# Bluear7878/Remote-Sensing-Vision-Language-Diffusion-Model

Measured on NVIDIA B200. Metric: stage2_denoise_steps_per_s_1024sq_cfg2, higher is better.
Workload: dtype bf16

## Files before the change

include/b200sr.h:

```cpp
#ifndef B200SR_H_
#define B200SR_H_

#include <stddef.h>
#include <stdint.h>

#ifdef __cplusplus
extern "C" {
#endif

int b200sr_abi_version(void);
int b200sr_num_sms(void);

typedef struct b200sr_epilogue {
  const float* bias;
  const float* rowvec;
  int32_t rows_per_group;
  int64_t ld_rowvec;
  const void* residual;
  int64_t ldr;
  void* out;
  int64_t ldc;
  int32_t out_fp32;
  int32_t geglu;
  float alpha;
  int32_t act;
  int32_t softmax_valid;
  int32_t w_dynamic;
  int32_t w_rows_per_group;
  int64_t w_group_stride;
  const float* a_gn_stats;
  const float* a_gn_weight;
  const float* a_gn_bias;
  int32_t a_gn_groups;
  int32_t a_gn_silu;
  const float* ln_stats;
  int32_t ln_parts;
  const float* ln_colsum;
  const float* ln_shift;
  float ln_eps;
  float* ln_stats_out;
  int32_t row_softmax;
  int32_t row_softmax_valid;
} b200sr_epilogue;

int b200sr_gemm_bf16(const void* A, int64_t lda, const void* W, int32_t M, int32_t N, int32_t K,
                     const b200sr_epilogue* epi, int32_t force_bn, void* stream);

int b200sr_gemm_n_tile(int32_t M, int32_t N, int32_t K);

int b200sr_conv3x3_bf16(const void* x, const void* w, int32_t N, int32_t H, int32_t W, int32_t Cin, int32_t Cout,
                        int32_t stride, int32_t pad_lo, const b200sr_epilogue* epi, int32_t force_bn, void* stream);

int b200sr_conv3x3_small(const void* x, const void* w, const float* bias, const void* addend, void* y, int32_t N,
                         int32_t H, int32_t W, int32_t Cin, int32_t Cout, int32_t out_nchw_f32, void* stream);

size_t b200sr_group_norm_workspace_bytes(int32_t N, int32_t HW, int32_t C, int32_t groups);
int b200sr_group_norm_launches(int32_t N, int32_t HW, int32_t C, int32_t groups);
int b200sr_group_norm_nhwc(const void* x, void* y, const float* weight, const float* bias, int32_t N, int32_t HW,
                           int32_t C, int32_t groups, float eps, int32_t silu, const void* sft_gamma,
                           const void* sft_beta, const void* raw, float control_scale, void* workspace, void* stream);

int b200sr_group_norm_stats(const void* x, int32_t N, int32_t HW, int32_t C, int32_t groups, float eps, float* stats_out,
                            void* workspace, void* stream);

int b200sr_layer_norm(const void* x, void* y, const float* weight, const float* bias, int32_t M, int32_t C, float eps,
                      void* stream);

size_t b200sr_attention_d64_workspace_bytes(int32_t B, int32_t H, int32_t Nq, int32_t Nk);
int b200sr_attention_d64(const void* q, int64_t ldq, int32_t q_col, const void* k, int64_t ldk, int32_t k_col,
                         const void* v, int64_t ldv, int32_t v_col, void* out, int64_t ldo, int32_t B, int32_t H,
                         int32_t Nq, int32_t Nk, float scale, int32_t causal, void* workspace, void* stream);

int b200sr_row_softmax_fold(const float* parts, int32_t n_parts, int64_t rows, float* out, void* stream);

int b200sr_softmax_rows(const float* x, void* y, int32_t rows, int32_t cols, int32_t valid_cols, float scale,
                        void* stream);

int b200sr_nchw_f32_to_nhwc_bf16(const float* x, void* y, int32_t N, int32_t C, int32_t HW, float scale, void* stream);
int b200sr_nhwc_bf16_to_nchw_f32(const void* x, float* y, int32_t N, int32_t C, int32_t HW, void* stream);
int b200sr_nhwc_bf16_to_nchw_f32_strided(const void* x, float* y, int32_t N, int32_t C, int32_t Cs, int32_t HW, void* stream);

int b200sr_upsample2x_nhwc(const void* x, void* y, int32_t N, int32_t H, int32_t W, int32_t C, void* stream);

int b200sr_concat_add(const void* a, int32_t Ca, const void* b, int32_t Cb, const void* c, void* out, int64_t rows,
                      void* stream);

int b200sr_axpy_bf16(const void* a, const void* b, void* y, float alpha, int64_t n, void* stream);

int b200sr_pad_channels(const void* x, void* y, int32_t C, int32_t Cpad, int64_t rows, void* stream);

int b200sr_silu_bf16(const void* x, void* y, int64_t n, void* stream);

int b200sr_embed_tokens(const int64_t* ids, const float* tok, const float* pos, void* out, int32_t B, int32_t T, int32_t C,
                        int32_t vocab, void* stream);

int b200sr_sinusoid_embedding(const float* t, void* out, int32_t B, int32_t dim, float max_period, int32_t sin_first,
                              void* stream);

int b200sr_sampler_pre(const float* x, const float* noise, const float* scalars, float* x_hat, void* net_in, int32_t B,
                       int32_t C, int32_t HW, int32_t cfg_copies, void* stream);
int b200sr_sampler_post(const float* eps, const float* x_hat, const float* scalars, float* denoised_out, float* x_next,
                        int32_t B, int32_t C, int32_t HW, int32_t use_cfg, void* stream);
int b200sr_euler_from_denoised(const float* denoised, const float* x_hat, const float* scalars, float* x_next,
                               int64_t n, void* stream);

int b200sr_tile_accumulate(const float* tile, const float* weight, float* acc, float* cnt, int32_t BC, int32_t th,
                           int32_t tw, int32_t H, int32_t W, int32_t h0, int32_t w0, void* stream);
int b200sr_tile_normalize(const float* acc, const float* cnt, float* out, int64_t n, void* stream);

int b200sr_tile_weighted_strip(const float* tile, const float* weight, float* strip, int32_t BC, int32_t th, int32_t tw,
                               int32_t y0, int32_t x0, int32_t sh, int32_t sw, void* stream);
int b200sr_strip_add(const float* strip, float* acc, int32_t BC, int32_t sh, int32_t sw, int32_t H, int32_t W,
                     int32_t h0, int32_t w0, void* stream);

int b200sr_pointwise_small(const void* x, const float* w, const float* bias, void* y, int32_t Cin, int32_t Cout,
                           int64_t rows, int32_t HW, int32_t out_nchw_f32, float scale, void* stream);
int b200sr_diag_gaussian(const float* moments, const float* noise, float* z, int32_t N, int32_t C, int32_t HW,
                         float scale, void* stream);

int b200sr_wavelet_level(const float* img, float* low, float* high, int32_t first, int32_t BC, int32_t H, int32_t W,
                         int32_t radius, void* stream);
int b200sr_add_f32(const float* a, const float* b, float* out, int64_t n, void* stream);
int b200sr_image_to_u8(const float* x, void* out, int32_t C, int32_t H, int32_t W, int32_t OH, int32_t OW, void* stream);

int b200sr_tensor2img_u8(const float* x, void* out, int32_t C, int32_t H, int32_t W, void* stream);
int b200sr_resample_u8(const void* src, void* dst, int32_t outer, int32_t in_len, int32_t out_len, int32_t inner,
                       const int32_t* bounds, const int32_t* coeffs, int32_t ksize, void* stream);
int b200sr_img_u8_to_tensor(const void* in, float* out, int32_t C, int32_t H, int32_t W, void* stream);

typedef struct b200sr_copy {
  const void* src;
  void* dst;
  int64_t bytes;
} b200sr_copy;
int b200sr_copy_batch(const b200sr_copy* copies, int32_t n, void* stream);

int b200sr_rel_l1_similarity(const void* prev, const void* cur, int64_t n, const float* threshold, void* workspace,
                             float* result, void* stream);

int b200sr_sr3_update(const float* x, const float* eps, const float* noise, const float* scalars, float* out,
                      int64_t n, void* stream);

#ifdef __cplusplus
}
#endif
#endif
```

remote-sensing-vision-language-diffusion-model_b200/b200sr/_lib.py:

```python
from __future__ import annotations

import ctypes as C
import os

_HERE = os.path.dirname(os.path.abspath(__file__))
LIB_PATH = os.path.join(_HERE, os.environ.get("B200SR_LIB", "libb200sr.so"))

ABI_VERSION = 6

c_void_p, c_int, c_i64, c_float, c_size_t = C.c_void_p, C.c_int32, C.c_int64, C.c_float, C.c_size_t


class Epilogue(C.Structure):

    _fields_ = [
        ("bias", c_void_p),
        ("rowvec", c_void_p),
        ("rows_per_group", c_int),
        ("ld_rowvec", c_i64),
        ("residual", c_void_p),
        ("ldr", c_i64),
        ("out", c_void_p),
        ("ldc", c_i64),
        ("out_fp32", c_int),
        ("geglu", c_int),
        ("alpha", c_float),
        ("act", c_int),
        ("softmax_valid", c_int),
        ("w_dynamic", c_int),
        ("w_rows_per_group", c_int),
        ("w_group_stride", c_i64),
        ("a_gn_stats", c_void_p),
        ("a_gn_weight", c_void_p),
        ("a_gn_bias", c_void_p),
        ("a_gn_groups", c_int),
        ("a_gn_silu", c_int),
        ("ln_stats", c_void_p),
        ("ln_parts", c_int),
        ("ln_colsum", c_void_p),
        ("ln_shift", c_void_p),
        ("ln_eps", c_float),
        ("ln_stats_out", c_void_p),
        ("row_softmax", c_int),
        ("row_softmax_valid", c_int),
    ]


class Copy(C.Structure):

    _fields_ = [("src", c_void_p), ("dst", c_void_p), ("bytes", c_i64)]


def binding_snippet() -> str:
    names = {c_void_p: "C.c_void_p", c_int: "C.c_int32", c_i64: "C.c_int64", c_float: "C.c_float"}
    out = []
    for cls, cname in ((Epilogue, "b200sr_epilogue"), (Copy, "b200sr_copy")):
        out.append(f"class {cls.__name__}(C.Structure):  # {cname} (ABI version {ABI_VERSION})")
        out.append("    _fields_ = [")
        for fname, ftype in cls._fields_:
            out.append(f'        ("{fname}", {names[ftype]}),')
        out.append("    ]")
        out.append("")
    return "\n".join(out).rstrip() + "\n"


P = c_void_p
SIGNATURES = {
    "b200sr_abi_version": (c_int, []),
    "b200sr_num_sms": (c_int, []),
    "b200sr_gemm_bf16": (c_int, [P, c_i64, P, c_int, c_int, c_int, C.POINTER(Epilogue), c_int, P]),
    "b200sr_gemm_n_tile": (c_int, [c_int, c_int, c_int]),
    "b200sr_row_softmax_fold": (c_int, [P, c_int, c_i64, P, P]),
    "b200sr_conv3x3_bf16": (c_int, [P, P, c_int, c_int, c_int, c_int, c_int, c_int, c_int, C.POINTER(Epilogue), c_int, P]),
    "b200sr_pointwise_small": (c_int, [P, P, P, P, c_int, c_int, c_i64, c_int, c_int, c_float, P]),
    "b200sr_diag_gaussian": (c_int, [P, P, P, c_int, c_int, c_int, c_float, P]),
    "b200sr_conv3x3_small": (c_int, [P, P, P, P, P, c_int, c_int, c_int, c_int, c_int, c_int, P]),
    "b200sr_group_norm_workspace_bytes": (c_size_t, [c_int, c_int, c_int, c_int]),
    "b200sr_group_norm_launches": (c_int, [c_int, c_int, c_int, c_int]),
    "b200sr_group_norm_nhwc": (
        c_int,
        [P, P, P, P, c_int, c_int, c_int, c_int, c_float, c_int, P, P, P, c_float, P, P],
    ),
    "b200sr_group_norm_stats": (c_int, [P, c_int, c_int, c_int, c_int, c_float, P, P, P]),
    "b200sr_layer_norm": (c_int, [P, P, P, P, c_int, c_int, c_float, P]),
    "b200sr_attention_d64": (
        c_int,
        [P, c_i64, c_int, P, c_i64, c_int, P, c_i64, c_int, P, c_i64, c_int, c_int, c_int, c_int, c_float, c_int, P, P],
    ),
    "b200sr_attention_d64_workspace_bytes": (C.c_size_t, [c_int, c_int, c_int, c_int]),
    "b200sr_softmax_rows": (c_int, [P, P, c_int, c_int, c_int, c_float, P]),
    "b200sr_nchw_f32_to_nhwc_bf16": (c_int, [P, P, c_int, c_int, c_int, c_float, P]),
    "b200sr_nhwc_bf16_to_nchw_f32": (c_int, [P, P, c_int, c_int, c_int, P]),
    "b200sr_nhwc_bf16_to_nchw_f32_strided": (c_int, [P, P, c_int, c_int, c_int, c_int, P]),
    "b200sr_upsample2x_nhwc": (c_int, [P, P, c_int, c_int, c_int, c_int, P]),
    "b200sr_concat_add": (c_int, [P, c_int, P, c_int, P, P, c_i64, P]),
    "b200sr_axpy_bf16": (c_int, [P, P, P, c_float, c_i64, P]),
    "b200sr_silu_bf16": (c_int, [P, P, c_i64, P]),
    "b200sr_pad_channels": (c_int, [P, P, c_int, c_int, c_i64, P]),
    "b200sr_embed_tokens": (c_int, [P, P, P, P, c_int, c_int, c_int, c_int, P]),
    "b200sr_sinusoid_embedding": (c_int, [P, P, c_int, c_int, c_float, c_int, P]),
    "b200sr_sampler_pre": (c_int, [P, P, P, P, P, c_int, c_int, c_int, c_int, P]),
    "b200sr_sampler_post": (c_int, [P, P, P, P, P, c_int, c_int, c_int, c_int, P]),
    "b200sr_euler_from_denoised": (c_int, [P, P, P, P, c_i64, P]),
    "b200sr_tile_accumulate": (c_int, [P, P, P, P, c_int, c_int, c_int, c_int, c_int, c_int, c_int, P]),
    "b200sr_tile_normalize": (c_int, [P, P, P, c_i64, P]),
    "b200sr_rel_l1_similarity": (c_int, [P, P, c_i64, P, P, P, P]),
    "b200sr_sr3_update": (c_int, [P, P, P, P, P, c_i64, P]),
    "b200sr_wavelet_level": (c_int, [P, P, P, c_int, c_int, c_int, c_int, c_int, P]),
    "b200sr_add_f32": (c_int, [P, P, P, c_i64, P]),
    "b200sr_image_to_u8": (c_int, [P, P, c_int, c_int, c_int, c_int, c_int, P]),
    "b200sr_tensor2img_u8": (c_int, [P, P, c_int, c_int, c_int, P]),
    "b200sr_resample_u8": (c_int, [P, P, c_int, c_int, c_int, c_int, P, P, c_int, P]),
    "b200sr_img_u8_to_tensor": (c_int, [P, P, c_int, c_int, c_int, P]),
    "b200sr_copy_batch": (c_int, [C.POINTER(Copy), c_int, P]),
    "b200sr_tile_weighted_strip": (c_int, [P, P, P, c_int, c_int, c_int, c_int, c_int, c_int, c_int, P]),
    "b200sr_strip_add": (c_int, [P, P, c_int, c_int, c_int, c_int, c_int, c_int, c_int, P]),
}

_ERRORS = {-22: "EINVAL (bad shape / alignment / flags)", -19: "ENODEV (no sm_100 device / driver)", -5: "EIO (CUDA launch error)"}

_lib = None


class B200SRError(RuntimeError):
    pass


def load() -> C.CDLL:
    global _lib
    if _lib is not None:
        return _lib
    if not os.path.exists(LIB_PATH):
        raise B200SRError(
            f"{LIB_PATH} not found: build the sm_100a extension first "
            "(python -c 'import __graft_entry__ as g; g.build()' or csrc/build.sh). There is no CPU fallback."
        )
    lib = C.CDLL(LIB_PATH)
    for name, (res, args) in SIGNATURES.items():
        fn = getattr(lib, name)
        fn.restype = res
        fn.argtypes = args
    if lib.b200sr_abi_version() != ABI_VERSION:
        raise B200SRError(f"libb200sr.so ABI {lib.b200sr_abi_version()} != binding ABI {ABI_VERSION}; rebuild")
    _lib = lib
    return lib


LAUNCHES = [0]


TRACE = None


def check(rc: int, what: str, kernels: int = 1) -> None:
    LAUNCHES[0] += kernels
    if TRACE is not None:
        TRACE.extend([what] * kernels)
    if rc != 0:
        raise B200SRError(f"{what} failed: {_ERRORS.get(rc, rc)}")
```

remote-sensing-vision-language-diffusion-model_b200/b200sr/modules.py:

```python
from __future__ import annotations

import os
from typing import Dict, List, Optional

import torch
import torch.nn as nn

from . import ops

bf16 = torch.bfloat16


def exists(x):
    return x is not None


def zero_module(module: nn.Module) -> nn.Module:
    for p in module.parameters():
        p.detach().zero_()
    return module


def to_nhwc(x: torch.Tensor) -> torch.Tensor:
    if x.dim() != 4:
        raise ValueError(f"expected a 4-D NCHW tensor, got {tuple(x.shape)}")
    v = x.permute(0, 2, 3, 1)
    if x.dtype == bf16 and v.is_contiguous():
        return v
    if x.dtype == torch.float32 and x.is_contiguous():
        return ops.nchw_to_nhwc_bf16(x)
    return v.to(bf16).contiguous()


def from_nhwc(y: torch.Tensor) -> torch.Tensor:
    return y.permute(0, 3, 1, 2)


def tokens_bf16(x: torch.Tensor) -> torch.Tensor:
    if x.dtype == bf16 and x.is_contiguous():
        return x
    if x.dtype == torch.float32:
        return ops.cast_bf16(x.contiguous())
    return x.to(bf16).contiguous()


class Packed:

    def _pk(self, name: str, params, fn):
        cache = self.__dict__.setdefault("_pk_cache", {})
        key = tuple((p.data_ptr(), p._version, str(p.device)) for p in params)
        hit = cache.get(name)
        if hit is None or hit[0] != key:
            with torch.no_grad():
                hit = (key, fn(*params))
            cache[name] = hit
        return hit[1]


_F32 = lambda p: p.detach().float().contiguous()


def _silu_of(emb: torch.Tensor) -> torch.Tensor:
    s = getattr(emb, "_b200sr_silu", None)
    if s is None:
        s = ops.silu(tokens_bf16(emb))
        try:
            emb._b200sr_silu = s
        except Exception:
            pass
    return s


class EmbSlot:

    def __init__(self, table):
        self._b200sr_rb = table


def _resblocks_of(root: nn.Module):
    blocks = root.__dict__.get("_b200sr_resblocks")
    if blocks is None:
        blocks = [m for m in root.modules() if isinstance(m, ResBlock)]
        root.__dict__["_b200sr_resblocks"] = blocks
    return blocks


def rb_table(root: nn.Module, proj: torch.Tensor):
    table, off = {}, 0
    for blk in _resblocks_of(root):
        table[id(blk)] = proj[:, off:off + blk.out_channels]
        off += blk.out_channels
    return table


def _project_emb_for_resblocks(holder: Packed, root: nn.Module, emb: torch.Tensor) -> Optional[torch.Tensor]:
    blocks = _resblocks_of(root)
    if not blocks:
        return None
    params = tuple(p for blk in blocks for p in (blk.emb_layers[1].weight, blk.emb_layers[1].bias))
    w_all, b_all = holder._pk("rb_emb", params, lambda *ps: (
        torch.cat([ops.pack_linear(w) for w in ps[0::2]], 0).contiguous(),
        torch.cat([_F32(b) for b in ps[1::2]], 0).contiguous()))
    proj = ops.gemm(_silu_of(emb), w_all, b_all, out_fp32=True)
    try:
        emb._b200sr_rb = rb_table(root, proj)
        emb._b200sr_proj = proj
    except Exception:
        pass
    return proj


def timestep_embedding(timesteps: torch.Tensor, dim: int, max_period: float = 10000.0) -> torch.Tensor:
    return ops.sinusoid_embedding(timesteps, dim, max_period, sin_first=False)


class GroupNorm32(nn.GroupNorm):
    """util.py:258-276 — parameter container; the fused kernel is invoked by the owning block."""


def normalization(channels: int) -> nn.GroupNorm:
    return GroupNorm32(32, channels)


def _gn(norm: nn.GroupNorm, x_nhwc: torch.Tensor, silu: bool = False, **kw) -> torch.Tensor:
    return ops.group_norm(x_nhwc, norm.weight, norm.bias, groups=norm.num_groups, eps=norm.eps, silu=silu, **kw)


def _conv3x3(holder: Packed, name: str, conv: nn.Conv2d, x_nhwc: torch.Tensor, **kw) -> torch.Tensor:
    w = holder._pk(name + ".w", (conv.weight,), ops.pack_conv3x3)
    b = holder._pk(name + ".b", (conv.bias,), _F32) if conv.bias is not None else None
    return ops.conv3x3(x_nhwc, w, b, **kw)


FUSE_LN_INTO_GEMM = os.environ.get("B200SR_FUSE_LN", "1") != "0"
FUSE_GN_INTO_CONV = True


def _gn_silu_conv3x3(holder: Packed, name: str, norm: nn.GroupNorm, conv: nn.Conv2d, x_nhwc: torch.Tensor, **kw) -> torch.Tensor:
    if FUSE_GN_INTO_CONV and ops.conv3x3_gn_fusable(x_nhwc, 1, conv.out_channels) and norm.affine:
        stats = ops.group_norm_stats(x_nhwc, norm.num_groups, norm.eps)
        return _conv3x3(holder, name, conv, x_nhwc, gn=(stats, norm.weight, norm.bias, norm.num_groups, True), **kw)
    return _conv3x3(holder, name, conv, _gn(norm, x_nhwc, silu=True), **kw)


def _linear(holder: Packed, name: str, lin, x: torch.Tensor, **kw) -> torch.Tensor:
    w = holder._pk(name + ".w", (lin.weight,), ops.pack_linear)
    b = holder._pk(name + ".b", (lin.bias,), _F32) if lin.bias is not None else None
    return ops.gemm(x, w, b, **kw)


class TimestepBlock(nn.Module):
    """openaimodel.py:63-72."""


class Upsample(nn.Module, Packed):

    def __init__(self, channels, use_conv, dims=2, out_channels=None, padding=1, third_up=False):
        super().__init__()
        assert dims == 2 and padding == 1
        self.channels, self.out_channels, self.use_conv, self.dims = channels, out_channels or channels, use_conv, dims
        if use_conv:
            self.conv = nn.Conv2d(self.channels, self.out_channels, 3, padding=padding)

    def forward_nhwc(self, x):
        assert x.shape[-1] == self.channels
        x = ops.upsample2x(x)
        return _conv3x3(self, "conv", self.conv, x) if self.use_conv else x

    def forward(self, x):
        return from_nhwc(self.forward_nhwc(to_nhwc(x)))


class Downsample(nn.Module, Packed):

    def __init__(self, channels, use_conv, dims=2, out_channels=None, padding=1, third_down=False):
        super().__init__()
        assert dims == 2 and use_conv and padding == 1, "only the learned stride-2 convolution is on the hot path"
        self.channels, self.out_channels, self.use_conv, self.dims = channels, out_channels or channels, use_conv, dims
        self.op = nn.Conv2d(self.channels, self.out_channels, 3, stride=2, padding=padding)

    def forward_nhwc(self, x):
        assert x.shape[-1] == self.channels
        return _conv3x3(self, "op", self.op, x, stride=2)

    def forward(self, x):
        return from_nhwc(self.forward_nhwc(to_nhwc(x)))


class ResBlock(TimestepBlock, Packed):

    def __init__(self, channels, emb_channels, dropout, out_channels=None, use_conv=False, use_scale_shift_norm=False,
                 dims=2, use_checkpoint=False, up=False, down=False, kernel_size=3, exchange_temb_dims=False,
                 skip_t_emb=False):
        super().__init__()
        assert dims == 2 and kernel_size == 3 and not (up or down or use_scale_shift_norm or skip_t_emb or use_conv)
        self.channels, self.emb_channels, self.dropout = channels, emb_channels, dropout
        self.out_channels = out_channels or channels
        self.use_checkpoint, self.use_scale_shift_norm = use_checkpoint, use_scale_shift_norm
        self.in_layers = nn.Sequential(normalization(channels), nn.SiLU(),
                                       nn.Conv2d(channels, self.out_channels, 3, padding=1))
        self.updown = False
        self.h_upd = self.x_upd = nn.Identity()
        self.emb_layers = nn.Sequential(nn.SiLU(), nn.Linear(emb_channels, self.out_channels))
        self.out_layers = nn.Sequential(normalization(self.out_channels), nn.SiLU(), nn.Dropout(p=dropout),
                                        zero_module(nn.Conv2d(self.out_channels, self.out_channels, 3, padding=1)))
        if self.out_channels == channels:
            self.skip_connection = nn.Identity()
        else:
            self.skip_connection = nn.Conv2d(channels, self.out_channels, 1)

    def forward_nhwc(self, x, emb):
        pre = getattr(emb, "_b200sr_rb", None)
        emb_out = pre.get(id(self)) if pre is not None else None
        if emb_out is None:
            emb_out = _linear(self, "emb", self.emb_layers[1], _silu_of(emb), out_fp32=True)
        h = _gn_silu_conv3x3(self, "conv1", self.in_layers[0], self.in_layers[2], x, rowvec=emb_out)
        skip = x if isinstance(self.skip_connection, nn.Identity) else _linear(self, "skip", self.skip_connection, x)
        return _gn_silu_conv3x3(self, "conv2", self.out_layers[0], self.out_layers[3], h, residual=skip)

    def forward(self, x, emb):
        return from_nhwc(self.forward_nhwc(to_nhwc(x), emb))


class GEGLU(nn.Module, Packed):

    def __init__(self, dim_in, dim_out):
        super().__init__()
        self.proj = nn.Linear(dim_in, dim_out * 2)

    def forward(self, x, ln=None):
        if ln is not None:
            norm, stats = ln
            w, colsum, shift = self._pk("proj_ln", (self.proj.weight, self.proj.bias, norm.weight, norm.bias),
                                        ops.pack_geglu_ln)
            return ops.gemm(tokens_bf16(x), w, None, geglu=True, ln=(stats, colsum, shift, norm.eps))
        w, b = self._pk("proj", (self.proj.weight, self.proj.bias), ops.pack_geglu)
        return ops.gemm(tokens_bf16(x), w, b, geglu=True)


class FeedForward(nn.Module, Packed):

    def __init__(self, dim, dim_out=None, mult=4, glu=False, dropout=0.0):
        super().__init__()
        assert glu, "only the gated feed-forward is on the hot path"
        inner_dim = int(dim * mult)
        dim_out = dim_out or dim
        self.net = nn.Sequential(GEGLU(dim, inner_dim), nn.Dropout(dropout), nn.Linear(inner_dim, dim_out))

    def forward(self, x, residual: Optional[torch.Tensor] = None, ln=None, want_stats: bool = False):
        return _linear(self, "out", self.net[2], self.net[0](x, ln=ln), residual=residual, want_stats=want_stats)


class CrossAttention(nn.Module, Packed):

    def __init__(self, query_dim, context_dim=None, heads=8, dim_head=64, dropout=0.0, backend=None):
        super().__init__()
        assert dim_head == 64, "the tcgen05 attention kernel is specialised for head_dim 64"
        inner_dim = dim_head * heads
        context_dim = context_dim or query_dim
        self.scale, self.heads = dim_head**-0.5, heads
        self.to_q = nn.Linear(query_dim, inner_dim, bias=False)
        self.to_k = nn.Linear(context_dim, inner_dim, bias=False)
        self.to_v = nn.Linear(context_dim, inner_dim, bias=False)
        self.to_out = nn.Sequential(nn.Linear(inner_dim, query_dim), nn.Dropout(dropout))
        self.backend = backend

    def attend(self, x, context=None, kv=None, ln=None):
        inner = self.to_q.weight.shape[0]
        if context is None:
            if ln is not None:
                norm, stats = ln
                w, colsum, shift = self._pk(
                    "qkv_ln", (self.to_q.weight, self.to_k.weight, self.to_v.weight, norm.weight, norm.bias),
                    lambda q, k, v, g, b: ops.pack_linear_ln(torch.cat([q, k, v], 0), g, b))
                qkv = ops.gemm(x, w, ln=(stats, colsum, shift, norm.eps))
            else:
                w = self._pk("qkv", (self.to_q.weight, self.to_k.weight, self.to_v.weight),
                             lambda q, k, v: torch.cat([q, k, v], 0).to(bf16).contiguous())
                qkv = ops.gemm(x, w)
            return ops.attention(qkv, qkv, qkv, self.heads, q_col=0, k_col=inner, v_col=2 * inner, scale=self.scale)
        q = _linear(self, "q", self.to_q, x)
        bound = self._bound_entry(context)
        if kv is not None:
            pass
        elif bound is not None:
            kv = bound[1]
        else:
            kv = ops.gemm(context, self._wkv())
        if kv.shape[0] != q.shape[0]:
            if q.shape[0] % kv.shape[0]:
                raise ValueError(f"context batch {kv.shape[0]} does not divide the query batch {q.shape[0]}")
            kv = kv.repeat_interleave(q.shape[0] // kv.shape[0], dim=0)
        return ops.attention(q, kv, kv, self.heads, q_col=0, k_col=0, v_col=inner, scale=self.scale)

    def _wkv(self):
        return self._pk("kv", (self.to_k.weight, self.to_v.weight), lambda k, v: torch.cat([k, v], 0).to(bf16).contiguous())

    def _fold_norm(self) -> Optional[nn.LayerNorm]:
        return self.__dict__.get("_pre_norm") if FUSE_LN_INTO_GEMM else None

    def _weights_key(self):
        ps = [self.to_q.weight, self.to_k.weight, self.to_v.weight, self.to_out[0].weight]
        norm = self._fold_norm()
        if norm is not None:
            ps += [norm.weight, norm.bias]
        return tuple((p.data_ptr(), p._version) for p in ps)

    def _bound_entry(self, context):
        if context is None:
            return None
        table = self.__dict__.get("_static")
        if not table:
            return None
        e = table.get(id(context))
        if e is None or e[0] is not context:
            return None
        if e[3] != self._weights_key():
            if torch.cuda.is_current_stream_capturing():
                raise RuntimeError("cross-attention weights changed after bind_static_context(); re-bind before capture")
            self.bind_static_context(context)
            e = table[id(context)]
        return e

    def bind_static_context(self, context: Optional[torch.Tensor]) -> None:
        table = self.__dict__.setdefault("_static", {})
        if context is None:
            table.clear()
            return
        old = table.get(id(context))
        shape = (*context.shape[:-1], 2 * self.to_q.weight.shape[0])
        same = old is not None and old[0] is context and tuple(old[1].shape) == shape
        kv = ops.gemm(context, self._wkv(), out=old[1] if same else None)
        fused = self._fold_projections(context)
        if same and old[2] is not None and fused is not None and len(old[2]) == len(fused):
            for dst, src in zip(old[2], fused):
                dst.copy_(src)
            fused = old[2]
        table[id(context)] = (context, kv, fused, self._weights_key())

    def bound_tensors(self, context):
        e = self.__dict__.get("_static", {}).get(id(context))
        if e is None or e[0] is not context:
            return []
        return [e[1]] + ([t for t in e[2] if t.is_cuda or t.dim() > 0] if e[2] is not None else [])

    SEG = 80

    @torch.no_grad()
    def _fold_projections(self, context: torch.Tensor):
        b, tk = context.shape[0], context.shape[1]
        if context.dim() != 3 or tk > self.SEG:
            return None
        h, c = self.heads, self.to_q.weight.shape[1]
        ctx = context.float()
        k = (ctx @ self.to_k.weight.float().t()).view(b, tk, h, 64)
        v = (ctx @ self.to_v.weight.float().t()).view(b, tk, h, 64)
        wq = self.to_q.weight.float().view(h, 64, c)
        wo = self.to_out[0].weight.float().view(-1, h, 64)
        kp = torch.zeros(b, h, self.SEG, c, device=context.device)
        kp[:, :, :tk] = torch.einsum("bjhd,hdc->bhjc", k, wq) * (self.scale * 1.4426950408889634)
        vp = torch.zeros(b, h, self.SEG, wo.shape[0], device=context.device)
        vp[:, :, :tk] = torch.einsum("bjhd,chd->bhjc", v, wo)
        kp = kp.reshape(b, h * self.SEG, c)
        vpt = vp.reshape(b, h * self.SEG, -1).transpose(1, 2).to(bf16).contiguous()
        norm = self._fold_norm()
        if norm is None:
            return (kp.to(bf16).contiguous(), vpt, torch.tensor(tk))
        kg = (kp * norm.weight.float()).to(bf16).contiguous()
        return (kg, vpt, torch.tensor(tk), kg.float().sum(-1).contiguous(), (kp @ norm.bias.float()).contiguous())

    def forward(self, x, context=None, mask=None, additional_tokens=None, n_times_crossframe_attn_in_self=0,
                residual: Optional[torch.Tensor] = None, alpha: float = 1.0, kv: Optional[torch.Tensor] = None,
                ln=None, want_stats: bool = False):
        if mask is not None or additional_tokens is not None or n_times_crossframe_attn_in_self:
            raise NotImplementedError("masks / additional tokens / cross-frame attention are not on the hot path")
        x = tokens_bf16(x)
        ctx = tokens_bf16(context) if context is not None else None
        if ctx is not None and kv is None and x.dim() == 3 and x.shape[1] % 256 == 0:
            bound = self._bound_entry(ctx)
            folds_ln = bound is not None and bound[2] is not None and len(bound[2]) == 5
            if folds_ln and (ln is None or ln[0] is not self._fold_norm()):
                bound = None
            if bound is not None and bound[2] is not None and x.shape[0] % bound[2][0].shape[0] == 0:
                k_fold, v_fold, tk = bound[2][:3]
                rpg = x.shape[1] * (x.shape[0] // k_fold.shape[0])
                if folds_ln:
                    p = ops.gemm(x, k_fold, softmax_valid=int(tk), w_rows_per_group=rpg,
                                 ln=(ln[1], bound[2][3], bound[2][4], ln[0].eps))
                else:
                    if ln is not None:
                        x = ops.layer_norm(x, ln[0].weight, ln[0].bias, ln[0].eps)
                    p = ops.gemm(x, k_fold, softmax_valid=int(tk), w_rows_per_group=rpg)
                bias = self._pk("out.b", (self.to_out[0].bias,), _F32)
                return ops.gemm(p, v_fold, bias, residual=residual, alpha=alpha, w_rows_per_group=rpg,
                                want_stats=want_stats)
        if ln is not None and ctx is not None:
            x, ln = ops.layer_norm(x, ln[0].weight, ln[0].bias, ln[0].eps), None
        return _linear(self, "out", self.to_out[0], self.attend(x, ctx, kv, ln=ln), residual=residual, alpha=alpha,
                       want_stats=want_stats)


MemoryEfficientCrossAttention = CrossAttention


class BasicTransformerBlock(nn.Module):

    def __init__(self, dim, n_heads, d_head, dropout=0.0, context_dim=None, gated_ff=True, checkpoint=True,
                 disable_self_attn=False, attn_mode="softmax", sdp_backend=None):
        super().__init__()
        self.disable_self_attn = disable_self_attn
        self.attn1 = CrossAttention(query_dim=dim, heads=n_heads, dim_head=d_head, dropout=dropout,
                                    context_dim=context_dim if disable_self_attn else None)
        self.ff = FeedForward(dim, dropout=dropout, glu=gated_ff)
        self.attn2 = CrossAttention(query_dim=dim, context_dim=context_dim, heads=n_heads, dim_head=d_head,
                                    dropout=dropout)
        self.norm1, self.norm2, self.norm3 = nn.LayerNorm(dim), nn.LayerNorm(dim), nn.LayerNorm(dim)
        self.checkpoint = checkpoint
        self.attn2.__dict__["_pre_norm"] = self.norm2

    @staticmethod
    def _ln(norm: nn.LayerNorm, x):
        return ops.layer_norm(x, norm.weight, norm.bias, norm.eps)

    def forward(self, x, context=None, additional_tokens=None, n_times_crossframe_attn_in_self=0, stats=None,
                want_stats: bool = False):
        x = tokens_bf16(x)
        if stats is None:
            x = self.attn1(self._ln(self.norm1, x), context=context if self.disable_self_attn else None, residual=x)
            x = self.attn2(self._ln(self.norm2, x), context=context, residual=x)
            return self.ff(self._ln(self.norm3, x), residual=x, want_stats=want_stats)
        x, stats = self.attn1(x, context=context if self.disable_self_attn else None, residual=x,
                              ln=(self.norm1, stats), want_stats=True)
        x, stats = self.attn2(x, context=context, residual=x, ln=(self.norm2, stats), want_stats=True)
        return self.ff(x, residual=x, ln=(self.norm3, stats), want_stats=want_stats)


class SpatialTransformer(nn.Module, Packed):

    def __init__(self, in_channels, n_heads, d_head, depth=1, dropout=0.0, context_dim=None, disable_self_attn=False,
                 use_linear=False, attn_type="softmax", use_checkpoint=True, sdp_backend=None):
        super().__init__()
        assert use_linear, "the YAML selects use_linear_in_transformer=True"
        if exists(context_dim) and not isinstance(context_dim, (list, tuple)):
            context_dim = [context_dim]
        if exists(context_dim):
            context_dim = list(context_dim)
            if depth != len(context_dim):
                assert all(c == context_dim[0] for c in context_dim)
                context_dim = depth * [context_dim[0]]
        else:
            context_dim = [None] * depth
        self.in_channels = in_channels
        inner_dim = n_heads * d_head
        self.norm = nn.GroupNorm(num_groups=32, num_channels=in_channels, eps=1e-6, affine=True)
        self.proj_in = nn.Linear(in_channels, inner_dim)
        self.transformer_blocks = nn.ModuleList([
            BasicTransformerBlock(inner_dim, n_heads, d_head, dropout=dropout, context_dim=context_dim[d],
                                  disable_self_attn=disable_self_attn, attn_mode=attn_type, checkpoint=use_checkpoint)
            for d in range(depth)])
        self.proj_out = zero_module(nn.Linear(inner_dim, in_channels))
        self.use_linear = use_linear

    def forward_nhwc(self, x, context=None):
        if not isinstance(context, list):
            context = [context]
        context = [tokens_bf16(c) if c is not None else None for c in context]
        b, h, w, c = x.shape
        t = _gn(self.norm, x).view(b, h * w, c)
        stats = None
        if FUSE_LN_INTO_GEMM:
            t, stats = _linear(self, "proj_in", self.proj_in, t, want_stats=True)
        else:
            t = _linear(self, "proj_in", self.proj_in, t)
        last = len(self.transformer_blocks) - 1
        for i, block in enumerate(self.transformer_blocks):
            r = block(t, context=context[i if len(context) > 1 else 0], stats=stats,
                      want_stats=stats is not None and i < last)
            t, stats = r if isinstance(r, tuple) else (r, None)
        t = _linear(self, "proj_out", self.proj_out, t, residual=x.view(b, h * w, c))
        return t.view(b, h, w, c)

    def forward(self, x, context=None):
        return from_nhwc(self.forward_nhwc(to_nhwc(x), context))


class TimestepEmbedSequential(nn.Sequential, TimestepBlock):

    def forward_nhwc(self, x, emb, context=None):
        for layer in self:
            if isinstance(layer, TimestepBlock):
                x = layer.forward_nhwc(x, emb)
            elif isinstance(layer, SpatialTransformer):
                x = layer.forward_nhwc(x, context)
            elif isinstance(layer, nn.Conv2d):
                x = _stem_conv(layer, x)
            else:
                x = layer.forward_nhwc(x)
        return x

    def forward(self, x, emb, context=None, **unused):
        return from_nhwc(self.forward_nhwc(to_nhwc(x), emb, context))


def _stem_conv(conv: nn.Conv2d, x_nhwc: torch.Tensor, addend: Optional[torch.Tensor] = None) -> torch.Tensor:
    cache = conv.__dict__.setdefault("_pk_cache", {})
    key = (conv.weight.data_ptr(), conv.weight._version, conv.bias.data_ptr(), conv.bias._version)
    if cache.get("key") != key:
        with torch.no_grad():
            cache["key"], cache["w"], cache["b"] = key, ops.pack_conv3x3_padded(conv.weight, 64), _F32(conv.bias)
    return ops.conv3x3(ops.pad_channels(x_nhwc, 64), cache["w"], cache["b"], residual=addend)


class UNetModel(nn.Module, Packed):

    def __init__(self, in_channels, model_channels, out_channels, num_res_blocks, attention_resolutions, dropout=0,
                 channel_mult=(1, 2, 4, 8), conv_resample=True, dims=2, num_classes=None, use_checkpoint=False,
                 use_fp16=False, num_heads=-1, num_head_channels=-1, num_heads_upsample=-1, use_scale_shift_norm=False,
                 resblock_updown=False, use_new_attention_order=False, use_spatial_transformer=False,
                 transformer_depth=1, context_dim=None, n_embed=None, legacy=True, disable_self_attentions=None,
                 num_attention_blocks=None, disable_middle_self_attn=False, use_linear_in_transformer=False,
                 spatial_transformer_attn_type="softmax", adm_in_channels=None, use_fairscale_checkpoint=False,
                 offload_to_cpu=False, transformer_depth_middle=None, _build_output_blocks=True):
        super().__init__()
        assert use_spatial_transformer and context_dim is not None and dims == 2 and conv_resample
        assert not resblock_updown and not use_scale_shift_norm and n_embed is None
        assert num_head_channels != -1 or num_heads != -1
        if isinstance(context_dim, (list, tuple)) or type(context_dim).__name__ == "ListConfig":
            context_dim = list(context_dim)
        self.in_channels, self.model_channels, self.out_channels = in_channels, model_channels, out_channels
        if isinstance(transformer_depth, int):
            transformer_depth = len(channel_mult) * [transformer_depth]
        transformer_depth = list(transformer_depth)
        transformer_depth_middle = transformer_depth[-1] if transformer_depth_middle is None else transformer_depth_middle
        if isinstance(num_res_blocks, int):
            self.num_res_blocks = len(channel_mult) * [num_res_blocks]
        else:
            if len(num_res_blocks) != len(channel_mult):
                raise ValueError("provide num_res_blocks either as an int (globally constant) or as a list/tuple "
                                 "(per-level) with the same length as channel_mult")
            self.num_res_blocks = list(num_res_blocks)
        self.attention_resolutions, self.dropout, self.channel_mult = attention_resolutions, dropout, channel_mult
        self.conv_resample, self.num_classes, self.use_checkpoint = conv_resample, num_classes, use_checkpoint
        self.num_heads, self.num_head_channels = num_heads, num_head_channels
        self.num_heads_upsample = num_heads if num_heads_upsample == -1 else num_heads_upsample
        self.predict_codebook_ids = False

        time_embed_dim = model_channels * 4
        self.time_embed = nn.Sequential(nn.Linear(model_channels, time_embed_dim), nn.SiLU(),
                                        nn.Linear(time_embed_dim, time_embed_dim))
        if num_classes is not None:
            if num_classes != "sequential":
                raise ValueError("only num_classes='sequential' (SDXL vector conditioning) is on the hot path")
            assert adm_in_channels is not None
            self.label_emb = nn.Sequential(nn.Sequential(nn.Linear(adm_in_channels, time_embed_dim), nn.SiLU(),
                                                         nn.Linear(time_embed_dim, time_embed_dim)))

        def heads_for(ch):
            if num_head_channels == -1:
                return num_heads, ch // num_heads
            return ch // num_head_channels, num_head_channels

        def transformer(ch, depth, level=None, middle=False):
            nh, dh = heads_for(ch)
            if legacy:
                dh = ch // nh
            disabled = disable_middle_self_attn if middle else (
                disable_self_attentions[level] if exists(disable_self_attentions) else False)
            return SpatialTransformer(ch, nh, dh, depth=depth, context_dim=context_dim, disable_self_attn=disabled,
                                      use_linear=use_linear_in_transformer, attn_type=spatial_transformer_attn_type,
                                      use_checkpoint=use_checkpoint)

        self.input_blocks = nn.ModuleList([TimestepEmbedSequential(nn.Conv2d(in_channels, model_channels, 3, padding=1))])
        input_block_chans = [model_channels]
        ch, ds = model_channels, 1
        for level, mult in enumerate(channel_mult):
            for nr in range(self.num_res_blocks[level]):
                layers = [ResBlock(ch, time_embed_dim, dropout, out_channels=mult * model_channels, dims=dims,
                                   use_checkpoint=use_checkpoint)]
                ch = mult * model_channels
                if ds in attention_resolutions and (not exists(num_attention_blocks) or nr < num_attention_blocks[level]):
                    layers.append(transformer(ch, transformer_depth[level], level))
                self.input_blocks.append(TimestepEmbedSequential(*layers))
                input_block_chans.append(ch)
            if level != len(channel_mult) - 1:
                self.input_blocks.append(TimestepEmbedSequential(Downsample(ch, conv_resample, dims=dims, out_channels=ch)))
                input_block_chans.append(ch)
                ds *= 2
        self.middle_block = TimestepEmbedSequential(
            ResBlock(ch, time_embed_dim, dropout, dims=dims, use_checkpoint=use_checkpoint),
            transformer(ch, transformer_depth_middle, middle=True),
            ResBlock(ch, time_embed_dim, dropout, dims=dims, use_checkpoint=use_checkpoint))
        if not _build_output_blocks:
            return
        self.output_blocks = nn.ModuleList([])
        for level, mult in list(enumerate(channel_mult))[::-1]:
            for i in range(self.num_res_blocks[level] + 1):
                ich = input_block_chans.pop()
                layers = [ResBlock(ch + ich, time_embed_dim, dropout, out_channels=model_channels * mult, dims=dims,
                                   use_checkpoint=use_checkpoint)]
                ch = model_channels * mult
                if ds in attention_resolutions and (not exists(num_attention_blocks) or i < num_attention_blocks[level]):
                    layers.append(transformer(ch, transformer_depth[level], level))
                if level and i == self.num_res_blocks[level]:
                    layers.append(Upsample(ch, conv_resample, dims=dims, out_channels=ch))
                    ds //= 2
                self.output_blocks.append(TimestepEmbedSequential(*layers))
        self.out = nn.Sequential(normalization(ch), nn.SiLU(),
                                 zero_module(nn.Conv2d(model_channels, out_channels, 3, padding=1)))

    def _embed(self, timesteps, y):
        t_emb = timestep_embedding(timesteps, self.model_channels)
        h = _linear(self, "te0", self.time_embed[0], t_emb, act=1)
        if self.num_classes is None:
            emb = _linear(self, "te2", self.time_embed[2], h)
        else:
            emb_t = _linear(self, "te2", self.time_embed[2], h)
            l = _linear(self, "le0", self.label_emb[0][0], tokens_bf16(y), act=1)
            emb = _linear(self, "le2", self.label_emb[0][2], l, residual=emb_t)
        _project_emb_for_resblocks(self, self, emb)
        return emb

    def _out_nchw_f32(self, h_nhwc):
        h = _gn(self.out[0], h_nhwc, silu=True)
        conv = self.out[2]
        w8, b8 = self._pk("out.wb8", (conv.weight, conv.bias), ops.pack_conv3x3_few_out)
        return ops.conv3x3_to_nchw_f32(h, w8, b8, conv.weight.shape[0])

    def forward(self, x, timesteps=None, context=None, y=None, **kwargs):
        assert (y is not None) == (self.num_classes is not None)
        emb = self._embed(timesteps, y)
        ctx = tokens_bf16(context)
        h, hs = to_nhwc(x), []
        for module in self.input_blocks:
            h = module.forward_nhwc(h, emb, ctx)
            hs.append(h)
        h = self.middle_block.forward_nhwc(h, emb, ctx)
        for module in self.output_blocks:
            h = module.forward_nhwc(ops.concat_add(h, hs.pop()), emb, ctx)
        return self._out_nchw_f32(h)


class ZeroSFT(nn.Module, Packed):

    def __init__(self, label_nc, norm_nc, concat_channels=0, norm=True, mask=False):
        super().__init__()
        assert norm
        self.norm = norm
        self.param_free_norm = normalization(norm_nc + concat_channels)
        nhidden = 128
        self.mlp_shared = nn.Sequential(nn.Conv2d(label_nc, nhidden, kernel_size=3, padding=1), nn.SiLU())
        self.zero_mul = zero_module(nn.Conv2d(nhidden, norm_nc + concat_channels, kernel_size=3, padding=1))
        self.zero_add = zero_module(nn.Conv2d(nhidden, norm_nc + concat_channels, kernel_size=3, padding=1))
        self.zero_conv = zero_module(nn.Conv2d(label_nc, norm_nc, 1, 1, 0))
        self.pre_concat = bool(concat_channels != 0)
        self.mask = mask

    def precompute(self, c):
        actv = _conv3x3(self, "mlp", self.mlp_shared[0], c, act=1)
        return {"zc": _linear(self, "zero_conv", self.zero_conv, c),
                "gamma": _conv3x3(self, "mul", self.zero_mul, actv), "beta": _conv3x3(self, "add", self.zero_add, actv)}

    def forward_nhwc(self, c, h, h_ori=None, control_scale=1, pre=None):
        assert self.mask is False
        cat = h_ori is not None and self.pre_concat
        if h_ori is not None and not self.pre_concat:
            raise NotImplementedError("post-concat ZeroSFT is not used by LightGLVUNet")
        control_scale = float(control_scale)
        if pre is None:
            hz = _linear(self, "zero_conv", self.zero_conv, c, residual=h)
            hc = ops.concat_add(h_ori, hz) if cat else hz
            actv = _conv3x3(self, "mlp", self.mlp_shared[0], c, act=1)
            gamma = _conv3x3(self, "mul", self.zero_mul, actv)
            beta = _conv3x3(self, "add", self.zero_add, actv)
        else:
            hc = ops.concat_add(h_ori, h, pre["zc"]) if cat else ops.axpy(h, pre["zc"], 1.0)
            gamma, beta = pre["gamma"], pre["beta"]
        raw = None
        if control_scale != 1.0:
            raw = ops.concat_add(h_ori, h) if cat else h
        return _gn(self.param_free_norm, hc, sft_gamma=gamma, sft_beta=beta, raw=raw, control_scale=control_scale)

    def forward(self, c, h, h_ori=None, control_scale=1):
        return from_nhwc(self.forward_nhwc(to_nhwc(c), to_nhwc(h), None if h_ori is None else to_nhwc(h_ori),
                                           control_scale))


class ZeroCrossAttn(nn.Module, Packed):

    def __init__(self, context_dim, query_dim, zero_out=True, mask=False):
        super().__init__()
        self.attn = CrossAttention(query_dim=query_dim, context_dim=context_dim, heads=query_dim // 64, dim_head=64)
        self.norm1 = normalization(query_dim)
        self.norm2 = normalization(context_dim)
        self.mask = mask

    def precompute(self, context):
        b, h, w, cc = context.shape
        ct = _gn(self.norm2, context).view(b, h * w, cc)
        return {"kv": ops.gemm(ct, self.attn._wkv())}

    def forward_nhwc(self, context, x, control_scale=1, pre=None):
        assert self.mask is False
        b, h, w, c = x.shape
        xt = _gn(self.norm1, x).view(b, h * w, c)
        if pre is None:
            ct = _gn(self.norm2, context).view(b, h * w, context.shape[-1])
            out = self.attn(xt, ct, residual=x.view(b, h * w, c), alpha=float(control_scale))
        else:
            out = self.attn(xt, xt, residual=x.view(b, h * w, c), alpha=float(control_scale), kv=pre["kv"])
        return out.view(b, h, w, c)

    def forward(self, context, x, control_scale=1):
        return from_nhwc(self.forward_nhwc(to_nhwc(context), to_nhwc(x), control_scale))


class GLVControl(UNetModel):

    def __init__(self, *args, input_upscale=1, **kwargs):
        super().__init__(*args, _build_output_blocks=False, **kwargs)
        assert input_upscale == 1
        self.input_upscale = input_upscale
        self.input_hint_block = TimestepEmbedSequential(
            zero_module(nn.Conv2d(self.in_channels, self.model_channels, 3, padding=1)))

    def forward_nhwc(self, x, timesteps, xt, context, y, emb=None) -> List[torch.Tensor]:
        if emb is None:
            emb = self._embed(timesteps, y)
        hint = _stem_conv(self.input_hint_block[0], x)
        hs = []
        h = _stem_conv(self.input_blocks[0][0], xt, addend=hint)
        hs.append(h)
        for module in list(self.input_blocks)[1:]:
            h = module.forward_nhwc(h, emb, context)
            hs.append(h)
        hs.append(self.middle_block.forward_nhwc(h, emb, context))
        return hs

# ... 189 lines not shown
```

remote-sensing-vision-language-diffusion-model_b200/b200sr/ops.py:

```python
from __future__ import annotations

import ctypes as C
import math
from typing import Optional

import numpy as np
import torch

from . import _lib
from ._lib import Epilogue, check

bf16 = torch.bfloat16


def launch_count() -> int:
    return _lib.LAUNCHES[0]


_profile = None


def set_profile(records) -> None:
    global _profile
    _profile = records


class _Timed:
    def __init__(self, kind: str, flops: float, desc: str = ""):
        self.kind, self.flops, self.desc = kind, flops, desc

    def __enter__(self):
        if _profile is not None:
            self.t0 = torch.cuda.Event(enable_timing=True)
            self.t1 = torch.cuda.Event(enable_timing=True)
            self.t0.record()
        return self

    def __exit__(self, *exc):
        if _profile is not None:
            self.t1.record()
            _profile.append((self.kind, self.flops, self.t0, self.t1, self.desc))
        return False


def _stream() -> int:
    return torch.cuda.current_stream().cuda_stream


def _ptr(t: Optional[torch.Tensor]) -> Optional[int]:
    return None if t is None else t.data_ptr()


def _req(t: torch.Tensor, dtype, name: str) -> None:
    if not t.is_cuda:
        raise _lib.B200SRError(f"{name}: expected a CUDA tensor (b200sr has no CPU path)")
    if t.device.index != torch.cuda.current_device():
        raise _lib.B200SRError(f"{name}: tensor lives on {t.device} but the current CUDA device is "
                               f"{torch.cuda.current_device()}; wrap the call in torch.cuda.device(tensor.device)")
    if t.dtype != dtype:
        raise _lib.B200SRError(f"{name}: expected {dtype}, got {t.dtype}")
    if not t.is_contiguous():
        raise _lib.B200SRError(f"{name}: expected a contiguous tensor")


def require_cuda(t: torch.Tensor, what: str) -> None:
    if not t.is_cuda:
        raise _lib.B200SRError(f"{what} runs on CUDA (sm_100a) only; there is no CPU fallback")


_ws_cache: dict = {}
_ws_retired: list = []
_ws_slot = [0]


class workspace_slot:

    def __init__(self, slot: int):
        self.slot = slot

    def __enter__(self):
        self.prev = _ws_slot[0]
        _ws_slot[0] = self.slot

    def __exit__(self, *exc):
        _ws_slot[0] = self.prev
        return False


def _workspace(device: torch.device, nbytes: int, kind: str = "gn") -> torch.Tensor:
    key = (device.type, device.index, _ws_slot[0], kind)
    ws = _ws_cache.get(key)
    if ws is None or ws.numel() * 4 < nbytes:
        if torch.cuda.is_current_stream_capturing():
            raise _lib.B200SRError("workspace allocation during CUDA-graph capture; run one eager warm-up step first")
        if ws is not None:
            _ws_retired.append(ws)
        floats = max(nbytes // 4 + 1, 1 << 22, 0 if ws is None else 2 * ws.numel())
        ws = torch.zeros(floats, dtype=torch.float32, device=device)
        _ws_cache[key] = ws
    return ws


def pack_linear(weight: torch.Tensor) -> torch.Tensor:
    w = weight.detach().reshape(weight.shape[0], -1)
    return w.to(bf16).contiguous()


def pack_conv3x3(weight: torch.Tensor) -> torch.Tensor:
    co, ci, kh, kw = weight.shape
    assert kh == 3 and kw == 3
    return weight.detach().permute(0, 2, 3, 1).reshape(co, 9 * ci).to(bf16).contiguous()


def geglu_interleave_index(inner: int, device=None) -> torch.Tensor:
    assert inner % 16 == 0
    j = torch.arange(inner, device=device)
    val_pos = (j // 16) * 32 + (j % 16)
    idx = torch.empty(2 * inner, dtype=torch.long, device=device)
    idx[val_pos] = j
    idx[val_pos + 16] = j + inner
    return idx


def pack_geglu(weight: torch.Tensor, bias: torch.Tensor):
    inner = weight.shape[0] // 2
    idx = geglu_interleave_index(inner, weight.device)
    return weight.detach()[idx].to(bf16).contiguous(), bias.detach()[idx].float().contiguous()


def pack_linear_ln(weight: torch.Tensor, gamma: torch.Tensor, beta: torch.Tensor, bias: Optional[torch.Tensor] = None):
    w32 = weight.detach().float()
    wp = (w32 * gamma.detach().float()[None, :]).to(bf16).contiguous()
    shift = w32 @ beta.detach().float()
    if bias is not None:
        shift = shift + bias.detach().float()
    return wp, wp.float().sum(1)[None].contiguous(), shift[None].contiguous()


def pack_geglu_ln(weight: torch.Tensor, bias: torch.Tensor, gamma: torch.Tensor, beta: torch.Tensor):
    idx = geglu_interleave_index(weight.shape[0] // 2, weight.device)
    return pack_linear_ln(weight.detach()[idx], gamma, beta, bias.detach()[idx])


class RowStats:

    __slots__ = ("buf", "parts", "dim")

    def __init__(self, buf: torch.Tensor, parts: int, dim: int):
        self.buf, self.parts, self.dim = buf, parts, dim


_n_tile_cache: dict = {}


def gemm_n_tile(M: int, N: int, K: int) -> int:
    key = (M, N, K)
    t = _n_tile_cache.get(key)
    if t is None:
        t = _lib.load().b200sr_gemm_n_tile(M, N, K)
        if t <= 0:
            raise _lib.B200SRError(f"gemm_n_tile({M}, {N}, {K}) = {t}")
        _n_tile_cache[key] = t
    return t


def _epilogue(out, ldc, bias, rowvec, rows_per_group, residual, ldr, out_fp32, geglu, alpha, act=0,
              softmax_valid=0, w_rows_per_group=0, w_group_stride=0, w_dynamic=False) -> Epilogue:
    e = Epilogue()
    e.bias = _ptr(bias)
    e.rowvec = _ptr(rowvec)
    e.rows_per_group = rows_per_group
    e.ld_rowvec = rowvec.stride(0) if rowvec is not None and rowvec.dim() == 2 else 0
    e.residual = _ptr(residual)
    e.ldr = ldr
    e.out = out.data_ptr()
    e.ldc = ldc
    e.out_fp32 = int(out_fp32)
    e.geglu = int(geglu)
    e.alpha = float(alpha)
    e.act = int(act)
    e.softmax_valid = int(softmax_valid)
    e.w_dynamic = int(w_dynamic)
    e.w_rows_per_group = int(w_rows_per_group)
    e.w_group_stride = int(w_group_stride)
    return e


def gemm(
    a: torch.Tensor,
    w: torch.Tensor,
    bias: Optional[torch.Tensor] = None,
    *,
    residual: Optional[torch.Tensor] = None,
    rowvec: Optional[torch.Tensor] = None,
    rows_per_group: int = 0,
    geglu: bool = False,
    alpha: float = 1.0,
    act: int = 0,
    out: Optional[torch.Tensor] = None,
    out_fp32: bool = False,
    force_bn: int = 0,
    softmax_valid: int = 0,
    w_rows_per_group: int = 0,
    w_dynamic: bool = False,
    ln=None,
    want_stats: bool = False,
):
    _req(w, bf16, "gemm.w")
    if a.dtype != bf16 or not a.is_cuda:
        raise _lib.B200SRError("gemm.a: expected CUDA bf16")
    K = a.shape[-1]
    N = w.shape[-2]
    w_group_stride = 0
    if w_rows_per_group:
        assert w.dim() == 3 and w.is_contiguous() and w.shape[0] * w_rows_per_group >= a.numel() // K
        w_group_stride = N
    a2 = a.reshape(-1, K)
    if a2.stride(-1) != 1:
        a2 = a2.contiguous()
    M, lda = a2.shape[0], a2.stride(0)
    n_out = N // 2 if geglu else N
    if out is None:
        out = torch.empty(*a.shape[:-1], n_out, dtype=torch.float32 if out_fp32 else bf16, device=a.device)
    o2 = out.reshape(-1, n_out) if out.is_contiguous() else out
    assert o2.shape[-1] == n_out and o2.stride(-1) == 1
    ldc = o2.stride(-2) if o2.dim() >= 2 else n_out
    ldr = 0
    if residual is not None:
        r2 = residual if residual.dim() == 2 else residual.reshape(-1, residual.shape[-1])
        assert r2.dtype == bf16 and r2.stride(-1) == 1
        ldr = r2.stride(0)
    e = _epilogue(o2, ldc, bias, rowvec, rows_per_group, residual, ldr, out_fp32, geglu, alpha, act,
                  softmax_valid, w_rows_per_group, w_group_stride, w_dynamic)
    if ln is not None:
        st, colsum, shift, eps = ln
        groups = w.shape[0] if w_rows_per_group else 1
        if st.buf.shape[1] != M or st.dim != K:
            raise _lib.B200SRError(f"gemm.ln: statistics of a [{st.buf.shape[1]}, {st.dim}] matrix, a is [{M}, {K}]")
        for t, nme in ((colsum, "colsum"), (shift, "shift")):
            _req(t, torch.float32, f"gemm.ln.{nme}")
            if t.numel() != groups * N:
                raise _lib.B200SRError(f"gemm.ln.{nme}: expected [{groups}, {N}]")
        e.ln_stats, e.ln_parts, e.ln_colsum, e.ln_shift, e.ln_eps = st.buf.data_ptr(), st.parts, colsum.data_ptr(), \
            shift.data_ptr(), float(eps)
    stats = None
    if want_stats:
        if geglu or softmax_valid or out_fp32:
            raise _lib.B200SRError("gemm.want_stats: plain bf16 output only")
        parts = -(-N // (force_bn if force_bn > 0 else gemm_n_tile(M, N, K)))
        stats = RowStats(torch.empty(parts, M, 2, dtype=torch.float32, device=a.device), parts, N)
        e.ln_stats_out = stats.buf.data_ptr()
    with _Timed("gemm", 2.0 * M * N * K, f"M{M} N{N} K{K}{' geglu' if geglu else ''}{' ln' if ln is not None else ''}"):
        rc = _lib.load().b200sr_gemm_bf16(a2.data_ptr(), lda, w.data_ptr(), M, N, K, C.byref(e), force_bn, _stream())
    check(rc, f"gemm M={M} N={N} K={K}")
    return (out, stats) if want_stats else out


def conv3x3(
    x: torch.Tensor,
    w: torch.Tensor,
    bias: Optional[torch.Tensor] = None,
    *,
    stride: int = 1,
    rowvec: Optional[torch.Tensor] = None,
    residual: Optional[torch.Tensor] = None,
    alpha: float = 1.0,
    act: int = 0,
    out: Optional[torch.Tensor] = None,
    force_bn: int = 0,
    pad_lo: int = 1,
    gn=None,
) -> torch.Tensor:
    _req(x, bf16, "conv3x3.x")
    _req(w, bf16, "conv3x3.w")
    n, h, wd, cin = x.shape
    cout = w.shape[0]
    assert w.shape[1] == 9 * cin
    oh, ow = h // stride, wd // stride
    if out is None:
        out = torch.empty(n, oh, ow, cout, dtype=bf16, device=x.device)
    ldc = out.stride(2)
    ldr = residual.stride(2) if residual is not None else 0
    e = _epilogue(out, ldc, bias, rowvec, 0, residual, ldr, False, False, alpha, act)
    if gn is not None:
        stats, gw, gb, groups, gsilu = gn
        _req(stats, torch.float32, "conv3x3.gn.stats")
        e.a_gn_stats, e.a_gn_weight, e.a_gn_bias = stats.data_ptr(), gw.data_ptr(), gb.data_ptr()
        e.a_gn_groups, e.a_gn_silu = int(groups), int(gsilu)
    with _Timed("conv3x3", 2.0 * n * oh * ow * cout * 9 * cin, f"{n}x{h}x{wd} Cin{cin} Cout{cout} s{stride}"):
        rc = _lib.load().b200sr_conv3x3_bf16(
            x.data_ptr(), w.data_ptr(), n, h, wd, cin, cout, stride, pad_lo, C.byref(e), force_bn, _stream()
        )
    check(rc, f"conv3x3 N={n} H={h} W={wd} Cin={cin} Cout={cout} s={stride}")
    return out


def conv3x3_small(
    x: torch.Tensor,
    w: torch.Tensor,
    bias: Optional[torch.Tensor],
    *,
    addend: Optional[torch.Tensor] = None,
    out_nchw_f32: bool = False,
) -> torch.Tensor:
    _req(x, bf16, "conv3x3_small.x")
    _req(w, bf16, "conv3x3_small.w")
    n, h, wd, cin = x.shape
    cout = w.shape[0]
    if out_nchw_f32:
        out = torch.empty(n, cout, h, wd, dtype=torch.float32, device=x.device)
    else:
        out = torch.empty(n, h, wd, cout, dtype=bf16, device=x.device)
    rc = _lib.load().b200sr_conv3x3_small(
        x.data_ptr(), w.data_ptr(), _ptr(bias), _ptr(addend), out.data_ptr(), n, h, wd, cin, cout, int(out_nchw_f32),
        _stream()
    )
    check(rc, f"conv3x3_small Cin={cin} Cout={cout}")
    return out


def group_norm(
    x: torch.Tensor,
    weight: Optional[torch.Tensor],
    bias: Optional[torch.Tensor],
    *,
    groups: int = 32,
    eps: float = 1e-5,
    silu: bool = False,
    sft_gamma: Optional[torch.Tensor] = None,
    sft_beta: Optional[torch.Tensor] = None,
    raw: Optional[torch.Tensor] = None,
    control_scale: float = 1.0,
) -> torch.Tensor:
    _req(x, bf16, "group_norm.x")
    n, c = x.shape[0], x.shape[-1]
    hw = x.numel() // (n * c)
    lib = _lib.load()
    ws = _workspace(x.device, lib.b200sr_group_norm_workspace_bytes(n, hw, c, groups))
    y = torch.empty_like(x)
    nbytes = 2.0 * x.numel() * (2 + (2 if sft_gamma is not None else 0) + (1 if raw is not None and control_scale != 1.0 else 0))
    with _Timed("group_norm", nbytes, f"N{n} HW{hw} C{c}{' sft' if sft_gamma is not None else ''}"):
        rc = lib.b200sr_group_norm_nhwc(
            x.data_ptr(), y.data_ptr(), _ptr(weight), _ptr(bias), n, hw, c, groups, eps, int(silu), _ptr(sft_gamma),
            _ptr(sft_beta), _ptr(raw), float(control_scale), ws.data_ptr(), _stream()
        )
    check(rc, f"group_norm N={n} HW={hw} C={c}", kernels=max(1, lib.b200sr_group_norm_launches(n, hw, c, groups)))
    return y


GN_FUSE_MAX_COUT = 256


def conv3x3_gn_fusable(x: torch.Tensor, stride: int = 1, cout: Optional[int] = None) -> bool:
    ok = stride == 1 and x.dim() == 4 and x.shape[2] % 8 == 0 and x.shape[1] >= 16 and x.shape[3] % 64 == 0
    return ok and (cout is None or cout <= GN_FUSE_MAX_COUT)


def group_norm_stats(x: torch.Tensor, groups: int = 32, eps: float = 1e-5) -> torch.Tensor:
    _req(x, bf16, "group_norm_stats.x")
    n, c = x.shape[0], x.shape[-1]
    hw = x.numel() // (n * c)
    lib = _lib.load()
    ws = _workspace(x.device, lib.b200sr_group_norm_workspace_bytes(n, hw, c, groups))
    stats = torch.empty(n, groups, 2, dtype=torch.float32, device=x.device)
    with _Timed("group_norm", 2.0 * x.numel(), f"N{n} HW{hw} C{c} stats"):
        rc = lib.b200sr_group_norm_stats(x.data_ptr(), n, hw, c, groups, eps, stats.data_ptr(), ws.data_ptr(), _stream())
    check(rc, f"group_norm_stats N={n} HW={hw} C={c}")
    return stats


def layer_norm(x: torch.Tensor, weight: torch.Tensor, bias: torch.Tensor, eps: float = 1e-5) -> torch.Tensor:
    _req(x, bf16, "layer_norm.x")
    c = x.shape[-1]
    m = x.numel() // c
    y = torch.empty_like(x)
    with _Timed("layer_norm", 4.0 * x.numel(), f"M{m} C{c}"):
        rc = _lib.load().b200sr_layer_norm(x.data_ptr(), y.data_ptr(), weight.data_ptr(), bias.data_ptr(), m, c, eps, _stream())
    check(rc, f"layer_norm M={m} C={c}")
    return y


def attention(
    q: torch.Tensor, k: torch.Tensor, v: torch.Tensor, heads: int, *, q_col: int = 0, k_col: int = 0, v_col: int = 0,
    scale: Optional[float] = None, causal: bool = False
) -> torch.Tensor:
    for t, nme in ((q, "q"), (k, "k"), (v, "v")):
        _req(t, bf16, f"attention.{nme}")
    b, nq, ldq = q.shape
    nk = k.shape[1]
    out = torch.empty(b, nq, heads * 64, dtype=bf16, device=q.device)
    lib = _lib.load()
    ws_bytes = lib.b200sr_attention_d64_workspace_bytes(b, heads, nq, nk)
    ws = _workspace(q.device, ws_bytes, "attn") if ws_bytes else None
    with _Timed("attention", 4.0 * b * heads * nq * nk * 64, f"B{b} H{heads} Nq{nq} Nk{nk}"):
        rc = lib.b200sr_attention_d64(
            q.data_ptr(), ldq, q_col, k.data_ptr(), k.shape[2], k_col, v.data_ptr(), v.shape[2], v_col, out.data_ptr(),
            heads * 64, b, heads, nq, nk, float(scale if scale is not None else 0.125), int(causal), _ptr(ws), _stream()
        )
    check(rc, f"attention B={b} H={heads} Nq={nq} Nk={nk}")
    return out


def softmax_rows(x: torch.Tensor, scale: float = 1.0, valid_cols: Optional[int] = None) -> torch.Tensor:
    _req(x, torch.float32, "softmax_rows.x")
    cols = x.shape[-1]
    y = torch.empty(x.shape, dtype=bf16, device=x.device)
    check(_lib.load().b200sr_softmax_rows(x.data_ptr(), y.data_ptr(), x.numel() // cols, cols,
                                          cols if valid_cols is None else valid_cols, float(scale), _stream()),
          "softmax_rows")
    return y


SCORE_CHUNK_BYTES = 1 << 30


def gemm_row_softmax(a: torch.Tensor, w: torch.Tensor, scale: float, valid_cols: Optional[int] = None,
                     w_dynamic: bool = True) -> torch.Tensor:
    _req(w, bf16, "gemm_row_softmax.w")
    _req(a, bf16, "gemm_row_softmax.a")
    K, N = a.shape[-1], w.shape[0]
    a2 = a.reshape(-1, K)
    if a2.stride(-1) != 1:
        a2 = a2.contiguous()
    M, lda = a2.shape[0], a2.stride(0)
    parts = -(-N // gemm_n_tile(M, N, K))
    stats = torch.empty(parts, M, 2, dtype=torch.float32, device=a.device)
    out = torch.empty(M, N, dtype=bf16, device=a.device)
    lib = _lib.load()
    folded = torch.empty(M, 2, dtype=torch.float32, device=a.device) if parts > 1 else stats
    for which in (1, 2):
        e = _epilogue(out, N, None, None, 0, None, 0, False, False, float(scale) * 1.4426950408889634, 0, 0, 0, 0, w_dynamic)
        e.row_softmax, e.row_softmax_valid = which, int(valid_cols) if valid_cols is not None else N
        if which == 1:
            e.out, e.ln_stats_out = None, stats.data_ptr()
        else:
            if parts > 1:
                check(lib.b200sr_row_softmax_fold(stats.data_ptr(), parts, M, folded.data_ptr(), _stream()), "row_softmax_fold")
            e.ln_stats, e.ln_parts = folded.data_ptr(), 1
        with _Timed("gemm", 2.0 * M * N * K, f"M{M} N{N} K{K} row softmax pass {which}"):
            rc = lib.b200sr_gemm_bf16(a2.data_ptr(), lda, w.data_ptr(), M, N, K, C.byref(e), 0, _stream())
        check(rc, f"gemm_row_softmax pass {which} M={M} N={N} K={K}")
    return out


TWO_PASS_SOFTMAX = True


def single_head_attention(q: torch.Tensor, k: torch.Tensor, v_t: torch.Tensor, scale: float,
                          out_bias: Optional[torch.Tensor] = None, valid_keys: Optional[int] = None) -> torch.Tensor:
    t, c = q.shape
    tk = k.shape[0]
    two_pass = TWO_PASS_SOFTMAX and tk % 8 == 0
    rows = (SCORE_CHUNK_BYTES // ((2 if two_pass else 4) * tk)) // 256 * 256
    rows = max(256, min(rows, t))
    out = torch.empty(t, c, dtype=bf16, device=q.device)
    for r0 in range(0, t, rows):
        r1 = min(t, r0 + rows)
        if two_pass:
            p = gemm_row_softmax(q[r0:r1], k, scale, valid_keys)
        else:
            s = gemm(q[r0:r1], k, out_fp32=True, w_dynamic=True)
            p = softmax_rows(s, scale, valid_cols=valid_keys)
        gemm(p, v_t, out_bias, w_dynamic=True, out=out[r0:r1])
    return out


def nchw_to_nhwc_bf16(x: torch.Tensor, scale: float = 1.0) -> torch.Tensor:
    _req(x, torch.float32, "nchw_to_nhwc.x")
    n, c, h, w = x.shape
    y = torch.empty(n, h, w, c, dtype=bf16, device=x.device)
    check(_lib.load().b200sr_nchw_f32_to_nhwc_bf16(x.data_ptr(), y.data_ptr(), n, c, h * w, float(scale), _stream()),
          "nchw_to_nhwc")
    return y


def cast_bf16(x: torch.Tensor) -> torch.Tensor:
    if x.dtype == bf16:
        return x if x.is_contiguous() else x.contiguous()
    _req(x, torch.float32, "cast_bf16.x")
    y = torch.empty(x.shape, dtype=bf16, device=x.device)
    check(_lib.load().b200sr_nchw_f32_to_nhwc_bf16(x.data_ptr(), y.data_ptr(), 1, 1, x.numel(), 1.0, _stream()),
          "cast_bf16")
    return y


def nhwc_to_nchw_f32(x: torch.Tensor) -> torch.Tensor:
    _req(x, bf16, "nhwc_to_nchw.x")
    n, h, w, c = x.shape
    y = torch.empty(n, c, h, w, dtype=torch.float32, device=x.device)
    check(_lib.load().b200sr_nhwc_bf16_to_nchw_f32(x.data_ptr(), y.data_ptr(), n, c, h * w, _stream()), "nhwc_to_nchw")
    return y


def pack_conv3x3_few_out(weight: torch.Tensor, bias: Optional[torch.Tensor]):
    co = weight.shape[0]
    w = torch.zeros(8, *weight.shape[1:], dtype=weight.dtype, device=weight.device)
    w[:co] = weight.detach()
    b = torch.zeros(8, dtype=torch.float32, device=weight.device)
    if bias is not None:
        b[:co] = bias.detach().float()
    return pack_conv3x3(w), b


def conv3x3_to_nchw_f32(x: torch.Tensor, w8: torch.Tensor, b8: torch.Tensor, cout: int) -> torch.Tensor:
    y8 = conv3x3(x, w8, b8)
    n, h, wd, cs = y8.shape
    out = torch.empty(n, cout, h, wd, dtype=torch.float32, device=x.device)
    check(_lib.load().b200sr_nhwc_bf16_to_nchw_f32_strided(y8.data_ptr(), out.data_ptr(), n, cout, cs, h * wd, _stream()),
          "nhwc_to_nchw_strided")
    return out


def upsample2x(x: torch.Tensor) -> torch.Tensor:
    _req(x, bf16, "upsample2x.x")
    n, h, w, c = x.shape
    y = torch.empty(n, 2 * h, 2 * w, c, dtype=bf16, device=x.device)
    check(_lib.load().b200sr_upsample2x_nhwc(x.data_ptr(), y.data_ptr(), n, h, w, c, _stream()), "upsample2x")
    return y


def concat_add(a: Optional[torch.Tensor], b: torch.Tensor, c: Optional[torch.Tensor] = None) -> torch.Tensor:
    _req(b, bf16, "concat_add.b")
    ca = 0 if a is None else a.shape[-1]
    cb = b.shape[-1]
    rows = b.numel() // cb
    out = torch.empty(*b.shape[:-1], ca + cb, dtype=bf16, device=b.device)
    check(_lib.load().b200sr_concat_add(_ptr(a), ca, b.data_ptr(), cb, _ptr(c), out.data_ptr(), rows, _stream()),
          "concat_add")
    return out


def axpy(a: torch.Tensor, b: torch.Tensor, alpha: float = 1.0) -> torch.Tensor:
    _req(a, bf16, "axpy.a")
    _req(b, bf16, "axpy.b")
    y = torch.empty_like(a)
    check(_lib.load().b200sr_axpy_bf16(a.data_ptr(), b.data_ptr(), y.data_ptr(), float(alpha), a.numel(), _stream()),
          "axpy")
    return y


def pad_channels(x: torch.Tensor, cpad: int) -> torch.Tensor:
    _req(x, bf16, "pad_channels.x")
    c = x.shape[-1]
    y = torch.empty(*x.shape[:-1], cpad, dtype=bf16, device=x.device)
    check(_lib.load().b200sr_pad_channels(x.data_ptr(), y.data_ptr(), c, cpad, x.numel() // c, _stream()), "pad_channels")
    return y


def pack_conv3x3_padded(weight: torch.Tensor, cin_pad: int) -> torch.Tensor:
    co, ci, kh, kw = weight.shape
    w = torch.zeros(co, 3, 3, cin_pad, dtype=weight.dtype, device=weight.device)
    w[..., :ci] = weight.detach().permute(0, 2, 3, 1)
    return w.reshape(co, 9 * cin_pad).to(bf16).contiguous()


def pointwise_small(x: torch.Tensor, w: torch.Tensor, bias: Optional[torch.Tensor], *, out_nchw_f32: bool = False,
                    scale: float = 1.0) -> torch.Tensor:
    _req(x, bf16, "pointwise_small.x")
    n, h, wd, cin = x.shape
    cout = w.shape[0]
# ... 262 lines not shown
```

remote-sensing-vision-language-diffusion-model_b200/csrc/capi.cu:

```cuda
#include "../../include/b200sr.h"
#include <stdlib.h>

#include "common.cuh"

namespace b200sr {

PFN_encodeTiled get_encode_tiled() {
  static PFN_encodeTiled fn = nullptr;
  static bool tried = false;
  if (!tried) {
    tried = true;
    void* p = nullptr;
    cudaDriverEntryPointQueryResult q;
    if (cudaGetDriverEntryPoint("cuTensorMapEncodeTiled", &p, cudaEnableDefault, &q) == cudaSuccess &&
        q == cudaDriverEntryPointSuccess)
      fn = reinterpret_cast<PFN_encodeTiled>(p);
  }
  return fn;
}

bool pdl_enabled() {
  static int v = -1;
  if (v < 0) {
    const char* e = getenv("B200SR_PDL");
    v = (e != nullptr && e[0] == '0') ? 0 : 1;
  }
  return v == 1;
}

int num_sms() {
  static int cached[64] = {0};
  int dev = 0;
  if (cudaGetDevice(&dev) != cudaSuccess || dev < 0 || dev >= 64) return 148;
  if (cached[dev] == 0) {
    int n = 0;
    if (cudaDeviceGetAttribute(&n, cudaDevAttrMultiProcessorCount, dev) != cudaSuccess || n <= 0) n = 148;
    cached[dev] = n;
  }
  return cached[dev];
}

bool first_use_on_device(bool (&flags)[64]) {
  int dev = 0;
  if (cudaGetDevice(&dev) != cudaSuccess || dev < 0 || dev >= 64) return true;
  if (flags[dev]) return false;
  flags[dev] = true;
  return true;
}

static int make_tmap_any(CUtensorMap* out, CUtensorMapDataType dtype, const void* base, int rank, const uint64_t* dims,
                         const uint64_t* strides_bytes, const uint32_t* box, int swizzle_bytes);

int make_tmap_bf16(CUtensorMap* out, const void* base, int rank, const uint64_t* dims, const uint64_t* strides_bytes,
                   const uint32_t* box, int swizzle_bytes) {
  return make_tmap_any(out, CU_TENSOR_MAP_DATA_TYPE_BFLOAT16, base, rank, dims, strides_bytes, box, swizzle_bytes);
}

int make_tmap_f32(CUtensorMap* out, const void* base, int rank, const uint64_t* dims, const uint64_t* strides_bytes,
                  const uint32_t* box) {
  return make_tmap_any(out, CU_TENSOR_MAP_DATA_TYPE_FLOAT32, base, rank, dims, strides_bytes, box, 128);
}

static int make_tmap_any(CUtensorMap* out, CUtensorMapDataType dtype, const void* base, int rank, const uint64_t* dims,
                         const uint64_t* strides_bytes, const uint32_t* box, int swizzle_bytes) {
  PFN_encodeTiled enc = get_encode_tiled();
  if (enc == nullptr) return B200SR_ENODEV;
  if ((reinterpret_cast<uintptr_t>(base) & 15) != 0) return B200SR_EINVAL;
  cuuint64_t gdim[5];
  cuuint64_t gstr[4];
  cuuint32_t bdim[5];
  cuuint32_t estr[5];
  for (int i = 0; i < rank; ++i) {
    gdim[i] = dims[i];
    bdim[i] = box[i];
    estr[i] = 1;
    if (box[i] == 0 || box[i] > 256) return B200SR_EINVAL;
  }
  for (int i = 0; i + 1 < rank; ++i) {
    gstr[i] = strides_bytes[i];
    if (gstr[i] % 16 != 0) return B200SR_EINVAL;
  }
  const CUresult r = enc(out, dtype, static_cast<cuuint32_t>(rank), const_cast<void*>(base),
                         gdim, gstr, bdim, estr, CU_TENSOR_MAP_INTERLEAVE_NONE,
                         swizzle_bytes == 64 ? CU_TENSOR_MAP_SWIZZLE_64B : CU_TENSOR_MAP_SWIZZLE_128B,
                         CU_TENSOR_MAP_L2_PROMOTION_L2_256B, CU_TENSOR_MAP_FLOAT_OOB_FILL_NONE);
  return r == CUDA_SUCCESS ? B200SR_OK : B200SR_EINVAL;
}

int gemm_bf16(const void* A, long long lda, const void* W, int M, int N, int K, const EpilogueArgs& e, int force_bn,
              cudaStream_t stream);
int conv3x3_bf16(const void* x, const void* w, int NB, int H, int W, int Cin, int Cout, int stride, int pad_lo,
                 const EpilogueArgs& e, int force_bn, cudaStream_t stream);
int gemm_n_tile(int M, int N, int K);
int pointwise_small(const void* x, const float* w, const float* bias, void* y, int Cin, int Cout, long long rows, int HW,
                    int out_nchw_f32, float scale, cudaStream_t stream);
int diag_gaussian(const float* moments, const float* noise, float* z, int N, int C, int HW, float scale,
                  cudaStream_t stream);
size_t group_norm_workspace_bytes(int N, int HW, int C, int groups);
int group_norm_launches(int N, int HW, int C, int groups);
int group_norm_nhwc(const void* x, void* y, const float* weight, const float* bias, int N, int HW, int C, int groups,
                    float eps, int silu, const void* sft_gamma, const void* sft_beta, const void* raw,
                    float control_scale, float* workspace, cudaStream_t stream);
int group_norm_stats(const void* x, int N, int HW, int C, int groups, float eps, float* stats_out, float* workspace,
                     cudaStream_t stream);
int layer_norm(const void* x, void* y, const float* weight, const float* bias, int M, int C, float eps,
               cudaStream_t stream);
int softmax_rows(const float* x, void* y, int rows, int cols, int valid, float scale, cudaStream_t stream);
int row_softmax_fold(const float* parts, int n_parts, long long rows, float* out, cudaStream_t stream);
int attention_d64(const void* q, long long ldq, int q_col, const void* k, long long ldk, int k_col, const void* v,
                  long long ldv, int v_col, void* out, long long ldo, int B, int H, int Nq, int Nk, float scale,
                  int causal, void* workspace, cudaStream_t stream);
int embed_tokens(const long long* ids, const float* tok, const float* pos, void* out, int B, int T, int C, int vocab,
                 cudaStream_t stream);
size_t attention_d64_workspace_bytes(int B, int H, int Nq, int Nk);
int nchw_f32_to_nhwc_bf16(const float* x, void* y, int N, int C, int HW, float scale, cudaStream_t stream);
int nhwc_bf16_to_nchw_f32(const void* x, float* y, int N, int C, int Cs, int HW, cudaStream_t stream);
int upsample2x_nhwc(const void* x, void* y, int N, int H, int W, int C, cudaStream_t stream);
int concat_add(const void* a, int Ca, const void* b, int Cb, const void* c, void* out, long long rows,
               cudaStream_t stream);
int axpy_bf16(const void* a, const void* b, void* y, float alpha, long long n, cudaStream_t stream);
int silu_bf16(const void* x, void* y, long long n, cudaStream_t stream);
int pad_channels(const void* x, void* y, int C, int Cpad, long long rows, cudaStream_t stream);
int sinusoid_embedding(const float* t, void* out, int B, int dim, float max_period, int sin_first,
                       cudaStream_t stream);
int conv3x3_small(const void* x, const void* w, const float* bias, const void* addend, void* y, int N, int H, int W,
                  int Cin, int Cout, int out_nchw_f32, cudaStream_t stream);
int sampler_pre(const float* x, const float* noise, const float* scalars, float* x_hat, void* net_in, int B, int C,
                int HW, int cfg_copies, cudaStream_t stream);
int sampler_post(const float* eps, const float* x_hat, const float* scalars, float* denoised_out, float* x_next, int B,
                 int C, int HW, int use_cfg, cudaStream_t stream);
int euler_from_denoised(const float* denoised, const float* x_hat, const float* scalars, float* x_next, long long n,
                        cudaStream_t stream);
int tile_accumulate(const float* tile, const float* weight, float* acc, float* cnt, int BC, int th, int tw, int H, int W,
                    int h0, int w0, cudaStream_t stream);
int tile_normalize(const float* acc, const float* cnt, float* out, long long n, cudaStream_t stream);
int rel_l1_similarity(const void* prev, const void* cur, long long n, const float* threshold, double* workspace,
                      float* result, cudaStream_t stream);
int sr3_update(const float* x, const float* eps, const float* noise, const float* scalars, float* out, long long n,
               cudaStream_t stream);
int wavelet_level(const float* img, float* low, float* high, int first, int BC, int H, int W, int radius,
                  cudaStream_t stream);
int add_f32(const float* a, const float* b, float* out, long long n, cudaStream_t stream);
int image_to_u8(const float* x, void* out, int C, int H, int W, int OH, int OW, cudaStream_t stream);
int tensor2img_u8(const float* x, void* out, int C, int H, int W, cudaStream_t stream);
int resample_u8(const void* src, void* dst, int outer, int in_len, int out_len, int inner, const int* bounds,
                const int* coeffs, int ksize, cudaStream_t stream);
int img_u8_to_tensor(const void* in, float* out, int C, int H, int W, cudaStream_t stream);
int copy_batch(const void* const* src, void* const* dst, const long long* bytes, int n, cudaStream_t stream);
int tile_weighted_strip(const float* tile, const float* weight, float* strip, int BC, int th, int tw, int y0, int x0,
                        int sh, int sw, cudaStream_t stream);
int strip_add(const float* strip, float* acc, int BC, int sh, int sw, int H, int W, int h0, int w0, cudaStream_t stream);

static EpilogueArgs to_args(const b200sr_epilogue* e) {
  EpilogueArgs a;
  a.bias = e->bias;
  a.rowvec = e->rowvec;
  a.rows_per_group = e->rows_per_group;
  a.ld_rowvec = e->ld_rowvec;
  a.residual = e->residual;
  a.ldr = e->ldr;
  a.out = e->out;
  a.ldc = e->ldc;
  a.out_fp32 = e->out_fp32;
  a.geglu = e->geglu;
  a.alpha = e->alpha;
  a.act = e->act;
  a.softmax_valid = e->softmax_valid;
  a.w_dynamic = e->w_dynamic;
  a.w_rows_per_group = e->w_rows_per_group;
  a.w_group_stride = e->w_group_stride;
  a.a_gn_stats = e->a_gn_stats;
  a.a_gn_weight = e->a_gn_weight;
  a.a_gn_bias = e->a_gn_bias;
  a.a_gn_groups = e->a_gn_groups;
  a.a_gn_silu = e->a_gn_silu;
  a.ln_stats = e->ln_stats;
  a.ln_parts = e->ln_parts;
  a.ln_colsum = e->ln_colsum;
  a.ln_shift = e->ln_shift;
  a.ln_eps = e->ln_eps;
  a.ln_stats_out = e->ln_stats_out;
  a.row_softmax = e->row_softmax;
  a.row_softmax_valid = e->row_softmax_valid;
  return a;
}

}

using namespace b200sr;
#define S(s) reinterpret_cast<cudaStream_t>(s)

extern "C" {

int b200sr_abi_version(void) { return 6; }
int b200sr_num_sms(void) {
  int dev = 0, n = 0;
  if (cudaGetDevice(&dev) != cudaSuccess) return B200SR_ENODEV;
  if (cudaDeviceGetAttribute(&n, cudaDevAttrMultiProcessorCount, dev) != cudaSuccess) return B200SR_ENODEV;
  return n;
}

int b200sr_gemm_bf16(const void* A, int64_t lda, const void* W, int32_t M, int32_t N, int32_t K,
                     const b200sr_epilogue* epi, int32_t force_bn, void* stream) {
  if (A == nullptr || W == nullptr || epi == nullptr) return B200SR_EINVAL;
  return gemm_bf16(A, lda, W, M, N, K, to_args(epi), force_bn, S(stream));
}
int b200sr_gemm_n_tile(int32_t M, int32_t N, int32_t K) { return gemm_n_tile(M, N, K); }
int b200sr_conv3x3_bf16(const void* x, const void* w, int32_t N, int32_t H, int32_t W, int32_t Cin, int32_t Cout,
                        int32_t stride, int32_t pad_lo, const b200sr_epilogue* epi, int32_t force_bn, void* stream) {
  if (x == nullptr || w == nullptr || epi == nullptr) return B200SR_EINVAL;
  return conv3x3_bf16(x, w, N, H, W, Cin, Cout, stride, pad_lo, to_args(epi), force_bn, S(stream));
}
int b200sr_pointwise_small(const void* x, const float* w, const float* bias, void* y, int32_t Cin, int32_t Cout,
                           int64_t rows, int32_t HW, int32_t out_nchw_f32, float scale, void* stream) {
  if (x == nullptr || w == nullptr || y == nullptr) return B200SR_EINVAL;
  return pointwise_small(x, w, bias, y, Cin, Cout, rows, HW, out_nchw_f32, scale, S(stream));
}
int b200sr_diag_gaussian(const float* moments, const float* noise, float* z, int32_t N, int32_t C, int32_t HW,
                         float scale, void* stream) {
  if (moments == nullptr || z == nullptr) return B200SR_EINVAL;
  return diag_gaussian(moments, noise, z, N, C, HW, scale, S(stream));
}
int b200sr_conv3x3_small(const void* x, const void* w, const float* bias, const void* addend, void* y, int32_t N,
                         int32_t H, int32_t W, int32_t Cin, int32_t Cout, int32_t out_nchw_f32, void* stream) {
  if (x == nullptr || w == nullptr || y == nullptr) return B200SR_EINVAL;
  return conv3x3_small(x, w, bias, addend, y, N, H, W, Cin, Cout, out_nchw_f32, S(stream));
}
size_t b200sr_group_norm_workspace_bytes(int32_t N, int32_t HW, int32_t C, int32_t groups) {
  if (N <= 0 || HW <= 0 || C < 8 || groups <= 0) return 0;
  return group_norm_workspace_bytes(N, HW, C, groups);
}
int b200sr_group_norm_launches(int32_t N, int32_t HW, int32_t C, int32_t groups) {
  return group_norm_launches(N, HW, C, groups);
}
int b200sr_group_norm_nhwc(const void* x, void* y, const float* weight, const float* bias, int32_t N, int32_t HW,
                           int32_t C, int32_t groups, float eps, int32_t silu, const void* sft_gamma,
                           const void* sft_beta, const void* raw, float control_scale, void* workspace, void* stream) {
  if (x == nullptr || y == nullptr) return B200SR_EINVAL;
  return group_norm_nhwc(x, y, weight, bias, N, HW, C, groups, eps, silu, sft_gamma, sft_beta, raw, control_scale,
                         reinterpret_cast<float*>(workspace), S(stream));
}
int b200sr_group_norm_stats(const void* x, int32_t N, int32_t HW, int32_t C, int32_t groups, float eps, float* stats_out,
                            void* workspace, void* stream) {
  if (x == nullptr) return B200SR_EINVAL;
  return group_norm_stats(x, N, HW, C, groups, eps, stats_out, reinterpret_cast<float*>(workspace), S(stream));
}
int b200sr_layer_norm(const void* x, void* y, const float* weight, const float* bias, int32_t M, int32_t C, float eps,
                      void* stream) {
  if (x == nullptr || y == nullptr) return B200SR_EINVAL;
  return layer_norm(x, y, weight, bias, M, C, eps, S(stream));
}
int b200sr_row_softmax_fold(const float* parts, int32_t n_parts, int64_t rows, float* out, void* stream) {
  return row_softmax_fold(parts, n_parts, rows, out, S(stream));
}
int b200sr_softmax_rows(const float* x, void* y, int32_t rows, int32_t cols, int32_t valid_cols, float scale,
                        void* stream) {
  if (x == nullptr || y == nullptr) return B200SR_EINVAL;
  return softmax_rows(x, y, rows, cols, valid_cols, scale, S(stream));
}
int b200sr_attention_d64(const void* q, int64_t ldq, int32_t q_col, const void* k, int64_t ldk, int32_t k_col,
                         const void* v, int64_t ldv, int32_t v_col, void* out, int64_t ldo, int32_t B, int32_t H,
                         int32_t Nq, int32_t Nk, float scale, int32_t causal, void* workspace, void* stream) {
  if (q == nullptr || k == nullptr || v == nullptr || out == nullptr) return B200SR_EINVAL;
  return attention_d64(q, ldq, q_col, k, ldk, k_col, v, ldv, v_col, out, ldo, B, H, Nq, Nk, scale, causal, workspace,
                       S(stream));
}
int b200sr_embed_tokens(const int64_t* ids, const float* tok, const float* pos, void* out, int32_t B, int32_t T, int32_t C,
                        int32_t vocab, void* stream) {
  if (ids == nullptr || tok == nullptr || pos == nullptr || out == nullptr) return B200SR_EINVAL;
  return embed_tokens(reinterpret_cast<const long long*>(ids), tok, pos, out, B, T, C, vocab, S(stream));
}
size_t b200sr_attention_d64_workspace_bytes(int32_t B, int32_t H, int32_t Nq, int32_t Nk) {
  return attention_d64_workspace_bytes(B, H, Nq, Nk);
}
int b200sr_nchw_f32_to_nhwc_bf16(const float* x, void* y, int32_t N, int32_t C, int32_t HW, float scale, void* stream) {
  if (x == nullptr || y == nullptr) return B200SR_EINVAL;
  return nchw_f32_to_nhwc_bf16(x, y, N, C, HW, scale, S(stream));
}
int b200sr_nhwc_bf16_to_nchw_f32(const void* x, float* y, int32_t N, int32_t C, int32_t HW, void* stream) {
  if (x == nullptr || y == nullptr) return B200SR_EINVAL;
  return nhwc_bf16_to_nchw_f32(x, y, N, C, C, HW, S(stream));
}
int b200sr_nhwc_bf16_to_nchw_f32_strided(const void* x, float* y, int32_t N, int32_t C, int32_t Cs, int32_t HW, void* stream) {
  if (x == nullptr || y == nullptr) return B200SR_EINVAL;
  return nhwc_bf16_to_nchw_f32(x, y, N, C, Cs, HW, S(stream));
}
int b200sr_upsample2x_nhwc(const void* x, void* y, int32_t N, int32_t H, int32_t W, int32_t C, void* stream) {
  if (x == nullptr || y == nullptr) return B200SR_EINVAL;
  return upsample2x_nhwc(x, y, N, H, W, C, S(stream));
}
int b200sr_concat_add(const void* a, int32_t Ca, const void* b, int32_t Cb, const void* c, void* out, int64_t rows,
                      void* stream) {
  if ((a == nullptr && Ca > 0) || b == nullptr || out == nullptr) return B200SR_EINVAL;
  return concat_add(a, Ca, b, Cb, c, out, rows, S(stream));
}
int b200sr_axpy_bf16(const void* a, const void* b, void* y, float alpha, int64_t n, void* stream) {
  if (a == nullptr || b == nullptr || y == nullptr) return B200SR_EINVAL;
  return axpy_bf16(a, b, y, alpha, n, S(stream));
}
int b200sr_pad_channels(const void* x, void* y, int32_t C, int32_t Cpad, int64_t rows, void* stream) {
  if (x == nullptr || y == nullptr) return B200SR_EINVAL;
  return pad_channels(x, y, C, Cpad, rows, S(stream));
}
int b200sr_silu_bf16(const void* x, void* y, int64_t n, void* stream) {
  if (x == nullptr || y == nullptr) return B200SR_EINVAL;
  return silu_bf16(x, y, n, S(stream));
}
int b200sr_sinusoid_embedding(const float* t, void* out, int32_t B, int32_t dim, float max_period, int32_t sin_first,
                              void* stream) {
  if (t == nullptr || out == nullptr) return B200SR_EINVAL;
  return sinusoid_embedding(t, out, B, dim, max_period, sin_first, S(stream));
}
int b200sr_sampler_pre(const float* x, const float* noise, const float* scalars, float* x_hat, void* net_in, int32_t B,
                       int32_t C, int32_t HW, int32_t cfg_copies, void* stream) {
  if (x == nullptr || scalars == nullptr || x_hat == nullptr || net_in == nullptr) return B200SR_EINVAL;
  return sampler_pre(x, noise, scalars, x_hat, net_in, B, C, HW, cfg_copies, S(stream));
}
int b200sr_sampler_post(const float* eps, const float* x_hat, const float* scalars, float* denoised_out, float* x_next,
                        int32_t B, int32_t C, int32_t HW, int32_t use_cfg, void* stream) {
  if (eps == nullptr || x_hat == nullptr || scalars == nullptr || x_next == nullptr) return B200SR_EINVAL;
  return sampler_post(eps, x_hat, scalars, denoised_out, x_next, B, C, HW, use_cfg, S(stream));
}
int b200sr_euler_from_denoised(const float* denoised, const float* x_hat, const float* scalars, float* x_next,
                               int64_t n, void* stream) {
  if (denoised == nullptr || x_hat == nullptr || scalars == nullptr || x_next == nullptr) return B200SR_EINVAL;
  return euler_from_denoised(denoised, x_hat, scalars, x_next, n, S(stream));
}
int b200sr_tile_accumulate(const float* tile, const float* weight, float* acc, float* cnt, int32_t BC, int32_t th,
                           int32_t tw, int32_t H, int32_t W, int32_t h0, int32_t w0, void* stream) {
  if (tile == nullptr || weight == nullptr || acc == nullptr) return B200SR_EINVAL;
  return tile_accumulate(tile, weight, acc, cnt, BC, th, tw, H, W, h0, w0, S(stream));
}
int b200sr_tile_normalize(const float* acc, const float* cnt, float* out, int64_t n, void* stream) {
  if (acc == nullptr || cnt == nullptr || out == nullptr) return B200SR_EINVAL;
  return tile_normalize(acc, cnt, out, n, S(stream));
}
int b200sr_rel_l1_similarity(const void* prev, const void* cur, int64_t n, const float* threshold, void* workspace,
                             float* result, void* stream) {
  if (prev == nullptr || cur == nullptr || threshold == nullptr || workspace == nullptr || result == nullptr)
    return B200SR_EINVAL;
  return rel_l1_similarity(prev, cur, n, threshold, reinterpret_cast<double*>(workspace), result, S(stream));
}
int b200sr_sr3_update(const float* x, const float* eps, const float* noise, const float* scalars, float* out,
                      int64_t n, void* stream) {
  if (x == nullptr || eps == nullptr || scalars == nullptr || out == nullptr) return B200SR_EINVAL;
  return sr3_update(x, eps, noise, scalars, out, n, S(stream));
}

int b200sr_copy_batch(const b200sr_copy* copies, int32_t n, void* stream) {
  if (copies == nullptr || n <= 0 || n > B200SR_MAX_COPIES) return B200SR_EINVAL;
  const void* src[B200SR_MAX_COPIES];
  void* dst[B200SR_MAX_COPIES];
  long long bytes[B200SR_MAX_COPIES];
  for (int i = 0; i < n; ++i) {
    src[i] = copies[i].src;
    dst[i] = copies[i].dst;
    bytes[i] = copies[i].bytes;
  }
  return copy_batch(src, dst, bytes, n, S(stream));
}
int b200sr_tile_weighted_strip(const float* tile, const float* weight, float* strip, int32_t BC, int32_t th, int32_t tw,
                               int32_t y0, int32_t x0, int32_t sh, int32_t sw, void* stream) {
  if (tile == nullptr || weight == nullptr || strip == nullptr) return B200SR_EINVAL;
  return tile_weighted_strip(tile, weight, strip, BC, th, tw, y0, x0, sh, sw, S(stream));
}
int b200sr_strip_add(const float* strip, float* acc, int32_t BC, int32_t sh, int32_t sw, int32_t H, int32_t W,
                     int32_t h0, int32_t w0, void* stream) {
  if (strip == nullptr || acc == nullptr) return B200SR_EINVAL;
  return strip_add(strip, acc, BC, sh, sw, H, W, h0, w0, S(stream));
}

int b200sr_wavelet_level(const float* img, float* low, float* high, int32_t first, int32_t BC, int32_t H, int32_t W,
                         int32_t radius, void* stream) {
  if (img == nullptr || low == nullptr) return B200SR_EINVAL;
  return wavelet_level(img, low, high, first, BC, H, W, radius, S(stream));
}
int b200sr_add_f32(const float* a, const float* b, float* out, int64_t n, void* stream) {
  if (a == nullptr || b == nullptr || out == nullptr) return B200SR_EINVAL;
  return add_f32(a, b, out, n, S(stream));
}
int b200sr_image_to_u8(const float* x, void* out, int32_t C, int32_t H, int32_t W, int32_t OH, int32_t OW, void* stream) {
  if (x == nullptr || out == nullptr) return B200SR_EINVAL;
  return image_to_u8(x, out, C, H, W, OH, OW, S(stream));
}
int b200sr_tensor2img_u8(const float* x, void* out, int32_t C, int32_t H, int32_t W, void* stream) {
  if (x == nullptr || out == nullptr) return B200SR_EINVAL;
  return tensor2img_u8(x, out, C, H, W, S(stream));
}
int b200sr_resample_u8(const void* src, void* dst, int32_t outer, int32_t in_len, int32_t out_len, int32_t inner,
                       const int32_t* bounds, const int32_t* coeffs, int32_t ksize, void* stream) {
  if (src == nullptr || dst == nullptr || bounds == nullptr || coeffs == nullptr) return B200SR_EINVAL;
  return resample_u8(src, dst, outer, in_len, out_len, inner, bounds, coeffs, ksize, S(stream));
}
int b200sr_img_u8_to_tensor(const void* in, float* out, int32_t C, int32_t H, int32_t W, void* stream) {
  if (in == nullptr || out == nullptr) return B200SR_EINVAL;
  return img_u8_to_tensor(in, out, C, H, W, S(stream));
}

}
```

remote-sensing-vision-language-diffusion-model_b200/csrc/common.cuh:

```cuda
#pragma once
#include <cuda.h>
#include <cuda_bf16.h>
#include <cuda_runtime.h>
#include <stdint.h>

#ifndef B200SR_HANG_GUARD
#define B200SR_HANG_GUARD 1
#endif

#define B200SR_MAX_COPIES 8

namespace b200sr {

enum : int {
  B200SR_OK = 0,
  B200SR_EINVAL = -22,
  B200SR_ENODEV = -19,
  B200SR_ELAUNCH = -5,
};

__device__ __forceinline__ uint32_t smem_u32(const void* p) {
  return static_cast<uint32_t>(__cvta_generic_to_shared(p));
}

// ... 32 lines not shown
__device__ __forceinline__ void mbar_wait(uint64_t* bar, uint32_t parity) {
#if B200SR_HANG_GUARD
  long long t0 = 0;
  uint32_t spins = 0;
  while (!mbar_try_wait(bar, parity)) {
    if (++spins == 1024u) t0 = clock64();
    if (spins > 1024u && (spins & 1023u) == 0 && clock64() - t0 > 8000000000LL) __trap();
  }
#else
  while (!mbar_try_wait(bar, parity)) {
  }
#endif
}
__device__ __forceinline__ void fence_barrier_init() {
  asm volatile("fence.mbarrier_init.release.cluster;" ::: "memory");
}
__device__ __forceinline__ void fence_proxy_async_smem() {
  asm volatile("fence.proxy.async.shared::cta;" ::: "memory");
}

__device__ __forceinline__ void tma_prefetch_desc(const CUtensorMap* m) {
  asm volatile("prefetch.tensormap [%0];" ::"l"(reinterpret_cast<uint64_t>(m)) : "memory");
}
__device__ __forceinline__ void tma_load_2d(void* dst, const CUtensorMap* m, uint64_t* bar, int c0, int c1) {
  asm volatile(
      "cp.async.bulk.tensor.2d.shared::cluster.global.tile.mbarrier::complete_tx::bytes [%0], [%1, {%3, %4}], [%2];" ::"r"(
          smem_u32(dst)),
      "l"(reinterpret_cast<uint64_t>(m)), "r"(smem_u32(bar)), "r"(c0), "r"(c1)
      : "memory");
}
__device__ __forceinline__ void tma_load_3d(void* dst, const CUtensorMap* m, uint64_t* bar, int c0, int c1,
                                            int c2) {
  asm volatile(
      "cp.async.bulk.tensor.3d.shared::cluster.global.tile.mbarrier::complete_tx::bytes [%0], [%1, {%3, %4, %5}], [%2];" ::
          "r"(smem_u32(dst)),
      "l"(reinterpret_cast<uint64_t>(m)), "r"(smem_u32(bar)), "r"(c0), "r"(c1), "r"(c2)
      : "memory");
}
__device__ __forceinline__ void tma_load_4d(void* dst, const CUtensorMap* m, uint64_t* bar, int c0, int c1,
                                            int c2, int c3) {
  asm volatile(
      "cp.async.bulk.tensor.4d.shared::cluster.global.tile.mbarrier::complete_tx::bytes [%0], [%1, {%3, %4, %5, %6}], "
      "[%2];" ::"r"(smem_u32(dst)),
      "l"(reinterpret_cast<uint64_t>(m)), "r"(smem_u32(bar)), "r"(c0), "r"(c1), "r"(c2), "r"(c3)
      : "memory");
}
__device__ __forceinline__ void tma_load_5d(void* dst, const CUtensorMap* m, uint64_t* bar, int c0, int c1,
                                            int c2, int c3, int c4) {
  asm volatile(
      "cp.async.bulk.tensor.5d.shared::cluster.global.tile.mbarrier::complete_tx::bytes [%0], [%1, {%3, %4, %5, %6, "
      "%7}], [%2];" ::"r"(smem_u32(dst)),
      "l"(reinterpret_cast<uint64_t>(m)), "r"(smem_u32(bar)), "r"(c0), "r"(c1), "r"(c2), "r"(c3), "r"(c4)
      : "memory");
}

__device__ __forceinline__ float4 lds128(const void* ptr) {
  float4 v;
  asm volatile("ld.shared.v4.f32 {%0, %1, %2, %3}, [%4];" : "=f"(v.x), "=f"(v.y), "=f"(v.z), "=f"(v.w) : "r"(smem_u32(ptr)));
  return v;
}
__device__ __forceinline__ void sts128(void* ptr, float a, float b, float c, float d) {
  asm volatile("st.shared.v4.f32 [%0], {%1, %2, %3, %4};" ::"r"(smem_u32(ptr)), "f"(a), "f"(b), "f"(c), "f"(d) : "memory");
}

__device__ __forceinline__ void ldg256(const void* ptr, uint4& a, uint4& b) {
  asm volatile("ld.global.nc.v8.b32 {%0, %1, %2, %3, %4, %5, %6, %7}, [%8];"
               : "=r"(a.x), "=r"(a.y), "=r"(a.z), "=r"(a.w), "=r"(b.x), "=r"(b.y), "=r"(b.z), "=r"(b.w)
               : "l"(ptr));
}
__device__ __forceinline__ void stg256(void* ptr, const uint4& a, const uint4& b) {
  asm volatile("st.global.v8.b32 [%0], {%1, %2, %3, %4, %5, %6, %7, %8};" ::"l"(ptr), "r"(a.x), "r"(a.y), "r"(a.z), "r"(a.w),
               "r"(b.x), "r"(b.y), "r"(b.z), "r"(b.w)
               : "memory");
}

__device__ __forceinline__ void tma_store_2d(const CUtensorMap* m, const void* src, int c0, int c1) {
  asm volatile("cp.async.bulk.tensor.2d.global.shared::cta.bulk_group [%0, {%2, %3}], [%1];" ::"l"(
                   reinterpret_cast<uint64_t>(m)),
               "r"(smem_u32(src)), "r"(c0), "r"(c1)
               : "memory");
}
__device__ __forceinline__ void tma_store_commit() { asm volatile("cp.async.bulk.commit_group;" ::: "memory"); }
template <int kPending>
__device__ __forceinline__ void tma_store_wait_read() {
  asm volatile("cp.async.bulk.wait_group.read %0;" ::"n"(kPending) : "memory");
}
__device__ __forceinline__ void tma_store_wait_all() { asm volatile("cp.async.bulk.wait_group 0;" ::: "memory"); }

__device__ __forceinline__ void tmem_alloc(uint32_t* dst_smem, uint32_t ncols) {
  asm volatile("tcgen05.alloc.cta_group::1.sync.aligned.shared::cta.b32 [%0], %1;" ::"r"(smem_u32(dst_smem)),
               "r"(ncols)
               : "memory");
}
__device__ __forceinline__ void tmem_relinquish() {
  asm volatile("tcgen05.relinquish_alloc_permit.cta_group::1.sync.aligned;" ::: "memory");
}
__device__ __forceinline__ void tmem_dealloc(uint32_t taddr, uint32_t ncols) {
  asm volatile("tcgen05.dealloc.cta_group::1.sync.aligned.b32 %0, %1;" ::"r"(taddr), "r"(ncols) : "memory");
}
__device__ __forceinline__ void tc_fence_before() {
  asm volatile("tcgen05.fence::before_thread_sync;" ::: "memory");
}
__device__ __forceinline__ void tc_fence_after() {
  asm volatile("tcgen05.fence::after_thread_sync;" ::: "memory");
}
__device__ __forceinline__ void umma_ss(uint32_t d_tmem, uint64_t a_desc, uint64_t b_desc, uint32_t idesc,
                                        uint32_t accumulate) {
  asm volatile(
      "{\n\t.reg .pred p;\n\t"
      "setp.ne.b32 p, %4, 0;\n\t"
      "tcgen05.mma.cta_group::1.kind::f16 [%0], %1, %2, %3, p;\n\t}" ::"r"(d_tmem),
      "l"(a_desc), "l"(b_desc), "r"(idesc), "r"(accumulate)
      : "memory");
}
__device__ __forceinline__ void umma_ts(uint32_t d_tmem, uint32_t a_tmem, uint64_t b_desc, uint32_t idesc,
                                        uint32_t accumulate) {
  asm volatile(
      "{\n\t.reg .pred p;\n\t"
      "setp.ne.b32 p, %4, 0;\n\t"
      "tcgen05.mma.cta_group::1.kind::f16 [%0], [%1], %2, %3, p;\n\t}" ::"r"(d_tmem),
      "r"(a_tmem), "l"(b_desc), "r"(idesc), "r"(accumulate)
      : "memory");
}
__device__ __forceinline__ void umma_commit(uint64_t* bar) {
  asm volatile("tcgen05.commit.cta_group::1.mbarrier::arrive::one.shared::cluster.b64 [%0];" ::"r"(smem_u32(bar))
               : "memory");
}
__device__ __forceinline__ void tmem_ld_wait() { asm volatile("tcgen05.wait::ld.sync.aligned;" ::: "memory"); }
__device__ __forceinline__ void tmem_st_wait() { asm volatile("tcgen05.wait::st.sync.aligned;" ::: "memory"); }

__device__ __forceinline__ void tmem_ld32(uint32_t taddr, uint32_t (&r)[32]) {
  asm volatile(
      "tcgen05.ld.sync.aligned.32x32b.x32.b32 "
      "{%0, %1, %2, %3, %4, %5, %6, %7, %8, %9, %10, %11, %12, %13, %14, %15, "
      "%16, %17, %18, %19, %20, %21, %22, %23, %24, %25, %26, %27, %28, %29, %30, %31}, [%32];"
      : "=r"(r[0]), "=r"(r[1]), "=r"(r[2]), "=r"(r[3]), "=r"(r[4]), "=r"(r[5]), "=r"(r[6]), "=r"(r[7]),
        "=r"(r[8]), "=r"(r[9]), "=r"(r[10]), "=r"(r[11]), "=r"(r[12]), "=r"(r[13]), "=r"(r[14]), "=r"(r[15]),
        "=r"(r[16]), "=r"(r[17]), "=r"(r[18]), "=r"(r[19]), "=r"(r[20]), "=r"(r[21]), "=r"(r[22]), "=r"(r[23]),
        "=r"(r[24]), "=r"(r[25]), "=r"(r[26]), "=r"(r[27]), "=r"(r[28]), "=r"(r[29]), "=r"(r[30]), "=r"(r[31])
      : "r"(taddr)
      : "memory");
}
__device__ __forceinline__ void tmem_ld16(uint32_t taddr, uint32_t (&r)[16]) {
  asm volatile(
      "tcgen05.ld.sync.aligned.32x32b.x16.b32 "
      "{%0, %1, %2, %3, %4, %5, %6, %7, %8, %9, %10, %11, %12, %13, %14, %15}, [%16];"
      : "=r"(r[0]), "=r"(r[1]), "=r"(r[2]), "=r"(r[3]), "=r"(r[4]), "=r"(r[5]), "=r"(r[6]), "=r"(r[7]),
        "=r"(r[8]), "=r"(r[9]), "=r"(r[10]), "=r"(r[11]), "=r"(r[12]), "=r"(r[13]), "=r"(r[14]), "=r"(r[15])
      : "r"(taddr)
      : "memory");
}
__device__ __forceinline__ void tmem_st16(uint32_t taddr, const uint32_t (&r)[16]) {
  asm volatile(
      "tcgen05.st.sync.aligned.32x32b.x16.b32 [%0], "
      "{%1, %2, %3, %4, %5, %6, %7, %8, %9, %10, %11, %12, %13, %14, %15, %16};" ::"r"(taddr),
      "r"(r[0]), "r"(r[1]), "r"(r[2]), "r"(r[3]), "r"(r[4]), "r"(r[5]), "r"(r[6]), "r"(r[7]), "r"(r[8]), "r"(r[9]),
      "r"(r[10]), "r"(r[11]), "r"(r[12]), "r"(r[13]), "r"(r[14]), "r"(r[15])
      : "memory");
}

__device__ __forceinline__ uint64_t umma_smem_desc_sw128(uint32_t smem_addr, uint32_t lbo_bytes,
                                                         uint32_t sbo_bytes) {
  uint64_t d = 0;
  d |= static_cast<uint64_t>((smem_addr & 0x3FFFFu) >> 4);
  d |= static_cast<uint64_t>((lbo_bytes >> 4) & 0x3FFFu) << 16;
  d |= static_cast<uint64_t>((sbo_bytes >> 4) & 0x3FFFu) << 32;
  d |= static_cast<uint64_t>(1) << 46;
  d |= static_cast<uint64_t>(2) << 61;
  return d;
}
__host__ __device__ constexpr uint32_t umma_idesc_bf16_f32(uint32_t m, uint32_t n, uint32_t a_mn_major,
                                                           uint32_t b_mn_major) {
  return (1u << 4)
         | (1u << 7)
         | (1u << 10)
         | (a_mn_major << 15)
         | (b_mn_major << 16)
         | ((n >> 3) << 17)
         | ((m >> 4) << 24);
}

__device__ __forceinline__ void pdl_wait() { asm volatile("griddepcontrol.wait;" ::: "memory"); }
__device__ __forceinline__ void pdl_launch_dependents() { asm volatile("griddepcontrol.launch_dependents;" ::: "memory"); }

__device__ __forceinline__ float silu_f(float x) {
  float e, r;
  asm("ex2.approx.ftz.f32 %0, %1;" : "=f"(e) : "f"(x * -1.4426950408889634f));
  asm("rcp.approx.ftz.f32 %0, %1;" : "=f"(r) : "f"(1.0f + e));
  return x * r;
}
__device__ __forceinline__ float quick_gelu_f(float x) {
  float e, r;
  asm("ex2.approx.ftz.f32 %0, %1;" : "=f"(e) : "f"(x * (-1.702f * 1.4426950408889634f)));
  asm("rcp.approx.ftz.f32 %0, %1;" : "=f"(r) : "f"(1.0f + e));
  return x * r;
}
__device__ __forceinline__ float gelu_erf_f(float x) {
  const float ax = fabsf(x);
  const float t = ax * 0.70710678118654752f;
  float p = fmaf(t, 0.0000430638f, 0.0002765672f);
  p = fmaf(p, t, 0.0001520143f);
  p = fmaf(p, t, 0.0092705272f);
  p = fmaf(p, t, 0.0422820123f);
  p = fmaf(p, t, 0.0705230784f);
  p = fmaf(p, t, 1.0f);
  p = p * p;
  p = p * p;
  p = p * p;
  p = p * p;
  float r;
  asm("rcp.approx.ftz.f32 %0, %1;" : "=f"(r) : "f"(p));
  return 0.5f * fmaf(ax, 1.0f - r, x);
}
__device__ __forceinline__ uint32_t pack_bf16x2(float lo, float hi) {
  __nv_bfloat162 v = __floats2bfloat162_rn(lo, hi);
  return *reinterpret_cast<uint32_t*>(&v);
}
__device__ __forceinline__ float2 unpack_bf16x2(uint32_t u) {
  __nv_bfloat162 v = *reinterpret_cast<__nv_bfloat162*>(&u);
  return __bfloat1622float2(v);
}
__device__ __forceinline__ float warp_sum(float v) {
#pragma unroll
  for (int o = 16; o > 0; o >>= 1) v += __shfl_xor_sync(0xffffffffu, v, o);
  return v;
}
__device__ __forceinline__ float warp_max(float v) {
#pragma unroll
  for (int o = 16; o > 0; o >>= 1) v = fmaxf(v, __shfl_xor_sync(0xffffffffu, v, o));
  return v;
}

typedef CUresult (*PFN_encodeTiled)(CUtensorMap*, CUtensorMapDataType, cuuint32_t, void*, const cuuint64_t*,
                                    const cuuint64_t*, const cuuint32_t*, const cuuint32_t*, CUtensorMapInterleave,
                                    CUtensorMapSwizzle, CUtensorMapL2promotion, CUtensorMapFloatOOBfill);
PFN_encodeTiled get_encode_tiled();
int num_sms();
bool first_use_on_device(bool (&flags)[64]);
bool pdl_enabled();

template <typename... KArgs, typename... Args>
inline cudaError_t launch_k(void (*kernel)(KArgs...), dim3 grid, dim3 block, size_t smem, cudaStream_t stream,
                            int cluster, Args... args) {
  cudaLaunchConfig_t cfg{};
  cfg.gridDim = grid;
  cfg.blockDim = block;
  cfg.dynamicSmemBytes = smem;
  cfg.stream = stream;
  cudaLaunchAttribute attr[2];
  int n = 0;
  if (pdl_enabled()) {
    attr[n].id = cudaLaunchAttributeProgrammaticStreamSerialization;
    attr[n].val.programmaticStreamSerializationAllowed = 1;
    ++n;
  }
  if (cluster > 1) {
    attr[n].id = cudaLaunchAttributeClusterDimension;
    attr[n].val.clusterDim.x = cluster;
    attr[n].val.clusterDim.y = 1;
    attr[n].val.clusterDim.z = 1;
    ++n;
  }
  cfg.attrs = attr;
  cfg.numAttrs = n;
  return cudaLaunchKernelEx(&cfg, kernel, static_cast<KArgs>(args)...);
}

int make_tmap_f32(CUtensorMap* out, const void* base, int rank, const uint64_t* dims, const uint64_t* strides_bytes,
                  const uint32_t* box);
int make_tmap_bf16(CUtensorMap* out, const void* base, int rank, const uint64_t* dims, const uint64_t* strides_bytes,
                   const uint32_t* box, int swizzle_bytes = 128);

struct EpilogueArgs {
  const float* bias;
  const float* rowvec;
  int rows_per_group;
  long long ld_rowvec;
  const void* residual;
  long long ldr;
  void* out;
  long long ldc;
  int out_fp32;
  int geglu;
  float alpha;
  int act;
  int softmax_valid;
  int w_dynamic;
  int w_rows_per_group;
  long long w_group_stride;
  const float* a_gn_stats;
  const float* a_gn_weight;
  const float* a_gn_bias;
  int a_gn_groups, a_gn_silu;
  const float* ln_stats;
  int ln_parts;
  const float* ln_colsum;
  const float* ln_shift;
  float ln_eps;
  float* ln_stats_out;
  int row_softmax;
  int row_softmax_valid;
};

}
```

remote-sensing-vision-language-diffusion-model_b200/csrc/gemm_conv.cu:

```cuda
#include "common.cuh"
#include <cstdlib>

namespace b200sr {

static constexpr int BLOCK_M = 128;
static constexpr int BLOCK_K = 64;
static constexpr int UMMA_K = 16;
static constexpr int A_STAGE_BYTES = BLOCK_M * BLOCK_K * 2;
static constexpr int MAX_STAGES = 8;
static constexpr int KSUB = 2;
static constexpr int HALO_TAPS = 3;
static constexpr int HALO_TILE_W = 8, HALO_TILE_H = 16;
static constexpr int HALO_W = HALO_TILE_W + 2, HALO_H = HALO_TILE_H + 2;
static constexpr int A_HALO_TX_BYTES = HALO_W * HALO_H * BLOCK_K * 2;
static constexpr int A_HALO_BYTES = 23 * 1024;
static constexpr int MAX_A_HALO_STAGES = 4;
static constexpr int MAX_B_STAGES = 16;
static constexpr int BAR_REGION_BYTES = 512;
static constexpr int GEMM_THREADS = 192;
static constexpr int XFORM_WARPS = 6;
static constexpr int GEMM_THREADS_XFORM = GEMM_THREADS + 32 * XFORM_WARPS;
static constexpr int TMEM_COLS = 512;
static constexpr int ACC_STAGE_COLS = 256;

// ... 771 lines not shown
          float v[SOFTMAX_SEG];
#pragma unroll
          for (int j = 0; j < 32; ++j) {
            v[j] = __uint_as_float(a0[j]);
            v[32 + j] = __uint_as_float(a1[j]);
          }
#pragma unroll
          for (int j = 0; j < 16; ++j) v[64 + j] = __uint_as_float(a2[j]);
          if (ln_in) {
#pragma unroll
            for (int j = 0; j < SOFTMAX_SEG; j += 4) {
              const float4 c4 = lds128(s_col + sg * SOFTMAX_SEG + j);
              const float4 b4 = lds128(s_bias + sg * SOFTMAX_SEG + j);
              ln_apply2(v[j], v[j + 1], ln_rstd, ln_nm, c4.x, c4.y, b4.x, b4.y);
              ln_apply2(v[j + 2], v[j + 3], ln_rstd, ln_nm, c4.z, c4.w, b4.z, b4.w);
            }
          }
          float mx = -INFINITY;
#pragma unroll
          for (int j = 0; j < SOFTMAX_SEG; ++j) {
            if (j >= p.softmax_valid) v[j] = -INFINITY;
            mx = fmaxf(mx, v[j]);
          }
          float sum = 0.f;
#pragma unroll
          for (int j = 0; j < SOFTMAX_SEG; ++j) {
            float e;
            asm("ex2.approx.ftz.f32 %0, %1;" : "=f"(e) : "f"(v[j] - mx));
            v[j] = e;
            sum += e;
          }
          const float inv = 1.0f / sum;
          if (valid) {
            uint4* dst = reinterpret_cast<uint4*>(reinterpret_cast<__nv_bfloat16*>(p.out) + row * p.ldc + col0);
#pragma unroll
            for (int q = 0; q < SOFTMAX_SEG / 8; q += 2) {
              uint4 u0, u1;
              u0.x = pack_bf16x2(v[q * 8 + 0] * inv, v[q * 8 + 1] * inv);
              u0.y = pack_bf16x2(v[q * 8 + 2] * inv, v[q * 8 + 3] * inv);
              u0.z = pack_bf16x2(v[q * 8 + 4] * inv, v[q * 8 + 5] * inv);
              u0.w = pack_bf16x2(v[q * 8 + 6] * inv, v[q * 8 + 7] * inv);
              u1.x = pack_bf16x2(v[q * 8 + 8] * inv, v[q * 8 + 9] * inv);
              u1.y = pack_bf16x2(v[q * 8 + 10] * inv, v[q * 8 + 11] * inv);
              u1.z = pack_bf16x2(v[q * 8 + 12] * inv, v[q * 8 + 13] * inv);
              u1.w = pack_bf16x2(v[q * 8 + 14] * inv, v[q * 8 + 15] * inv);
              if (p.wide_io) {
                stg256(dst + q, u0, u1);
              } else {
                dst[q] = u0;
                dst[q + 1] = u1;
              }
            }
          }
        }
      }
      uint32_t a_cur[32];
      if (!kSoftmax) tmem_ld32(t_row, a_cur);
      for (int c = 0; c < (kSoftmax ? 0 : p.BN); c += 32) {
        tmem_ld_wait();
        ET(e_ld, et);
#ifdef B200SR_GEMM_TRACE
        ++e_chunks;
#endif
        const bool more = c + 32 < p.BN;
        if (has_res && c + 32 * kResAhead < p.BN) load_res(res[kResAhead], c + 32 * kResAhead);
        const int col0 = n0 + c;
        float v[32];
        if (kRs) {
          const int left = p.row_softmax_valid - col0;
#pragma unroll
          for (int j = 0; j < 32; ++j) v[j] = j < left ? __uint_as_float(a_cur[j]) * p.alpha : -INFINITY;
        } else {
#pragma unroll
          for (int j = 0; j < 32; j += 4) {
            const float4 b4 = lds128(s_bias + c + j);
            if (ln_in) {
              const float4 c4 = lds128(s_col + c + j);
              v[j] = __uint_as_float(a_cur[j]);
              v[j + 1] = __uint_as_float(a_cur[j + 1]);
              v[j + 2] = __uint_as_float(a_cur[j + 2]);
              v[j + 3] = __uint_as_float(a_cur[j + 3]);
              ln_apply2(v[j], v[j + 1], ln_rstd, ln_nm, c4.x, c4.y, b4.x, b4.y);
              ln_apply2(v[j + 2], v[j + 3], ln_rstd, ln_nm, c4.z, c4.w, b4.z, b4.w);
            } else {
              v[j] = __uint_as_float(a_cur[j]) + b4.x;
              v[j + 1] = __uint_as_float(a_cur[j + 1]) + b4.y;
              v[j + 2] = __uint_as_float(a_cur[j + 2]) + b4.z;
              v[j + 3] = __uint_as_float(a_cur[j + 3]) + b4.w;
            }
          }
        }
        if (more) tmem_ld32(t_row + c + 32, a_cur);
        if (kRs) {
          if (valid && col0 < p.N) {
            if (kRsStats) {
              float cmax = v[0];
#pragma unroll
              for (int j = 1; j < 32; ++j) cmax = fmaxf(cmax, v[j]);
              const float m_new = fmaxf(rs_m, cmax);
              if (m_new > -INFINITY) {
                float s0 = 0.f, s1 = 0.f;
#pragma unroll
                for (int j = 0; j < 32; j += 2) {
                  s0 += ex2_approx_f(v[j] - m_new);
                  s1 += ex2_approx_f(v[j + 1] - m_new);
                }
                rs_l = rs_l * ex2_approx_f(rs_m - m_new) + (s0 + s1);
                rs_m = m_new;
              }
            } else {
              __nv_bfloat16* dst = reinterpret_cast<__nv_bfloat16*>(p.out) + row * p.ldc + col0;
              uint4 uu[4];
#pragma unroll
              for (int q = 0; q < 4; ++q) {
                float e[8];
#pragma unroll
                for (int t = 0; t < 8; ++t) e[t] = ex2_approx_f(v[q * 8 + t] - rs_m) * rs_l;
                uu[q].x = pack_bf16x2(e[0], e[1]);
                uu[q].y = pack_bf16x2(e[2], e[3]);
                uu[q].z = pack_bf16x2(e[4], e[5]);
                uu[q].w = pack_bf16x2(e[6], e[7]);
              }
              if (p.wide_io) {
#pragma unroll
                for (int hq = 0; hq < 2; ++hq)
                  if (col0 + hq * 16 < p.N) stg256(dst + hq * 16, uu[2 * hq], uu[2 * hq + 1]);
              } else {
#pragma unroll
                for (int q = 0; q < 4; ++q)
                  if (col0 + q * 8 < p.N) reinterpret_cast<uint4*>(dst)[q] = uu[q];
              }
            }
          }
        } else if ((valid || epi_tma) && col0 < p.N) {
          if (kGeglu) {
            const long long ocol = col0 >> 1;
            float o[16];
#pragma unroll
            for (int j = 0; j < 16; ++j) o[j] = v[j] * gelu_erf_f(v[16 + j]);
            __nv_bfloat16* dst = reinterpret_cast<__nv_bfloat16*>(p.out) + row * p.ldc + ocol;
            uint4 q0, q1;
            q0.x = pack_bf16x2(o[0], o[1]);
            q0.y = pack_bf16x2(o[2], o[3]);
            q0.z = pack_bf16x2(o[4], o[5]);
            q0.w = pack_bf16x2(o[6], o[7]);
            q1.x = pack_bf16x2(o[8], o[9]);
            q1.y = pack_bf16x2(o[10], o[11]);
            q1.z = pack_bf16x2(o[12], o[13]);
            q1.w = pack_bf16x2(o[14], o[15]);
            if (p.wide_io) {
              stg256(dst, q0, q1);
            } else {
              reinterpret_cast<uint4*>(dst)[0] = q0;
              reinterpret_cast<uint4*>(dst)[1] = q1;
            }
          } else {
            if (p.alpha != 1.0f) {
#pragma unroll
              for (int j = 0; j < 32; ++j) v[j] *= p.alpha;
            }
            if (rv_row != nullptr) {
#pragma unroll
              for (int j = 0; j < 32; j += 4) {
                if (col0 + j < p.N) {
                  const float4 r4 = __ldg(reinterpret_cast<const float4*>(rv_row + c + j));
                  v[j] += r4.x;
                  v[j + 1] += r4.y;
                  v[j + 2] += r4.z;
                  v[j + 3] += r4.w;
                }
              }
            }
            if (has_res) {
#pragma unroll
              for (int q = 0; q < 4; ++q) {
                const float2 f0 = unpack_bf16x2(res[0][q].x), f1 = unpack_bf16x2(res[0][q].y),
                             f2 = unpack_bf16x2(res[0][q].z), f3 = unpack_bf16x2(res[0][q].w);
                v[q * 8 + 0] += f0.x;
                v[q * 8 + 1] += f0.y;
                v[q * 8 + 2] += f1.x;
                v[q * 8 + 3] += f1.y;
                v[q * 8 + 4] += f2.x;
                v[q * 8 + 5] += f2.y;
                v[q * 8 + 6] += f3.x;
                v[q * 8 + 7] += f3.y;
              }
            }
            if (!kExtras) {
            } else if (p.act == 1) {
#pragma unroll
              for (int j = 0; j < 32; ++j) v[j] = silu_f(v[j]);
            } else if (p.act == 2) {
#pragma unroll
              for (int j = 0; j < 32; ++j) v[j] = gelu_erf_f(v[j]);
            } else if (p.act == 3) {
#pragma unroll
              for (int j = 0; j < 32; ++j) v[j] = quick_gelu_f(v[j]);
            }
            ET(e_math, et);
            if (epi_tma) {
              uint8_t* slab = s_out + ((warp - 2) * EPI_SLABS + (slab_i % EPI_SLABS)) * 4096;
              if (lane == 0) tma_store_wait_read<EPI_SLABS - 1>();
              __syncwarp();
#pragma unroll
              for (int q = 0; q < 8; ++q)
                sts128(slab + lane * 128 + ((q ^ (lane & 7)) << 4), v[q * 4], v[q * 4 + 1], v[q * 4 + 2], v[q * 4 + 3]);
              fence_proxy_async_smem();
              __syncwarp();
              if (lane == 0) {
                tma_store_2d(&tmO, slab, col0, m_blk * BLOCK_M + sub * 32);
                tma_store_commit();
              }
              ++slab_i;
            } else if (kF32 && p.out_fp32) {
              float* dst = reinterpret_cast<float*>(p.out) + row * p.ldc + col0;
#pragma unroll
              for (int q = 0; q < 8; ++q) {
                if (col0 + q * 4 < p.N)
                  reinterpret_cast<float4*>(dst)[q] = make_float4(v[q * 4], v[q * 4 + 1], v[q * 4 + 2], v[q * 4 + 3]);
              }
            } else {
              __nv_bfloat16* dst = reinterpret_cast<__nv_bfloat16*>(p.out) + row * p.ldc + col0;
              uint4 uu[4];
#pragma unroll
              for (int q = 0; q < 4; ++q) {
                uu[q].x = pack_bf16x2(v[q * 8 + 0], v[q * 8 + 1]);
                uu[q].y = pack_bf16x2(v[q * 8 + 2], v[q * 8 + 3]);
                uu[q].z = pack_bf16x2(v[q * 8 + 4], v[q * 8 + 5]);
                uu[q].w = pack_bf16x2(v[q * 8 + 6], v[q * 8 + 7]);
              }
              if (p.wide_io) {
#pragma unroll
                for (int hq = 0; hq < 2; ++hq)
                  if (col0 + hq * 16 < p.N) stg256(dst + hq * 16, uu[2 * hq], uu[2 * hq + 1]);
              }
#pragma unroll
              for (int q = 0; q < 4; ++q) {
                if (col0 + q * 8 < p.N) {
                  if (!p.wide_io) reinterpret_cast<uint4*>(dst)[q] = uu[q];
                  if (ln_out) {
#pragma unroll
                    for (int t = 0; t < 8; t += 2) stats_acc2(ln_acc1, ln_acc2, v[q * 8 + t], v[q * 8 + t + 1]);
                  }
                }
              }
            }
          }
        }
        ET(e_st, et);
        if (more) {
#pragma unroll
          for (int d = 0; d < kResAhead; ++d) {
#pragma unroll
            for (int q = 0; q < 4; ++q) res[d][q] = res[d + 1][q];
          }
        }
      }
      if (kRsStats && valid) p.ln_stats_out[static_cast<long long>(n_blk) * p.M + row] = make_float2(rs_m, rs_l);
      if (ln_out && valid)
        p.ln_stats_out[static_cast<long long>(n_blk) * p.M + row] = make_float2(ln_acc1.x + ln_acc1.y, ln_acc2.x + ln_acc2.y);
      if (threadIdx.x == 64) GT(10);
#ifdef B200SR_GEMM_TRACE
      if (threadIdx.x == 64 && p.trace != nullptr) {
        long long* tr = p.trace + blockIdx.x * 32 + 16;
        tr[0] = e_ld; tr[1] = e_math; tr[2] = e_st; tr[3] = e_pro; tr[4] = e_chunks; tr[5] = e_tiles;
      }
#endif
      tc_fence_before();
      __syncwarp();
      if (lane == 0) {
        if (kCluster == 1)
          mbar_arrive(&tmem_empty[acc]);
        else
          mbar_arrive_cluster(mapa_cluster(smem_u32(&tmem_empty[acc]), 0));
      }
      if (++acc == 2) {
        acc = 0;
        acc_phase ^= 1;
      }
    }
  }

  if (kF32 && p.epi_tma != 0 && warp >= 2 && lane == 0) tma_store_wait_all();
  tc_fence_before();
  __syncthreads();
  if (kCluster > 1) cluster_sync_all();
  tc_fence_after();
  if (warp == 1) {
    if (kCluster == 1)
      tmem_dealloc(tmem_base, TMEM_COLS);
    else
      tmem2_dealloc(tmem_base, TMEM_COLS);
  }
#ifdef B200SR_GEMM_TRACE
  if (threadIdx.x == 0 && p.trace != nullptr) {
    long long gt;
    asm volatile("mov.u64 %0, %%globaltimer;" : "=l"(gt));
    p.trace[blockIdx.x * 32 + 13] = gt;
    GT(11);
  }
#endif
}

static int ilog2_exact(int v) {
  int l = 0;
  while ((1 << l) < v) ++l;
  return ((1 << l) == v) ? l : -1;
}

static int pick_bn(int m_blocks, int N, int k_iters, int sms, int cluster) {
  int best = 128;
  double best_cost = 1e30;
  const int slots = sms / cluster;
  const int m_groups = (m_blocks + cluster - 1) / cluster;
  for (int bn = 32; bn <= 256; bn += 32) {
    if (bn > ((N + 31) / 32) * 32 && bn != 32) continue;
    const int n_blocks = (N + bn - 1) / bn;
    const long long work = static_cast<long long>(m_groups) * n_blocks;
    const long long waves = (work + slots - 1) / slots;
    const double mma = 4.0 * (bn / 2.0);
    const double smem = 2.0 * (16384.0 + bn * 128.0 / cluster) / 128.0;
    const double tile_cost = fmax(mma, smem) * k_iters + 2500.0 + bn * 8.0;
    const double cost = waves * tile_cost;
    if (cost < best_cost - 1e-9) {
      best_cost = cost;
      best = bn;
    }
  }
  return best;
}

#ifdef B200SR_GEMM_TRACE
static long long* g_gemm_trace = nullptr;
#endif

template <int kCluster, int kEpi>
static cudaError_t launch_epi(int grid, size_t smem_bytes, cudaStream_t stream, const CUtensorMap& tmA, const CUtensorMap& tmB,
                              const CUtensorMap& tmO, const GemmParams& p) {
  static bool attr_set[64] = {false};
  if (first_use_on_device(attr_set)) {
    const cudaError_t e =
        cudaFuncSetAttribute(gemm_conv_kernel<kCluster, kEpi>, cudaFuncAttributeMaxDynamicSharedMemorySize, 227 * 1024);
    if (e != cudaSuccess) return e;
  }
  return launch_k(gemm_conv_kernel<kCluster, kEpi>, dim3(grid), dim3(kEpi == EPI_XFORM ? GEMM_THREADS_XFORM : GEMM_THREADS),
                  smem_bytes, stream, kCluster, tmA, tmB, tmO, p);
}

template <int kCluster>
static int launch_t(const CUtensorMap& tmA, const CUtensorMap& tmB, const CUtensorMap& tmO, GemmParams& p,
                    cudaStream_t stream) {
  const int xform_bytes = p.gn_stats != nullptr ? ((p.Cin * 8 + 1023) / 1024) * 1024
                          : (p.ln_stats != nullptr && p.row_softmax == 0) ? 4096
                          : p.epi_tma ? 4 * EPI_SLABS * 4096 + 1024
                                      : 0;
  const int smem_budget = 227 * 1024 - 1024  - BAR_REGION_BYTES - 4096  - xform_bytes;
  const int b_sub_bytes = (p.BN / kCluster) * BLOCK_K * 2;
  const int stage_bytes = KSUB * (A_STAGE_BYTES + b_sub_bytes);
  size_t ring_bytes;
  if (p.mode == 3) {
    const int b_stage_bytes = HALO_TAPS * b_sub_bytes;
    p.a_stages = p.kc_per_tap >= 2 ? 2 : 1;
    if (p.gn_stats != nullptr && (smem_budget - 3 * A_HALO_BYTES) / b_stage_bytes >= 3) p.a_stages = 3;
    int stages = (smem_budget - p.a_stages * A_HALO_BYTES) / b_stage_bytes;
    if (stages > MAX_B_STAGES) stages = MAX_B_STAGES;
    if (stages < 2) return B200SR_EINVAL;
    static const bool resident_enabled = [] {
      const char* e = getenv("B200SR_CONV_RESIDENT");
      return e == nullptr || e[0] != '0';
    }();
    p.w_resident = 0;
    if (resident_enabled && p.num_n_blocks == 1 && 3 * p.kc_per_tap <= stages && 3 * p.kc_per_tap <= MAX_B_STAGES) {
      p.w_resident = 1;
      stages = 3 * p.kc_per_tap;
      while (p.a_stages < MAX_A_HALO_STAGES && (smem_budget - (p.a_stages + 1) * A_HALO_BYTES) / b_stage_bytes >= stages)
        ++p.a_stages;
    }
    p.stages = stages;
    ring_bytes = static_cast<size_t>(p.a_stages) * A_HALO_BYTES + static_cast<size_t>(stages) * b_stage_bytes;
  } else {
    const int s_iters = (p.k_iters + KSUB - 1) / KSUB;
    int stages = smem_budget / stage_bytes;
    if (stages > MAX_STAGES) stages = MAX_STAGES;
    if (stages > s_iters + 1) stages = s_iters + 1;
    if (stages < 2) stages = 2;
    p.stages = stages;
    p.a_stages = 0;
    ring_bytes = static_cast<size_t>(stages) * stage_bytes;
  }
  const size_t smem_bytes = ring_bytes + 1024 + BAR_REGION_BYTES + 4096 + xform_bytes;
#ifdef B200SR_GEMM_TRACE
  p.trace = g_gemm_trace;
#endif
  const int work = (p.num_m_blocks / kCluster) * p.num_n_blocks;
  const int slots = num_sms() / kCluster;
  const int grid = (work < slots ? work : slots) * kCluster;
  const bool ln = p.row_softmax == 0 && (p.ln_stats != nullptr || p.ln_stats_out != nullptr);
  cudaError_t err;
  if (p.row_softmax == 1)
    err = launch_epi<kCluster, EPI_RS_STATS>(grid, smem_bytes, stream, tmA, tmB, tmO, p);
  else if (p.row_softmax == 2)
    err = launch_epi<kCluster, EPI_RS_APPLY>(grid, smem_bytes, stream, tmA, tmB, tmO, p);
  else if (p.gn_stats != nullptr)
    err = launch_epi<kCluster, EPI_XFORM>(grid, smem_bytes, stream, tmA, tmB, tmO, p);
  else if (p.softmax_valid > 0)
    err = ln ? launch_epi<kCluster, EPI_LN_SOFTMAX>(grid, smem_bytes, stream, tmA, tmB, tmO, p)
             : launch_epi<kCluster, EPI_SOFTMAX>(grid, smem_bytes, stream, tmA, tmB, tmO, p);
  else if (p.geglu)
    err = ln ? launch_epi<kCluster, EPI_LN_GEGLU>(grid, smem_bytes, stream, tmA, tmB, tmO, p)
             : launch_epi<kCluster, EPI_GEGLU>(grid, smem_bytes, stream, tmA, tmB, tmO, p);
  else if (ln)
    err = launch_epi<kCluster, EPI_LN_PLAIN>(grid, smem_bytes, stream, tmA, tmB, tmO, p);
  else if (p.rowvec != nullptr || p.act != 0 || p.out_fp32)
    err = launch_epi<kCluster, EPI_GENERAL>(grid, smem_bytes, stream, tmA, tmB, tmO, p);
  else
    err = launch_epi<kCluster, EPI_PLAIN>(grid, smem_bytes, stream, tmA, tmB, tmO, p);
  return err == cudaSuccess ? B200SR_OK : B200SR_ELAUNCH;
}

static int fill_epilogue(GemmParams& p, const EpilogueArgs& e) {
  p.bias = e.bias;
  p.rowvec = e.rowvec;
  p.rows_per_group = e.rows_per_group;
  p.ld_rowvec = e.ld_rowvec != 0 ? e.ld_rowvec : p.N;
  if (e.rowvec != nullptr && ((p.ld_rowvec % 4) != 0 || p.ld_rowvec < p.N)) return B200SR_EINVAL;
  p.residual = reinterpret_cast<const __nv_bfloat16*>(e.residual);
  p.ldr = e.ldr;
  p.out = e.out;
  p.ldc = e.ldc;
  p.out_fp32 = e.out_fp32;
  p.geglu = e.geglu;
  p.alpha = e.alpha;
  p.act = e.act;
  p.softmax_valid = e.softmax_valid;
  p.w_dynamic = e.w_dynamic;
  p.w_rows_per_group = e.w_rows_per_group;
  p.w_group_stride = e.w_group_stride;
  p.gn_stats = e.a_gn_stats;
  p.gn_weight = e.a_gn_weight;
  p.gn_bias = e.a_gn_bias;
  p.gn_groups = e.a_gn_groups;
  p.gn_silu = e.a_gn_silu;
  p.ln_stats = reinterpret_cast<const float2*>(e.ln_stats);
  p.ln_parts = e.ln_parts;
  p.ln_colsum = e.ln_colsum;
  p.ln_shift = e.ln_shift;
  p.ln_eps = e.ln_eps;
  p.ln_stats_out = reinterpret_cast<float2*>(e.ln_stats_out);
  p.row_softmax = e.row_softmax;
  p.row_softmax_valid = e.row_softmax_valid > 0 ? e.row_softmax_valid : p.N;
  if (e.row_softmax != 0) {
    if (p.mode != 0 || e.row_softmax < 0 || e.row_softmax > 2 || e.geglu || e.out_fp32 || e.residual != nullptr ||
        e.rowvec != nullptr || e.bias != nullptr || e.act != 0 || e.softmax_valid != 0 || e.a_gn_stats != nullptr ||
        e.ln_colsum != nullptr || e.ln_shift != nullptr)
      return B200SR_EINVAL;
    if (e.row_softmax == 1 && (e.ln_stats_out == nullptr || e.ln_stats != nullptr)) return B200SR_EINVAL;
    if (e.row_softmax == 2 && (e.ln_stats == nullptr || e.ln_parts <= 0 || e.ln_stats_out != nullptr || e.out == nullptr))
      return B200SR_EINVAL;
    if ((p.N % 8) != 0 || (e.row_softmax == 2 && (e.ldc % 8) != 0)) return B200SR_EINVAL;
    p.out = e.out;
    p.ldc = e.ldc;
    p.alpha = e.alpha;
    p.w_dynamic = e.w_dynamic;
    return B200SR_OK;
  }
  if (e.ln_stats != nullptr &&
      (p.mode != 0 || e.ln_parts <= 0 || e.ln_colsum == nullptr || e.ln_shift == nullptr || e.a_gn_stats != nullptr))
    return B200SR_EINVAL;
  if (e.ln_stats_out != nullptr && (p.mode != 0 || e.geglu || e.softmax_valid > 0)) return B200SR_EINVAL;
  if ((e.ln_stats != nullptr || e.ln_stats_out != nullptr) && (e.out_fp32 || e.rowvec != nullptr || e.act != 0))
    return B200SR_EINVAL;
  if (e.a_gn_stats != nullptr) {
    if (p.mode != 3 || e.a_gn_weight == nullptr || e.a_gn_bias == nullptr || e.a_gn_groups <= 0 ||
        (p.Cin % e.a_gn_groups) != 0)
      return B200SR_EINVAL;
  }
  if (e.softmax_valid < 0 || e.softmax_valid > SOFTMAX_SEG) return B200SR_EINVAL;
  if (e.softmax_valid > 0 && (e.geglu || e.out_fp32 || e.residual != nullptr || e.rowvec != nullptr || e.bias != nullptr ||
                              e.act != 0 || (p.N % SOFTMAX_SEG) != 0))
    return B200SR_EINVAL;
  if (e.w_rows_per_group < 0 || (e.w_rows_per_group % (2 * BLOCK_M)) != 0) return B200SR_EINVAL;
  if (e.geglu && e.act) return B200SR_EINVAL;
  if (e.act < 0 || e.act > 3) return B200SR_EINVAL;
  if (e.out == nullptr) return B200SR_EINVAL;
  if (e.geglu && (e.out_fp32 || e.residual != nullptr || e.rowvec != nullptr || (p.N % 32) != 0)) return B200SR_EINVAL;
  if (p.N % 8 != 0) return B200SR_EINVAL;
  if ((e.ldc % 8) != 0 || (e.residual != nullptr && (e.ldr % 8) != 0)) return B200SR_EINVAL;
  return B200SR_OK;
}

static int finish(const CUtensorMap& tmA, const void* W, GemmParams& p, int real_m_blocks, int force_bn,
                  cudaStream_t stream) {
  const int cluster = real_m_blocks >= 2 ? 2 : 1;
  p.num_m_blocks = ((real_m_blocks + cluster - 1) / cluster) * cluster;
  p.BN = force_bn > 0 ? force_bn : pick_bn(real_m_blocks, p.N, p.k_iters, num_sms(), cluster);
  if (p.softmax_valid > 0) p.BN = p.N >= 3 * SOFTMAX_SEG ? 3 * SOFTMAX_SEG : p.N;
  if (p.mode == 3 && cluster == 1 && p.BN > 192 && force_bn <= 0) p.BN = 192;
  if (p.BN % (p.softmax_valid > 0 ? 16 : 32) != 0 || p.BN > 256 || p.BN <= 0) return B200SR_EINVAL;
  p.num_n_blocks = (p.N + p.BN - 1) / p.BN;
  CUtensorMap tmB;
  const long long w_rows = p.w_rows_per_group > 0
                               ? ((static_cast<long long>(p.M) + p.w_rows_per_group - 1) / p.w_rows_per_group - 1) *
                                         p.w_group_stride + p.N
                               : p.N;
  uint64_t dims[2] = {static_cast<uint64_t>(p.K), static_cast<uint64_t>(w_rows)};
  uint64_t strides[1] = {static_cast<uint64_t>(p.K) * 2};
  uint32_t box[2] = {BLOCK_K, static_cast<uint32_t>(p.BN / cluster)};
  int rc = make_tmap_bf16(&tmB, W, 2, dims, strides, box);
  if (rc) return rc;
  static const bool epi_tma_enabled = [] {
    const char* e = getenv("B200SR_EPI_TMA");
    return e == nullptr || e[0] != '0';
  }();
  {
    const long long n_out = p.geglu ? p.N / 2 : p.N;
    const long long esz = p.out_fp32 ? 4 : 2;
    p.wide_io = !p.out_fp32 && (n_out % 16) == 0 && (p.ldc * esz) % 32 == 0 && (reinterpret_cast<uintptr_t>(p.out) & 31) == 0 &&
                (p.residual == nullptr || ((p.ldr * 2) % 32 == 0 && (reinterpret_cast<uintptr_t>(p.residual) & 31) == 0));
    static const bool wide_enabled = [] {
      const char* e = getenv("B200SR_WIDE_IO");
      return e == nullptr || e[0] != '0';
    }();
    if (!wide_enabled) p.wide_io = 0;
  }
  CUtensorMap tmO = tmA;
  p.epi_tma = 0;
  if (epi_tma_enabled && p.mode == 0 && p.out_fp32 && !p.geglu && p.softmax_valid <= 0 && p.ln_stats == nullptr &&
      p.ln_stats_out == nullptr && p.residual == nullptr && p.rowvec == nullptr && (p.ldc % 4) == 0 &&
      static_cast<long long>(p.num_m_blocks / cluster) * p.num_n_blocks >= 2LL * (num_sms() / cluster)) {
    uint64_t odims[2] = {static_cast<uint64_t>(p.N), static_cast<uint64_t>(p.M)};
    uint64_t ostrides[1] = {static_cast<uint64_t>(p.ldc) * 4};
    uint32_t obox[2] = {32, 32};
    if (make_tmap_f32(&tmO, p.out, 2, odims, ostrides, obox) == B200SR_OK) p.epi_tma = 1;
  }
  return cluster == 2 ? launch_t<2>(tmA, tmB, tmO, p, stream) : launch_t<1>(tmA, tmB, tmO, p, stream);
}

int gemm_n_tile(int M, int N, int K) {
  if (M <= 0 || N <= 0 || K <= 0) return 0;
  const int m_blocks = (M + BLOCK_M - 1) / BLOCK_M;
  return pick_bn(m_blocks, N, (K + BLOCK_K - 1) / BLOCK_K, num_sms(), m_blocks >= 2 ? 2 : 1);
}

int gemm_bf16(const void* A, long long lda, const void* W, int M, int N, int K, const EpilogueArgs& e, int force_bn,
              cudaStream_t stream) {
  if (M <= 0 || N <= 0 || K <= 0 || (K % 8) != 0 || (lda % 8) != 0) return B200SR_EINVAL;
  GemmParams p{};
  p.mode = 0;
  p.M = M;
  p.N = N;
  p.K = K;
  p.k_iters = (K + BLOCK_K - 1) / BLOCK_K;
  int rc = fill_epilogue(p, e);
  if (rc) return rc;
  CUtensorMap tmA;
  uint64_t dims[2] = {static_cast<uint64_t>(K), static_cast<uint64_t>(M)};
  uint64_t strides[1] = {static_cast<uint64_t>(lda) * 2};
  uint32_t box[2] = {BLOCK_K, BLOCK_M};
  rc = make_tmap_bf16(&tmA, A, 2, dims, strides, box);
  if (rc) return rc;
  return finish(tmA, W, p, (M + BLOCK_M - 1) / BLOCK_M, force_bn, stream);
}

int conv3x3_bf16(const void* x, const void* w, int NB, int H, int W, int Cin, int Cout, int stride, int pad_lo,
                 const EpilogueArgs& e, int force_bn, cudaStream_t stream) {
  if (NB <= 0 || H <= 0 || W <= 0 || Cin <= 0 || (Cin % BLOCK_K) != 0 || Cout <= 0) return B200SR_EINVAL;
  if (stride != 1 && stride != 2) return B200SR_EINVAL;
  if (pad_lo != 1 && !(pad_lo == 0 && stride == 2)) return B200SR_EINVAL;
  if (stride == 2 && ((H | W) & 1)) return B200SR_EINVAL;
  if (e.geglu) return B200SR_EINVAL;
  const int OH = H / stride, OW = W / stride;
  int bw = 1;
  while (bw * 2 <= 128 && (OW % (bw * 2)) == 0) bw *= 2;
  int bh = 1;
  while (bw * bh * 2 <= 128 && bh < OH) bh *= 2;
  int bn = 128 / (bw * bh);
  static const bool halo_enabled = [] {
    const char* e = getenv("B200SR_CONV_HALO");
    return e == nullptr || e[0] != '0';
  }();
  const bool halo = halo_enabled && stride == 1 && (W % HALO_TILE_W) == 0 && H >= HALO_TILE_H;
  if (halo) {
    bw = HALO_TILE_W;
    bh = HALO_TILE_H;
    bn = 1;
  }
  GemmParams p{};
  p.mode = halo ? 3 : (stride == 1 ? 1 : 2);
  p.NB = NB;
  p.OH = OH;
  p.OW = OW;
  p.Cin = Cin;
  p.pad_lo = pad_lo;
  p.M = NB * OH * OW;
  p.N = Cout;
  p.K = 9 * Cin;
  p.bw_log2 = ilog2_exact(bw);
  p.bh_log2 = ilog2_exact(bh);
  p.bn_log2 = ilog2_exact(bn);
  p.tiles_w = OW / bw;
  p.tiles_h = (OH + bh - 1) / bh;
  p.tiles_n = (NB + bn - 1) / bn;
  p.kc_per_tap = Cin / BLOCK_K;
  p.k_iters = 9 * p.kc_per_tap;
  int rc = fill_epilogue(p, e);
  if (rc) return rc;
  CUtensorMap tmA;
  if (stride == 1) {
    uint64_t dims[4] = {static_cast<uint64_t>(Cin), static_cast<uint64_t>(W), static_cast<uint64_t>(H),
                        static_cast<uint64_t>(NB)};
    uint64_t strides[3] = {static_cast<uint64_t>(Cin) * 2, static_cast<uint64_t>(W) * Cin * 2,
                           static_cast<uint64_t>(H) * W * Cin * 2};
    uint32_t box[4] = {BLOCK_K, static_cast<uint32_t>(bw), static_cast<uint32_t>(bh), static_cast<uint32_t>(bn)};
    if (halo) {
      box[1] = HALO_W;
      box[2] = HALO_H;
    }
    rc = make_tmap_bf16(&tmA, x, 4, dims, strides, box);
  } else {
    uint64_t dims[5] = {static_cast<uint64_t>(2 * Cin), static_cast<uint64_t>(W / 2), 2,
                        static_cast<uint64_t>(H / 2), static_cast<uint64_t>(NB)};
    uint64_t strides[4] = {static_cast<uint64_t>(2 * Cin) * 2, static_cast<uint64_t>(W) * Cin * 2,
                           static_cast<uint64_t>(2) * W * Cin * 2, static_cast<uint64_t>(H) * W * Cin * 2};
    uint32_t box[5] = {BLOCK_K, static_cast<uint32_t>(bw), 1, static_cast<uint32_t>(bh), static_cast<uint32_t>(bn)};
    rc = make_tmap_bf16(&tmA, x, 5, dims, strides, box);
  }
  if (rc) return rc;
  return finish(tmA, w, p, p.tiles_w * p.tiles_h * p.tiles_n, force_bn, stream);
}

}

#ifdef B200SR_GEMM_TRACE
extern "C" void b200sr_debug_set_gemm_trace(void* p) { b200sr::g_gemm_trace = reinterpret_cast<long long*>(p); }
#endif
```

Measured before the change: 37.95.

## Fuse transformer block GEMMs into a persistent dependency-tracked chain kernel

Adds a persistent tcgen05 GEMM chain kernel that runs up to five dependent GEMMs of a transformer block (attn1 out-proj, folded cross-attention K and V, GEGLU, FF out) in one launch. Tiles of later GEMMs wait on per-m-group global ready counters published by earlier GEMMs' epilogues. This removes separate kernel launches and tail idle time between the GEMMs so their tiles can overlap. The price is spin-waiting on counters, possible load imbalance, and added complexity in counter reset and grid sizing.

```diff
diff --git a/include/b200sr.h b/include/b200sr.h
--- a/include/b200sr.h
+++ b/include/b200sr.h
@@ -45,6 +45,16 @@
 
 int b200sr_gemm_bf16(const void* A, int64_t lda, const void* W, int32_t M, int32_t N, int32_t K,
                      const b200sr_epilogue* epi, int32_t force_bn, void* stream);
+
+typedef struct b200sr_chain_gemm {
+  const void* A;
+  int64_t lda;
+  const void* W;
+  int32_t M, N, K;
+  b200sr_epilogue epi;
+} b200sr_chain_gemm;
+int b200sr_gemm_chain(const b200sr_chain_gemm* gemms, int32_t n, void* workspace, void* stream);
+size_t b200sr_gemm_chain_workspace_bytes(int32_t M);
 
 int b200sr_gemm_n_tile(int32_t M, int32_t N, int32_t K);
 
diff --git a/remote-sensing-vision-language-diffusion-model_b200/b200sr/_lib.py b/remote-sensing-vision-language-diffusion-model_b200/b200sr/_lib.py
--- a/remote-sensing-vision-language-diffusion-model_b200/b200sr/_lib.py
+++ b/remote-sensing-vision-language-diffusion-model_b200/b200sr/_lib.py
@@ -6,7 +6,7 @@
 _HERE = os.path.dirname(os.path.abspath(__file__))
 LIB_PATH = os.path.join(_HERE, os.environ.get("B200SR_LIB", "libb200sr.so"))
 
-ABI_VERSION = 6
+ABI_VERSION = 7
 
 c_void_p, c_int, c_i64, c_float, c_size_t = C.c_void_p, C.c_int32, C.c_int64, C.c_float, C.c_size_t
 
@@ -46,15 +46,28 @@
     ]
 
 
+class ChainGemm(C.Structure):
+
+    _fields_ = [
+        ("A", c_void_p),
+        ("lda", c_i64),
+        ("W", c_void_p),
+        ("M", c_int),
+        ("N", c_int),
+        ("K", c_int),
+        ("epi", Epilogue),
+    ]
+
+
 class Copy(C.Structure):
 
     _fields_ = [("src", c_void_p), ("dst", c_void_p), ("bytes", c_i64)]
 
 
 def binding_snippet() -> str:
-    names = {c_void_p: "C.c_void_p", c_int: "C.c_int32", c_i64: "C.c_int64", c_float: "C.c_float"}
+    names = {c_void_p: "C.c_void_p", c_int: "C.c_int32", c_i64: "C.c_int64", c_float: "C.c_float", Epilogue: "Epilogue"}
     out = []
-    for cls, cname in ((Epilogue, "b200sr_epilogue"), (Copy, "b200sr_copy")):
+    for cls, cname in ((Epilogue, "b200sr_epilogue"), (ChainGemm, "b200sr_chain_gemm"), (Copy, "b200sr_copy")):
         out.append(f"class {cls.__name__}(C.Structure):  # {cname} (ABI version {ABI_VERSION})")
         out.append("    _fields_ = [")
         for fname, ftype in cls._fields_:
@@ -70,6 +83,8 @@
     "b200sr_num_sms": (c_int, []),
     "b200sr_gemm_bf16": (c_int, [P, c_i64, P, c_int, c_int, c_int, C.POINTER(Epilogue), c_int, P]),
     "b200sr_gemm_n_tile": (c_int, [c_int, c_int, c_int]),
+    "b200sr_gemm_chain": (c_int, [C.POINTER(ChainGemm), c_int, P, P]),
+    "b200sr_gemm_chain_workspace_bytes": (c_size_t, [c_int]),
     "b200sr_row_softmax_fold": (c_int, [P, c_int, c_i64, P, P]),
     "b200sr_conv3x3_bf16": (c_int, [P, P, c_int, c_int, c_int, c_int, c_int, c_int, c_int, C.POINTER(Epilogue), c_int, P]),
     "b200sr_pointwise_small": (c_int, [P, P, P, P, c_int, c_int, c_i64, c_int, c_int, c_float, P]),
diff --git a/remote-sensing-vision-language-diffusion-model_b200/b200sr/modules.py b/remote-sensing-vision-language-diffusion-model_b200/b200sr/modules.py
--- a/remote-sensing-vision-language-diffusion-model_b200/b200sr/modules.py
+++ b/remote-sensing-vision-language-diffusion-model_b200/b200sr/modules.py
@@ -143,9 +143,14 @@
     return _conv3x3(holder, name, conv, _gn(norm, x_nhwc, silu=True), **kw)
 
 
-def _linear(holder: Packed, name: str, lin, x: torch.Tensor, **kw) -> torch.Tensor:
+def _linear_operands(holder: Packed, name: str, lin):
     w = holder._pk(name + ".w", (lin.weight,), ops.pack_linear)
     b = holder._pk(name + ".b", (lin.bias,), _F32) if lin.bias is not None else None
+    return w, b
+
+
+def _linear(holder: Packed, name: str, lin, x: torch.Tensor, **kw) -> torch.Tensor:
+    w, b = _linear_operands(holder, name, lin)
     return ops.gemm(x, w, b, **kw)
 
 
@@ -228,11 +233,13 @@
         super().__init__()
         self.proj = nn.Linear(dim_in, dim_out * 2)
 
+    def ln_operands(self, norm: nn.LayerNorm):
+        return self._pk("proj_ln", (self.proj.weight, self.proj.bias, norm.weight, norm.bias), ops.pack_geglu_ln)
+
     def forward(self, x, ln=None):
         if ln is not None:
             norm, stats = ln
-            w, colsum, shift = self._pk("proj_ln", (self.proj.weight, self.proj.bias, norm.weight, norm.bias),
-                                        ops.pack_geglu_ln)
+            w, colsum, shift = self.ln_operands(norm)
             return ops.gemm(tokens_bf16(x), w, None, geglu=True, ln=(stats, colsum, shift, norm.eps))
         w, b = self._pk("proj", (self.proj.weight, self.proj.bias), ops.pack_geglu)
         return ops.gemm(tokens_bf16(x), w, b, geglu=True)
@@ -249,6 +256,9 @@
 
     def forward(self, x, residual: Optional[torch.Tensor] = None, ln=None, want_stats: bool = False):
         return _linear(self, "out", self.net[2], self.net[0](x, ln=ln), residual=residual, want_stats=want_stats)
+
+    def out_operands(self):
+        return _linear_operands(self, "out", self.net[2])
 
 
 class CrossAttention(nn.Module, Packed):
@@ -292,6 +302,18 @@
                 raise ValueError(f"context batch {kv.shape[0]} does not divide the query batch {q.shape[0]}")
             kv = kv.repeat_interleave(q.shape[0] // kv.shape[0], dim=0)
         return ops.attention(q, kv, kv, self.heads, q_col=0, k_col=0, v_col=inner, scale=self.scale)
+
+    def out_operands(self):
+        return _linear_operands(self, "out", self.to_out[0])
+
+    def folded_ln(self, x, context, norm: nn.LayerNorm):
+        if context is None or x.dim() != 3 or x.shape[1] % 256 != 0 or norm is not self._fold_norm():
+            return None
+        bound = self._bound_entry(tokens_bf16(context))
+        if bound is None or bound[2] is None or len(bound[2]) != 5 or x.shape[0] % bound[2][0].shape[0] != 0:
+            return None
+        k_fold, v_fold, tk, colsum, shift = bound[2]
+        return k_fold, v_fold, int(tk), colsum, shift, x.shape[1] * (x.shape[0] // k_fold.shape[0])
 
     def _wkv(self):
         return self._pk("kv", (self.to_k.weight, self.to_v.weight), lambda k, v: torch.cat([k, v], 0).to(bf16).contiguous())
@@ -425,6 +447,10 @@
     def forward(self, x, context=None, additional_tokens=None, n_times_crossframe_attn_in_self=0, stats=None,
                 want_stats: bool = False):
         x = tokens_bf16(x)
+        chain = stats is not None and not self.disable_self_attn and x.is_cuda
+        fold = self.attn2.folded_ln(x, context, self.norm2) if chain else None
+        if fold is not None:
+            return self._forward_chain(x, stats, fold, want_stats)
         if stats is None:
             x = self.attn1(self._ln(self.norm1, x), context=context if self.disable_self_attn else None, residual=x)
             x = self.attn2(self._ln(self.norm2, x), context=context, residual=x)
@@ -433,6 +459,21 @@
                               ln=(self.norm1, stats), want_stats=True)
         x, stats = self.attn2(x, context=context, residual=x, ln=(self.norm2, stats), want_stats=True)
         return self.ff(x, residual=x, ln=(self.norm3, stats), want_stats=want_stats)
+
+    def _forward_chain(self, x, stats, fold, want_stats: bool):
+        k_fold, v_fold, tk, colsum2, shift2, rpg = fold
+        h = self.attn1.attend(x, None, None, ln=(self.norm1, stats))
+        wo, bo = self.attn1.out_operands()
+        wg, cg, sg = self.ff.net[0].ln_operands(self.norm3)
+        wf, bf = self.ff.out_operands()
+        return ops.gemm_chain([
+            dict(a=h, w=wo, bias=bo, residual=x, want_stats=True),
+            dict(a=0, w=k_fold, softmax_valid=tk, w_rows_per_group=rpg, ln=(0, colsum2, shift2, self.norm2.eps)),
+            dict(a=1, w=v_fold, bias=self.attn2.out_operands()[1], residual=0, w_rows_per_group=rpg,
+                 want_stats=True),
+            dict(a=2, w=wg, geglu=True, ln=(2, cg, sg, self.norm3.eps)),
+            dict(a=3, w=wf, bias=bf, residual=2, want_stats=want_stats),
+        ])[4]
 
 
 class SpatialTransformer(nn.Module, Packed):
diff --git a/remote-sensing-vision-language-diffusion-model_b200/b200sr/ops.py b/remote-sensing-vision-language-diffusion-model_b200/b200sr/ops.py
--- a/remote-sensing-vision-language-diffusion-model_b200/b200sr/ops.py
+++ b/remote-sensing-vision-language-diffusion-model_b200/b200sr/ops.py
@@ -256,6 +256,77 @@
     return (out, stats) if want_stats else out
 
 
+def gemm_chain(steps):
+    n = len(steps)
+    if not 1 <= n <= 5:
+        raise _lib.B200SRError(f"gemm_chain: {n} GEMMs (1 to 5)")
+    descs = (_lib.ChainGemm * n)()
+    results, keep = [], []
+    M = None
+    flops = 0.0
+    for i, s in enumerate(steps):
+        a = s["a"]
+        a = results[a][0] if isinstance(a, int) else a
+        w = s["w"]
+        _req(w, bf16, "gemm_chain.w")
+        if a.dtype != bf16 or not a.is_cuda:
+            raise _lib.B200SRError("gemm_chain.a: expected CUDA bf16")
+        K, N = a.shape[-1], w.shape[-2]
+        geglu = bool(s.get("geglu", False))
+        rpg = int(s.get("w_rows_per_group", 0))
+        a2 = a.reshape(-1, K)
+        if a2.stride(-1) != 1:
+            a2 = a2.contiguous()
+        if M is None:
+            M = a2.shape[0]
+        n_out = N // 2 if geglu else N
+        out = torch.empty(*a.shape[:-1], n_out, dtype=bf16, device=a.device)
+        residual = s.get("residual")
+        residual = results[residual][0] if isinstance(residual, int) else residual
+        ldr = 0
+        if residual is not None:
+            r2 = residual if residual.dim() == 2 else residual.reshape(-1, residual.shape[-1])
+            assert r2.dtype == bf16 and r2.stride(-1) == 1
+            ldr = r2.stride(0)
+        if rpg:
+            assert w.dim() == 3 and w.is_contiguous() and w.shape[0] * rpg >= M
+        e = _epilogue(out, n_out, s.get("bias"), None, 0, residual, ldr, False, geglu, s.get("alpha", 1.0), 0,
+                      s.get("softmax_valid", 0), rpg, N if rpg else 0)
+        ln = s.get("ln")
+        if ln is not None:
+            st, colsum, shift, eps = ln
+            st = results[st][1] if isinstance(st, int) else st
+            groups = w.shape[0] if rpg else 1
+            if st.buf.shape[1] != a2.shape[0] or st.dim != K:
+                raise _lib.B200SRError(f"gemm_chain.ln: statistics of a [{st.buf.shape[1]}, {st.dim}] matrix, a is "
+                                       f"[{a2.shape[0]}, {K}]")
+            for t, nme in ((colsum, "colsum"), (shift, "shift")):
+                _req(t, torch.float32, f"gemm_chain.ln.{nme}")
+                if t.numel() != groups * N:
+                    raise _lib.B200SRError(f"gemm_chain.ln.{nme}: expected [{groups}, {N}]")
+            e.ln_stats, e.ln_parts, e.ln_colsum, e.ln_shift, e.ln_eps = st.buf.data_ptr(), st.parts, \
+                colsum.data_ptr(), shift.data_ptr(), float(eps)
+            keep.append(st)
+        stats = None
+        if s.get("want_stats", False):
+            if geglu or s.get("softmax_valid", 0):
+                raise _lib.B200SRError("gemm_chain.want_stats: plain bf16 output only")
+            parts = -(-N // gemm_n_tile(a2.shape[0], N, K))
+            stats = RowStats(torch.empty(parts, a2.shape[0], 2, dtype=torch.float32, device=a.device), parts, N)
+            e.ln_stats_out = stats.buf.data_ptr()
+        d = descs[i]
+        d.A, d.lda, d.W, d.M, d.N, d.K, d.epi = a2.data_ptr(), a2.stride(0), w.data_ptr(), a2.shape[0], N, K, e
+        keep.append(a2)
+        results.append((out, stats))
+        flops += 2.0 * a2.shape[0] * N * K
+    lib = _lib.load()
+    ws = _workspace(results[0][0].device, lib.b200sr_gemm_chain_workspace_bytes(M), kind="chain")
+    with _Timed("gemm", flops, f"chain M{M} " + " ".join(f"N{d.N} K{d.K}" for d in descs)):
+        rc = lib.b200sr_gemm_chain(descs, n, ws.data_ptr(), _stream())
+    check(rc, f"gemm_chain M={M} n={n}")
+    return [(o, st) if s.get("want_stats", False) else o for (o, st), s in zip(results, steps)]
+
+
 def conv3x3(
     x: torch.Tensor,
     w: torch.Tensor,
diff --git a/remote-sensing-vision-language-diffusion-model_b200/csrc/capi.cu b/remote-sensing-vision-language-diffusion-model_b200/csrc/capi.cu
--- a/remote-sensing-vision-language-diffusion-model_b200/csrc/capi.cu
+++ b/remote-sensing-vision-language-diffusion-model_b200/csrc/capi.cu
@@ -92,6 +92,8 @@
 int conv3x3_bf16(const void* x, const void* w, int NB, int H, int W, int Cin, int Cout, int stride, int pad_lo,
                  const EpilogueArgs& e, int force_bn, cudaStream_t stream);
 int gemm_n_tile(int M, int N, int K);
+int gemm_chain(const ChainGemmArgs* g, int n, unsigned int* counters, cudaStream_t stream);
+size_t gemm_chain_workspace_bytes(int M);
 int pointwise_small(const void* x, const float* w, const float* bias, void* y, int Cin, int Cout, long long rows, int HW,
                     int out_nchw_f32, float scale, cudaStream_t stream);
 int diag_gaussian(const float* moments, const float* noise, float* z, int N, int C, int HW, float scale,
@@ -192,7 +194,7 @@
 
 extern "C" {
 
-int b200sr_abi_version(void) { return 6; }
+int b200sr_abi_version(void) { return 7; }
 int b200sr_num_sms(void) {
   int dev = 0, n = 0;
   if (cudaGetDevice(&dev) != cudaSuccess) return B200SR_ENODEV;
@@ -206,6 +208,21 @@
   return gemm_bf16(A, lda, W, M, N, K, to_args(epi), force_bn, S(stream));
 }
 int b200sr_gemm_n_tile(int32_t M, int32_t N, int32_t K) { return gemm_n_tile(M, N, K); }
+int b200sr_gemm_chain(const b200sr_chain_gemm* gemms, int32_t n, void* workspace, void* stream) {
+  if (gemms == nullptr || workspace == nullptr || n < 1 || n > 5) return B200SR_EINVAL;
+  ChainGemmArgs g[5];
+  for (int i = 0; i < n; ++i) {
+    g[i].A = gemms[i].A;
+    g[i].lda = gemms[i].lda;
+    g[i].W = gemms[i].W;
+    g[i].M = gemms[i].M;
+    g[i].N = gemms[i].N;
+    g[i].K = gemms[i].K;
+    g[i].e = to_args(&gemms[i].epi);
+  }
+  return gemm_chain(g, n, static_cast<unsigned int*>(workspace), S(stream));
+}
+size_t b200sr_gemm_chain_workspace_bytes(int32_t M) { return gemm_chain_workspace_bytes(M); }
 int b200sr_conv3x3_bf16(const void* x, const void* w, int32_t N, int32_t H, int32_t W, int32_t Cin, int32_t Cout,
                         int32_t stride, int32_t pad_lo, const b200sr_epilogue* epi, int32_t force_bn, void* stream) {
   if (x == nullptr || w == nullptr || epi == nullptr) return B200SR_EINVAL;
diff --git a/remote-sensing-vision-language-diffusion-model_b200/csrc/common.cuh b/remote-sensing-vision-language-diffusion-model_b200/csrc/common.cuh
--- a/remote-sensing-vision-language-diffusion-model_b200/csrc/common.cuh
+++ b/remote-sensing-vision-language-diffusion-model_b200/csrc/common.cuh
@@ -358,4 +358,12 @@
   int row_softmax_valid;
 };
 
-}
+struct ChainGemmArgs {
+  const void* A;
+  long long lda;
+  const void* W;
+  int M, N, K;
+  EpilogueArgs e;
+};
+
+}
diff --git a/remote-sensing-vision-language-diffusion-model_b200/csrc/gemm_conv.cu b/remote-sensing-vision-language-diffusion-model_b200/csrc/gemm_conv.cu
--- a/remote-sensing-vision-language-diffusion-model_b200/csrc/gemm_conv.cu
+++ b/remote-sensing-vision-language-diffusion-model_b200/csrc/gemm_conv.cu
@@ -1097,6 +1097,611 @@
 #endif
 }
 
+static constexpr int CHAIN_MAX_GEMMS = 5;
+static constexpr int CHAIN_CLAIM_SLOTS = 4;
+static constexpr int CHAIN_CLAIM_READERS = 10;
+static constexpr int CHAIN_READY0 = 2;
+#ifdef B200SR_CHAIN_WARP_PUBLISH
+static constexpr unsigned int CHAIN_TILE_ARRIVALS = 8;
+#else
+static constexpr unsigned int CHAIN_TILE_ARRIVALS = 2;
+#endif
+
+struct ChainGemm {
+  GemmParams p;
+  int family;
+  int tile0;
+};
+
+struct ChainParams {
+  CUtensorMap tmA[CHAIN_MAX_GEMMS];
+  CUtensorMap tmB[CHAIN_MAX_GEMMS];
+  ChainGemm g[CHAIN_MAX_GEMMS];
+  int n_gemms;
+  int m_groups;
+  int num_tiles;
+  int stages;
+  int b_sub_stride;
+  unsigned int* counters;
+};
+
+__device__ __forceinline__ bool mbar_try_wait_cluster(uint64_t* bar, uint32_t parity) {
+  uint32_t ok;
+  asm volatile(
+      "{\n\t.reg .pred p;\n\t"
+      "mbarrier.try_wait.parity.acquire.cluster.shared::cta.b64 p, [%1], %2;\n\t"
+      "selp.u32 %0, 1, 0, p;\n\t}"
+      : "=r"(ok)
+      : "r"(smem_u32(bar)), "r"(parity)
+      : "memory");
+  return ok != 0;
+}
+__device__ __forceinline__ void mbar_wait_cluster(uint64_t* bar, uint32_t parity) {
+  long long t0 = 0;
+  uint32_t spins = 0;
+  while (!mbar_try_wait_cluster(bar, parity)) {
+    if (++spins == 1024u) t0 = clock64();
+    if (spins > 1024u && (spins & 1023u) == 0 && clock64() - t0 > 8000000000LL) __trap();
+  }
+}
+__device__ __forceinline__ void st_cluster_s32(uint32_t cluster_addr, int v) {
+  asm volatile("st.shared::cluster.s32 [%0], %1;" ::"r"(cluster_addr), "r"(v) : "memory");
+}
+__device__ __forceinline__ unsigned int ld_acquire_gpu(const unsigned int* p) {
+  unsigned int v;
+  asm volatile("ld.acquire.gpu.global.u32 %0, [%1];" : "=r"(v) : "l"(p) : "memory");
+  return v;
+}
+__device__ __forceinline__ void chain_wait_ready(const unsigned int* c, unsigned int target) {
+  if (ld_acquire_gpu(c) >= target) return;
+  const long long t0 = clock64();
+  unsigned int ns = 32;
+  while (ld_acquire_gpu(c) < target) {
+    __nanosleep(ns);
+    if (ns < 512) ns *= 2;
+    if (clock64() - t0 > 4000000000LL) __trap();
+  }
+}
+
+template <int kFam>
+__device__ __forceinline__ void chain_epilogue(const GemmParams& p, int m_blk, int n_blk, int lane, int r, uint32_t t_row,
+                                               float* s_bias, float* s_col, int& bias_key, int key, uint64_t* tmem_full_bar,
+                                               uint32_t acc_phase) {
+  constexpr bool kSoftmax = kFam == EPI_LN_SOFTMAX;
+  constexpr bool kGeglu = kFam == EPI_LN_GEGLU;
+  constexpr bool kTail = kFam == EPI_LN_PLAIN;
+  constexpr int kResAhead = 2;
+  const int n0 = n_blk * p.BN;
+  const long long row = static_cast<long long>(m_blk) * BLOCK_M + r;
+  const bool valid = row < p.M;
+  __syncwarp();
+  const bool ln_in = p.ln_stats != nullptr;
+  const bool ln_out = kTail && p.ln_stats_out != nullptr;
+  const bool has_res = kTail && p.residual != nullptr && valid;
+  const __nv_bfloat16* res_row = has_res ? p.residual + row * p.ldr + n0 : nullptr;
+  uint4 res[kResAhead + 1][4];
+  auto load_res = [&](uint4 (&dst)[4], int cc) {
+    if (p.wide_io) {
+#pragma unroll
+      for (int hq = 0; hq < 2; ++hq) {
+        if (n0 + cc + hq * 16 < p.N)
+          ldg256(res_row + cc + hq * 16, dst[2 * hq], dst[2 * hq + 1]);
+        else
+          dst[2 * hq] = dst[2 * hq + 1] = make_uint4(0, 0, 0, 0);
+      }
+    } else {
+#pragma unroll
+      for (int q = 0; q < 4; ++q)
+        dst[q] = (n0 + cc + q * 8 < p.N) ? __ldg(reinterpret_cast<const uint4*>(res_row + cc) + q) : make_uint4(0, 0, 0, 0);
+    }
+  };
+  float ln_rstd = 1.f, ln_nm = 0.f;
+  if (!ln_in) {
+    if (key != bias_key) {
+      for (int j = lane; j < p.BN; j += 32) s_bias[j] = (p.bias != nullptr && n0 + j < p.N) ? __ldg(p.bias + n0 + j) : 0.f;
+      bias_key = key;
+    }
+    __syncwarp();
+    if (has_res) {
+#pragma unroll
+      for (int d = 0; d < kResAhead; ++d)
+        if (d * 32 < p.BN) load_res(res[d], d * 32);
+    }
+  } else {
+    const long long wg = p.w_rows_per_group > 0 ? (static_cast<long long>(m_blk) * BLOCK_M / p.w_rows_per_group) * p.N : 0;
+    float bb[8], cc[8];
+#pragma unroll
+    for (int i = 0; i < 8; ++i) {
+      const int j = lane + 32 * i;
+      const bool in = j < p.BN && n0 + j < p.N;
+      bb[i] = (in && p.bias != nullptr) ? __ldg(p.bias + n0 + j) : 0.f;
+      cc[i] = in ? __ldg(p.ln_colsum + wg + n0 + j) : 0.f;
+      bb[i] += in ? __ldg(p.ln_shift + wg + n0 + j) : 0.f;
+    }
+    float s1 = 0.f, s2 = 0.f;
+    if (valid) {
+      for (int q = 0; q < p.ln_parts; ++q) {
+        const float2 t = __ldg(p.ln_stats + static_cast<long long>(q) * p.M + row);
+        s1 += t.x;
+        s2 += t.y;
+      }
+    }
+    if (has_res) {
+#pragma unroll
+      for (int d = 0; d < kResAhead; ++d)
+        if (d * 32 < p.BN) load_res(res[d], d * 32);
+    }
+#pragma unroll
+    for (int i = 0; i < 8; ++i) {
+      const int j = lane + 32 * i;
+      if (j < p.BN) {
+        s_bias[j] = bb[i];
+        s_col[j] = cc[i];
+      }
+    }
+    bias_key = -1;
+    __syncwarp();
+    const float inv_k = 1.0f / static_cast<float>(p.K);
+    const float mean = s1 * inv_k;
+    const float var = fmaxf(s2 * inv_k - mean * mean, 0.f);
+    ln_rstd = rsqrtf(var + p.ln_eps);
+    ln_nm = -mean * ln_rstd;
+  }
+  float2 ln_acc1 = make_float2(0.f, 0.f), ln_acc2 = make_float2(0.f, 0.f);
+  mbar_wait(tmem_full_bar, acc_phase);
+  tc_fence_after();
+  if (kSoftmax) {
+    for (int sg = 0; sg * SOFTMAX_SEG < p.BN; ++sg) {
+      const int col0 = n0 + sg * SOFTMAX_SEG;
+      if (col0 >= p.N) break;
+      uint32_t a0[32], a1[32], a2[16];
+      tmem_ld32(t_row + sg * SOFTMAX_SEG, a0);
+      tmem_ld32(t_row + sg * SOFTMAX_SEG + 32, a1);
+      tmem_ld16(t_row + sg * SOFTMAX_SEG + 64, a2);
+      tmem_ld_wait();
+      float v[SOFTMAX_SEG];
+#pragma unroll
+      for (int j = 0; j < 32; ++j) {
+        v[j] = __uint_as_float(a0[j]);
+        v[32 + j] = __uint_as_float(a1[j]);
+      }
+#pragma unroll
+      for (int j = 0; j < 16; ++j) v[64 + j] = __uint_as_float(a2[j]);
+      if (ln_in) {
+#pragma unroll
+        for (int j = 0; j < SOFTMAX_SEG; j += 4) {
+          const float4 c4 = lds128(s_col + sg * SOFTMAX_SEG + j);
+          const float4 b4 = lds128(s_bias + sg * SOFTMAX_SEG + j);
+          ln_apply2(v[j], v[j + 1], ln_rstd, ln_nm, c4.x, c4.y, b4.x, b4.y);
+          ln_apply2(v[j + 2], v[j + 3], ln_rstd, ln_nm, c4.z, c4.w, b4.z, b4.w);
+        }
+      }
+      float mx = -INFINITY;
+#pragma unroll
+      for (int j = 0; j < SOFTMAX_SEG; ++j) {
+        if (j >= p.softmax_valid) v[j] = -INFINITY;
+        mx = fmaxf(mx, v[j]);
+      }
+      float sum = 0.f;
+#pragma unroll
+      for (int j = 0; j < SOFTMAX_SEG; ++j) {
+        float e;
+        asm("ex2.approx.ftz.f32 %0, %1;" : "=f"(e) : "f"(v[j] - mx));
+        v[j] = e;
+        sum += e;
+      }
+      const float inv = 1.0f / sum;
+      if (valid) {
+        uint4* dst = reinterpret_cast<uint4*>(reinterpret_cast<__nv_bfloat16*>(p.out) + row * p.ldc + col0);
+#pragma unroll
+        for (int q = 0; q < SOFTMAX_SEG / 8; q += 2) {
+          uint4 u0, u1;
+          u0.x = pack_bf16x2(v[q * 8 + 0] * inv, v[q * 8 + 1] * inv);
+          u0.y = pack_bf16x2(v[q * 8 + 2] * inv, v[q * 8 + 3] * inv);
+          u0.z = pack_bf16x2(v[q * 8 + 4] * inv, v[q * 8 + 5] * inv);
+          u0.w = pack_bf16x2(v[q * 8 + 6] * inv, v[q * 8 + 7] * inv);
+          u1.x = pack_bf16x2(v[q * 8 + 8] * inv, v[q * 8 + 9] * inv);
+          u1.y = pack_bf16x2(v[q * 8 + 10] * inv, v[q * 8 + 11] * inv);
+          u1.z = pack_bf16x2(v[q * 8 + 12] * inv, v[q * 8 + 13] * inv);
+          u1.w = pack_bf16x2(v[q * 8 + 14] * inv, v[q * 8 + 15] * inv);
+          if (p.wide_io) {
+            stg256(dst + q, u0, u1);
+          } else {
+            dst[q] = u0;
+            dst[q + 1] = u1;
+          }
+        }
+      }
+    }
+  } else {
+    uint32_t a_cur[32];
+    tmem_ld32(t_row, a_cur);
+    for (int c = 0; c < p.BN; c += 32) {
+      tmem_ld_wait();
+      const bool more = c + 32 < p.BN;
+      if (has_res && c + 32 * kResAhead < p.BN) load_res(res[kResAhead], c + 32 * kResAhead);
+      const int col0 = n0 + c;
+      float v[32];
+#pragma unroll
+      for (int j = 0; j < 32; j += 4) {
+        const float4 b4 = lds128(s_bias + c + j);
+        if (ln_in) {
+          const float4 c4 = lds128(s_col + c + j);
+          v[j] = __uint_as_float(a_cur[j]);
+          v[j + 1] = __uint_as_float(a_cur[j + 1]);
+          v[j + 2] = __uint_as_float(a_cur[j + 2]);
+          v[j + 3] = __uint_as_float(a_cur[j + 3]);
+          ln_apply2(v[j], v[j + 1], ln_rstd, ln_nm, c4.x, c4.y, b4.x, b4.y);
+          ln_apply2(v[j + 2], v[j + 3], ln_rstd, ln_nm, c4.z, c4.w, b4.z, b4.w);
+        } else {
+          v[j] = __uint_as_float(a_cur[j]) + b4.x;
+          v[j + 1] = __uint_as_float(a_cur[j + 1]) + b4.y;
+          v[j + 2] = __uint_as_float(a_cur[j + 2]) + b4.z;
+          v[j + 3] = __uint_as_float(a_cur[j + 3]) + b4.w;
+        }
+      }
+      if (more) tmem_ld32(t_row + c + 32, a_cur);
+      if (valid && col0 < p.N) {
+        if (kGeglu) {
+          const long long ocol = col0 >> 1;
+          float o[16];
+#pragma unroll
+          for (int j = 0; j < 16; ++j) o[j] = v[j] * gelu_erf_f(v[16 + j]);
+          __nv_bfloat16* dst = reinterpret_cast<__nv_bfloat16*>(p.out) + row * p.ldc + ocol;
+          uint4 q0, q1;
+          q0.x = pack_bf16x2(o[0], o[1]);
+          q0.y = pack_bf16x2(o[2], o[3]);
+          q0.z = pack_bf16x2(o[4], o[5]);
+          q0.w = pack_bf16x2(o[6], o[7]);
+          q1.x = pack_bf16x2(o[8], o[9]);
+          q1.y = pack_bf16x2(o[10], o[11]);
+          q1.z = pack_bf16x2(o[12], o[13]);
+          q1.w = pack_bf16x2(o[14], o[15]);
+          if (p.wide_io) {
+            stg256(dst, q0, q1);
+          } else {
+            reinterpret_cast<uint4*>(dst)[0] = q0;
+            reinterpret_cast<uint4*>(dst)[1] = q1;
+          }
+        } else {
+          if (p.alpha != 1.0f) {
+#pragma unroll
+            for (int j = 0; j < 32; ++j) v[j] *= p.alpha;
+          }
+          if (has_res) {
+#pragma unroll
+            for (int q = 0; q < 4; ++q) {
+              const float2 f0 = unpack_bf16x2(res[0][q].x), f1 = unpack_bf16x2(res[0][q].y),
+                           f2 = unpack_bf16x2(res[0][q].z), f3 = unpack_bf16x2(res[0][q].w);
+              v[q * 8 + 0] += f0.x;
+              v[q * 8 + 1] += f0.y;
+              v[q * 8 + 2] += f1.x;
+              v[q * 8 + 3] += f1.y;
+              v[q * 8 + 4] += f2.x;
+              v[q * 8 + 5] += f2.y;
+              v[q * 8 + 6] += f3.x;
+              v[q * 8 + 7] += f3.y;
+            }
+          }
+          __nv_bfloat16* dst = reinterpret_cast<__nv_bfloat16*>(p.out) + row * p.ldc + col0;
+          uint4 uu[4];
+#pragma unroll
+          for (int q = 0; q < 4; ++q) {
+            uu[q].x = pack_bf16x2(v[q * 8 + 0], v[q * 8 + 1]);
+            uu[q].y = pack_bf16x2(v[q * 8 + 2], v[q * 8 + 3]);
+            uu[q].z = pack_bf16x2(v[q * 8 + 4], v[q * 8 + 5]);
+            uu[q].w = pack_bf16x2(v[q * 8 + 6], v[q * 8 + 7]);
+          }
+          if (p.wide_io) {
+#pragma unroll
+            for (int hq = 0; hq < 2; ++hq)
+              if (col0 + hq * 16 < p.N) stg256(dst + hq * 16, uu[2 * hq], uu[2 * hq + 1]);
+          }
+#pragma unroll
+          for (int q = 0; q < 4; ++q) {
+            if (col0 + q * 8 < p.N) {
+              if (!p.wide_io) reinterpret_cast<uint4*>(dst)[q] = uu[q];
+              if (ln_out) {
+#pragma unroll
+                for (int t = 0; t < 8; t += 2) stats_acc2(ln_acc1, ln_acc2, v[q * 8 + t], v[q * 8 + t + 1]);
+              }
+            }
+          }
+        }
+      }
+      if (more) {
+#pragma unroll
+        for (int d = 0; d < kResAhead; ++d) {
+#pragma unroll
+          for (int q = 0; q < 4; ++q) res[d][q] = res[d + 1][q];
+        }
+      }
+    }
+  }
+  if (ln_out && valid)
+    p.ln_stats_out[static_cast<long long>(n_blk) * p.M + row] = make_float2(ln_acc1.x + ln_acc1.y, ln_acc2.x + ln_acc2.y);
+}
+
+__global__ void __launch_bounds__(GEMM_THREADS, 1) gemm_chain_kernel(const __grid_constant__ ChainParams cp) {
+  extern __shared__ __align__(1024) uint8_t smem_raw[];
+  uint8_t* smem = reinterpret_cast<uint8_t*>((reinterpret_cast<uintptr_t>(smem_raw) + 1023) & ~uintptr_t(1023));
+  const int warp = threadIdx.x >> 5;
+  const int lane = threadIdx.x & 31;
+  const int stage_bytes = KSUB * (A_STAGE_BYTES + cp.b_sub_stride);
+  const int stages = cp.stages;
+  const uint32_t rank = cluster_ctarank();
+  const bool leader = rank == 0;
+  const int ring_bytes = stages * stage_bytes;
+  uint64_t* full_bar = reinterpret_cast<uint64_t*>(smem + ring_bytes);
+  uint64_t* empty_bar = full_bar + MAX_STAGES;
+  uint64_t* tmem_full = empty_bar + MAX_STAGES;
+  uint64_t* tmem_empty = tmem_full + 2;
+  uint64_t* claim_full = tmem_empty + 2;
+  uint64_t* claim_empty = claim_full + CHAIN_CLAIM_SLOTS;
+  int* claim_tile = reinterpret_cast<int*>(claim_empty + CHAIN_CLAIM_SLOTS);
+  uint32_t* tmem_base_slot = reinterpret_cast<uint32_t*>(claim_tile + CHAIN_CLAIM_SLOTS);
+  float* s_epi = reinterpret_cast<float*>(smem + ring_bytes + BAR_REGION_BYTES);
+  float* s_colsum = s_epi + 4 * 256;
+
+  if (warp == 0 && lane == 0) {
+    for (int i = 0; i < cp.n_gemms; ++i) {
+      tma_prefetch_desc(&cp.tmA[i]);
+      tma_prefetch_desc(&cp.tmB[i]);
+    }
+    for (int s = 0; s < stages; ++s) {
+      mbar_init(&full_bar[s], 1);
+      mbar_init(&empty_bar[s], 1);
+    }
+    for (int s = 0; s < 2; ++s) {
+      mbar_init(&tmem_full[s], 1);
+      mbar_init(&tmem_empty[s], 8);
+    }
+    for (int s = 0; s < CHAIN_CLAIM_SLOTS; ++s) {
+      mbar_init(&claim_full[s], 1);
+      mbar_init(&claim_empty[s], CHAIN_CLAIM_READERS);
+    }
+    fence_barrier_init();
+  }
+  if (warp == 1) {
+    tmem2_alloc(tmem_base_slot, TMEM_COLS);
+    tmem2_relinquish();
+  }
+  tc_fence_before();
+  __syncthreads();
+  cluster_sync_all();
+  tc_fence_after();
+  const uint32_t tmem_base = *tmem_base_slot;
+  pdl_launch_dependents();
+
+  int cs = 0;
+  uint32_t cph = 0;
+  auto read_claim = [&]() -> int {
+    if (leader)
+      mbar_wait(&claim_full[cs], cph);
+    else
+      mbar_wait_cluster(&claim_full[cs], cph);
+    return *reinterpret_cast<volatile int*>(&claim_tile[cs]);
+  };
+  auto release_claim = [&]() {
+    if (leader)
+      mbar_arrive(&claim_empty[cs]);
+    else
+      mbar_arrive_cluster(mapa_cluster(smem_u32(&claim_empty[cs]), 0));
+    if (++cs == CHAIN_CLAIM_SLOTS) {
+      cs = 0;
+      cph ^= 1;
+    }
+  };
+  auto gemm_of = [&](int tile) {
+    int i = 0;
+    while (i + 1 < cp.n_gemms && tile >= cp.g[i + 1].tile0) ++i;
+    return i;
+  };
+  const unsigned int* ready = cp.counters + CHAIN_READY0;
+
+  if (warp == 0) {
+    if (lane == 0) {
+      pdl_wait();
+      int stage = 0;
+      uint32_t phase = 0;
+      for (;;) {
+        int tile;
+        if (leader) {
+          mbar_wait(&claim_empty[cs], cph ^ 1);
+          const unsigned int t = atomicAdd(cp.counters, 1u);
+          tile = t < static_cast<unsigned int>(cp.num_tiles) ? static_cast<int>(t) : -1;
+          claim_tile[cs] = tile;
+          st_cluster_s32(mapa_cluster(smem_u32(&claim_tile[cs]), 1), tile);
+          mbar_arrive(&claim_full[cs]);
+          mbar_arrive_cluster(mapa_cluster(smem_u32(&claim_full[cs]), 1));
+          if (++cs == CHAIN_CLAIM_SLOTS) {
+            cs = 0;
+            cph ^= 1;
+          }
+        } else {
+          tile = read_claim();
+          release_claim();
+        }
+        if (tile < 0) break;
+        const int gi = gemm_of(tile);
+        const GemmParams& p = cp.g[gi].p;
+        const int local = tile - cp.g[gi].tile0;
+        const int mg = local / p.num_n_blocks;
+        const int n_blk = local - mg * p.num_n_blocks;
+        const int m_blk = mg * 2 + static_cast<int>(rank);
+        const int b_rows = p.BN / 2;
+        const uint32_t sub_tx = static_cast<uint32_t>(A_STAGE_BYTES + b_rows * BLOCK_K * 2) * 2;
+        int n0 = n_blk * p.BN + static_cast<int>(rank) * b_rows;
+        if (p.w_rows_per_group > 0)
+          n0 += static_cast<int>((static_cast<long long>(m_blk) * BLOCK_M / p.w_rows_per_group) * p.w_group_stride);
+        const int s_iters = (p.k_iters + KSUB - 1) / KSUB;
+        const unsigned int* dep = gi > 0 ? ready + (gi - 1) * cp.m_groups + mg : nullptr;
+        const unsigned int dep_target = gi > 0 ? CHAIN_TILE_ARRIVALS * cp.g[gi - 1].p.num_n_blocks : 0u;
+        const bool dep_ready = dep == nullptr || ld_acquire_gpu(dep) >= dep_target;
+        const int pre = dep_ready ? 0 : (s_iters < stages ? s_iters : stages);
+        auto load_w = [&](int st, int sit) {
+          const int nsub = p.k_iters - sit * KSUB < KSUB ? p.k_iters - sit * KSUB : KSUB;
+          if (leader) mbar_expect_tx(&full_bar[st], sub_tx * nsub);
+          const uint32_t bar = mapa_cluster(smem_u32(&full_bar[st]), 0);
+          for (int j = 0; j < nsub; ++j)
+            tma2_load_2d(smem + st * stage_bytes + KSUB * A_STAGE_BYTES + j * cp.b_sub_stride, &cp.tmB[gi], bar,
+                         (sit * KSUB + j) * BLOCK_K, n0);
+        };
+        int st = stage;
+        uint32_t ph = phase;
+        for (int it = 0; it < pre; ++it) {
+          mbar_wait(&empty_bar[st], ph ^ 1);
+          load_w(st, it);
+          if (++st == stages) {
+            st = 0;
+            ph ^= 1;
+          }
+        }
+        if (gi > 0) {
+          if (!dep_ready) chain_wait_ready(dep, dep_target);
+          asm volatile("fence.proxy.async.global;" ::: "memory");
+        }
+        st = stage;
+        ph = phase;
+        for (int it = 0; it < s_iters; ++it) {
+          if (it >= pre) {
+            mbar_wait(&empty_bar[st], ph ^ 1);
+            load_w(st, it);
+          }
+          const int nsub = p.k_iters - it * KSUB < KSUB ? p.k_iters - it * KSUB : KSUB;
+          const uint32_t bar = mapa_cluster(smem_u32(&full_bar[st]), 0);
+          for (int j = 0; j < nsub; ++j)
+            tma2_load_2d(smem + st * stage_bytes + j * A_STAGE_BYTES, &cp.tmA[gi], bar, (it * KSUB + j) * BLOCK_K,
+                         m_blk * BLOCK_M);
+          if (++st == stages) {
+            st = 0;
+            ph ^= 1;
+          }
+        }
+        stage = st;
+        phase = ph;
+      }
+    }
+  } else if (warp == 1) {
+    if (lane == 0 && leader) {
+      int stage = 0;
+      uint32_t phase = 0;
+      int acc = 0;
+      uint32_t acc_phase = 0;
+      bool ready_next = false;
+      for (;;) {
+        const int tile = read_claim();
+        release_claim();
+        if (tile < 0) break;
+        const GemmParams& p = cp.g[gemm_of(tile)].p;
+        const uint32_t idesc = umma_idesc_bf16_f32(BLOCK_M * 2, static_cast<uint32_t>(p.BN), 0, 0);
+        mbar_wait(&tmem_empty[acc], acc_phase ^ 1);
+        tc_fence_after();
+        const uint32_t d_tmem = tmem_base + acc * ACC_STAGE_COLS;
+        const int s_iters = (p.k_iters + KSUB - 1) / KSUB;
+        for (int it = 0; it < s_iters; ++it) {
+          const int nsub = p.k_iters - it * KSUB < KSUB ? p.k_iters - it * KSUB : KSUB;
+          if (!ready_next) mbar_wait(&full_bar[stage], phase);
+          tc_fence_after();
+          {
+            const int ns = stage + 1 == stages ? 0 : stage + 1;
+            ready_next = mbar_test_wait(&full_bar[ns], ns == 0 ? phase ^ 1 : phase);
+          }
+          const uint32_t sa0 = smem_u32(smem + stage * stage_bytes);
+          const uint32_t sb0 = sa0 + KSUB * A_STAGE_BYTES;
+          for (int j = 0; j < nsub; ++j) {
+            const uint64_t adesc = umma_smem_desc_sw128(sa0 + j * A_STAGE_BYTES, 16, 1024);
+            const uint64_t bdesc = umma_smem_desc_sw128(sb0 + j * cp.b_sub_stride, 16, 1024);
+#pragma unroll
+            for (int k = 0; k < BLOCK_K / UMMA_K; ++k)
+              umma2_ss(d_tmem, adesc + 2 * k, bdesc + 2 * k, idesc, (it | j | k) != 0);
+          }
+          umma2_commit_mc(&empty_bar[stage], 3);
+          if (++stage == stages) {
+            stage = 0;
+            phase ^= 1;
+          }
+        }
+        umma2_commit_mc(&tmem_full[acc], 3);
+        if (++acc == 2) {
+          acc = 0;
+          acc_phase ^= 1;
+        }
+      }
+    }
+  } else {
+    const int sub = warp & 3;
+    const int r = sub * 32 + lane;
+    float* s_bias = s_epi + (warp - 2) * 256;
+    float* s_col = s_colsum + (warp - 2) * 256;
+    int bias_key = -1;
+    int acc = 0;
+    uint32_t acc_phase = 0;
+    pdl_wait();
+    for (;;) {
+      const int tile = read_claim();
+      __syncwarp();
+      if (lane == 0) release_claim();
+      else if (++cs == CHAIN_CLAIM_SLOTS) {
+        cs = 0;
+        cph ^= 1;
+      }
+      if (tile < 0) break;
+      const int gi = gemm_of(tile);
+      const ChainGemm& G = cp.g[gi];
+      const int local = tile - G.tile0;
+      const int mg = local / G.p.num_n_blocks;
+      const int n_blk = local - mg * G.p.num_n_blocks;
+      const int m_blk = mg * 2 + static_cast<int>(rank);
+      if (gi > 0) chain_wait_ready(ready + (gi - 1) * cp.m_groups + mg, CHAIN_TILE_ARRIVALS * cp.g[gi - 1].p.num_n_blocks);
+      const uint32_t t_row = tmem_base + (static_cast<uint32_t>(sub * 32) << 16) + acc * ACC_STAGE_COLS;
+      const int key = gi * 65536 + n_blk;
+      if (G.family == EPI_LN_SOFTMAX)
+        chain_epilogue<EPI_LN_SOFTMAX>(G.p, m_blk, n_blk, lane, r, t_row, s_bias, s_col, bias_key, key, &tmem_full[acc],
+                                       acc_phase);
+      else if (G.family == EPI_LN_GEGLU)
+        chain_epilogue<EPI_LN_GEGLU>(G.p, m_blk, n_blk, lane, r, t_row, s_bias, s_col, bias_key, key, &tmem_full[acc],
+                                     acc_phase);
+      else
+        chain_epilogue<EPI_LN_PLAIN>(G.p, m_blk, n_blk, lane, r, t_row, s_bias, s_col, bias_key, key, &tmem_full[acc],
+                                     acc_phase);
+      tc_fence_before();
+      __syncwarp();
+      if (lane == 0) mbar_arrive_cluster(mapa_cluster(smem_u32(&tmem_empty[acc]), 0));
+      if (++acc == 2) {
+        acc = 0;
+        acc_phase ^= 1;
+      }
+#ifdef B200SR_CHAIN_WARP_PUBLISH
+      if (lane == 0) {
+#else
+      asm volatile("bar.sync 1, 128;" ::: "memory");
+      if (threadIdx.x == 64) {
+#endif
+        asm volatile("fence.acq_rel.gpu;" ::: "memory");
+        asm volatile("red.relaxed.gpu.global.add.u32 [%0], 1;" ::"l"(cp.counters + CHAIN_READY0 + gi * cp.m_groups + mg)
+                     : "memory");
+      }
+    }
+  }
+
+  tc_fence_before();
+  __syncthreads();
+  cluster_sync_all();
+  tc_fence_after();
+  if (warp == 1) tmem2_dealloc(tmem_base, TMEM_COLS);
+  if (threadIdx.x == 0) {
+    __threadfence();
+    const unsigned int prev = atomicAdd(cp.counters + 1, 1u);
+    if (prev == gridDim.x - 1) {
+      __threadfence();
+      const int n = CHAIN_READY0 + cp.n_gemms * cp.m_groups;
+      for (int i = 0; i < n; ++i) cp.counters[i] = 0u;
+      __threadfence();
+    }
+  }
+}
+
 static int ilog2_exact(int v) {
   int l = 0;
   while ((1 << l) < v) ++l;
@@ -1284,6 +1889,29 @@
   return B200SR_OK;
 }
 
+static int weight_map(CUtensorMap* tmB, const void* W, const GemmParams& p, int cluster) {
+  const long long w_rows = p.w_rows_per_group > 0
+                               ? ((static_cast<long long>(p.M) + p.w_rows_per_group - 1) / p.w_rows_per_group - 1) *
+                                         p.w_group_stride + p.N
+                               : p.N;
+  uint64_t dims[2] = {static_cast<uint64_t>(p.K), static_cast<uint64_t>(w_rows)};
+  uint64_t strides[1] = {static_cast<uint64_t>(p.K) * 2};
+  uint32_t box[2] = {BLOCK_K, static_cast<uint32_t>(p.BN / cluster)};
+  return make_tmap_bf16(tmB, W, 2, dims, strides, box);
+}
+
+static void set_wide_io(GemmParams& p) {
+  const long long n_out = p.geglu ? p.N / 2 : p.N;
+  const long long esz = p.out_fp32 ? 4 : 2;
+  p.wide_io = !p.out_fp32 && (n_out % 16) == 0 && (p.ldc * esz) % 32 == 0 && (reinterpret_cast<uintptr_t>(p.out) & 31) == 0 &&
+              (p.residual == nullptr || ((p.ldr * 2) % 32 == 0 && (reinterpret_cast<uintptr_t>(p.residual) & 31) == 0));
+  static const bool wide_enabled = [] {
+    const char* e = getenv("B200SR_WIDE_IO");
+    return e == nullptr || e[0] != '0';
+  }();
+  if (!wide_enabled) p.wide_io = 0;
+}
+
 static int finish(const CUtensorMap& tmA, const void* W, GemmParams& p, int real_m_blocks, int force_bn,
                   cudaStream_t stream) {
   const int cluster = real_m_blocks >= 2 ? 2 : 1;
@@ -1294,30 +1922,13 @@
   if (p.BN % (p.softmax_valid > 0 ? 16 : 32) != 0 || p.BN > 256 || p.BN <= 0) return B200SR_EINVAL;
   p.num_n_blocks = (p.N + p.BN - 1) / p.BN;
   CUtensorMap tmB;
-  const long long w_rows = p.w_rows_per_group > 0
-                               ? ((static_cast<long long>(p.M) + p.w_rows_per_group - 1) / p.w_rows_per_group - 1) *
-                                         p.w_group_stride + p.N
-                               : p.N;
-  uint64_t dims[2] = {static_cast<uint64_t>(p.K), static_cast<uint64_t>(w_rows)};
-  uint64_t strides[1] = {static_cast<uint64_t>(p.K) * 2};
-  uint32_t box[2] = {BLOCK_K, static_cast<uint32_t>(p.BN / cluster)};
-  int rc = make_tmap_bf16(&tmB, W, 2, dims, strides, box);
+  int rc = weight_map(&tmB, W, p, cluster);
   if (rc) return rc;
   static const bool epi_tma_enabled = [] {
     const char* e = getenv("B200SR_EPI_TMA");
     return e == nullptr || e[0] != '0';
   }();
-  {
-    const long long n_out = p.geglu ? p.N / 2 : p.N;
-    const long long esz = p.out_fp32 ? 4 : 2;
-    p.wide_io = !p.out_fp32 && (n_out % 16) == 0 && (p.ldc * esz) % 32 == 0 && (reinterpret_cast<uintptr_t>(p.out) & 31) == 0 &&
-                (p.residual == nullptr || ((p.ldr * 2) % 32 == 0 && (reinterpret_cast<uintptr_t>(p.residual) & 31) == 0));
-    static const bool wide_enabled = [] {
-      const char* e = getenv("B200SR_WIDE_IO");
-      return e == nullptr || e[0] != '0';
-    }();
-    if (!wide_enabled) p.wide_io = 0;
-  }
+  set_wide_io(p);
   CUtensorMap tmO = tmA;
   p.epi_tma = 0;
   if (epi_tma_enabled && p.mode == 0 && p.out_fp32 && !p.geglu && p.softmax_valid <= 0 && p.ln_stats == nullptr &&
@@ -1355,6 +1966,76 @@
   rc = make_tmap_bf16(&tmA, A, 2, dims, strides, box);
   if (rc) return rc;
   return finish(tmA, W, p, (M + BLOCK_M - 1) / BLOCK_M, force_bn, stream);
+}
+
+size_t gemm_chain_workspace_bytes(int M) {
+  if (M <= 0) return 0;
+  const int m_groups = (M + 2 * BLOCK_M - 1) / (2 * BLOCK_M);
+  return sizeof(unsigned int) * (CHAIN_READY0 + static_cast<size_t>(CHAIN_MAX_GEMMS) * m_groups);
+}
+
+int gemm_chain(const ChainGemmArgs* g, int n, unsigned int* counters, cudaStream_t stream) {
+  if (g == nullptr || counters == nullptr || n < 1 || n > CHAIN_MAX_GEMMS) return B200SR_EINVAL;
+  const int M = g[0].M;
+  if (M <= BLOCK_M) return B200SR_EINVAL;
+  ChainParams cp{};
+  const int m_blocks = (M + BLOCK_M - 1) / BLOCK_M;
+  cp.n_gemms = n;
+  cp.m_groups = (m_blocks + 1) / 2;
+  cp.counters = counters;
+  int tiles = 0, max_bn = 0;
+  for (int i = 0; i < n; ++i) {
+    const ChainGemmArgs& a = g[i];
+    if (a.M != M || a.A == nullptr || a.W == nullptr || a.N <= 0 || a.K <= 0 || (a.K % 8) != 0 || (a.lda % 8) != 0)
+      return B200SR_EINVAL;
+    GemmParams& p = cp.g[i].p;
+    p.mode = 0;
+    p.M = M;
+    p.N = a.N;
+    p.K = a.K;
+    p.k_iters = (a.K + BLOCK_K - 1) / BLOCK_K;
+    int rc = fill_epilogue(p, a.e);
+    if (rc) return rc;
+    if (p.row_softmax != 0 || p.rowvec != nullptr || p.act != 0 || p.out_fp32 || p.w_dynamic || p.gn_stats != nullptr)
+      return B200SR_EINVAL;
+    cp.g[i].family = p.softmax_valid > 0 ? EPI_LN_SOFTMAX : p.geglu ? EPI_LN_GEGLU : EPI_LN_PLAIN;
+    uint64_t dims[2] = {static_cast<uint64_t>(a.K), static_cast<uint64_t>(M)};
+    uint64_t strides[1] = {static_cast<uint64_t>(a.lda) * 2};
+    uint32_t box[2] = {BLOCK_K, BLOCK_M};
+    rc = make_tmap_bf16(&cp.tmA[i], a.A, 2, dims, strides, box);
+    if (rc) return rc;
+    p.num_m_blocks = cp.m_groups * 2;
+    p.BN = p.softmax_valid > 0 ? (p.N >= 3 * SOFTMAX_SEG ? 3 * SOFTMAX_SEG : p.N) : pick_bn(m_blocks, p.N, p.k_iters, num_sms(), 2);
+#ifdef B200SR_CHAIN_MAX_BN
+    if (p.ln_stats_out == nullptr && p.BN > B200SR_CHAIN_MAX_BN) p.BN = p.softmax_valid > 0 ? 2 * SOFTMAX_SEG : B200SR_CHAIN_MAX_BN;
+#endif
+    if (p.BN % (p.softmax_valid > 0 ? 16 : 32) != 0 || p.BN > ACC_STAGE_COLS || p.BN <= 0) return B200SR_EINVAL;
+    p.num_n_blocks = (p.N + p.BN - 1) / p.BN;
+    rc = weight_map(&cp.tmB[i], a.W, p, 2);
+    if (rc) return rc;
+    set_wide_io(p);
+    cp.g[i].tile0 = tiles;
+    tiles += cp.m_groups * p.num_n_blocks;
+    if (p.BN > max_bn) max_bn = p.BN;
+  }
+  cp.num_tiles = tiles;
+  cp.b_sub_stride = (max_bn / 2) * BLOCK_K * 2;
+  const int stage_bytes = KSUB * (A_STAGE_BYTES + cp.b_sub_stride);
+  const int smem_budget = 227 * 1024 - 1024 - BAR_REGION_BYTES - 4096  - 4096 ;
+  int stages = smem_budget / stage_bytes;
+  if (stages > MAX_STAGES) stages = MAX_STAGES;
+  if (stages < 2) return B200SR_EINVAL;
+  cp.stages = stages;
+  const size_t smem_bytes = static_cast<size_t>(stages) * stage_bytes + 1024 + BAR_REGION_BYTES + 4096 + 4096;
+  static bool attr_set[64] = {false};
+  if (first_use_on_device(attr_set)) {
+    const cudaError_t e = cudaFuncSetAttribute(gemm_chain_kernel, cudaFuncAttributeMaxDynamicSharedMemorySize, 227 * 1024);
+    if (e != cudaSuccess) return B200SR_ELAUNCH;
+  }
+  const int slots = num_sms() / 2;
+  const int grid = (tiles < slots ? tiles : slots) * 2;
+  const cudaError_t err = launch_k(gemm_chain_kernel, dim3(grid), dim3(GEMM_THREADS), smem_bytes, stream, 2, cp);
+  return err == cudaSuccess ? B200SR_OK : B200SR_ELAUNCH;
 }
 
 int conv3x3_bf16(const void* x, const void* w, int NB, int H, int W, int Cin, int Cout, int stride, int pad_lo,
```

Measured after the change: 35.64, median of 6. -6.1%, worse.
